# openai/tiktoken

Measured on NVIDIA H100. Metric: input_GB_per_s, higher is better.
Workload: dtype u8

## Files before the change

include/b200bpe.h:

```cpp
#ifndef B200BPE_H
#define B200BPE_H

#include <stdint.h>

#ifdef __cplusplus
extern "C" {
#endif

#define B200BPE_OK        0
#define B200BPE_EINVAL   -1
#define B200BPE_EPATTERN -2
#define B200BPE_EDUPRANK -3
#define B200BPE_ECUDA    -4
#define B200BPE_ENOBYTE  -5
#define B200BPE_EKEY     -6
#define B200BPE_ESPECIAL -7
#define B200BPE_ECAPACITY -8
#define B200BPE_ENOPAIR  -9

typedef struct b200bpe b200bpe_t;
typedef struct b200bpe_result b200bpe_result_t;

int b200bpe_create(const uint8_t *tok_bytes, const uint64_t *tok_off, const uint32_t *tok_rank,
                   uint32_t n_tok,
                   const uint8_t *sp_bytes, const uint64_t *sp_off, const uint32_t *sp_rank,
                   uint32_t n_sp,
                   const char *pat_str, int device, b200bpe_t **out);

int b200bpe_create_multi(const uint8_t *tok_bytes, const uint64_t *tok_off, const uint32_t *tok_rank,
                         uint32_t n_tok,
                         const uint8_t *sp_bytes, const uint64_t *sp_off, const uint32_t *sp_rank,
                         uint32_t n_sp,
                         const char *pat_str, const int *devices, int n_dev, b200bpe_t **out);

int b200bpe_n_devices(b200bpe_t *h);

int b200bpe_trim(b200bpe_t *h);

void b200bpe_destroy(b200bpe_t *h);

int b200bpe_encode_ordinary_batch(b200bpe_t *h, const uint8_t *text, const uint64_t *doc_off,
                                  uint64_t n_docs, b200bpe_result_t **out);

int b200bpe_encode_batch(b200bpe_t *h, const uint8_t *text, const uint64_t *doc_off, uint64_t n_docs,
                         const uint8_t *allowed, b200bpe_result_t **out);

int b200bpe_encode_batch_special(b200bpe_t *h, const uint8_t *text, const uint64_t *doc_off, uint64_t n_docs,
                                 const uint8_t *flags, b200bpe_result_t **out, int32_t *special_index);

int b200bpe_encode_bytes_batch(b200bpe_t *h, const uint8_t *text, const uint64_t *doc_off, uint64_t n_docs,
                               b200bpe_result_t **out);

int b200bpe_encode_with_unstable_batch(b200bpe_t *h, const uint8_t *text, const uint64_t *doc_off, uint64_t n_docs,
                                       const uint8_t *flags, b200bpe_result_t **stable, b200bpe_result_t **completions,
                                       int32_t *special_index);

int b200bpe_bpe_train(const uint8_t *text, const uint64_t *doc_off, uint64_t n_docs, const char *pat_str,
                      uint32_t vocab_size, int device, uint32_t *merges_out, uint64_t merges_cap,
                      uint64_t *n_merges_out, double *stats8);

const char *b200bpe_special_name(b200bpe_t *h, int32_t index);

int b200bpe_encode_device(b200bpe_t *h, const uint8_t *d_text, uint64_t n_bytes,
                          const uint64_t *d_doc_off, uint64_t n_docs,
                          uint32_t *d_tokens, uint64_t *d_tok_off, uint64_t *n_tokens, void *stream);

int b200bpe_encode_device_async(b200bpe_t *h, const uint8_t *d_text, uint64_t n_bytes,
                                const uint64_t *d_doc_off, uint64_t n_docs,
                                uint32_t *d_tokens, uint64_t *d_tok_off, uint64_t *d_counts, void *stream);
int b200bpe_device_wait(b200bpe_t *h, uint64_t *n_tokens);

int b200bpe_encode_single_piece(b200bpe_t *h, const uint8_t *piece, uint64_t len, b200bpe_result_t **out);

const uint32_t *b200bpe_result_tokens(const b200bpe_result_t *r);
const uint64_t *b200bpe_result_offsets(const b200bpe_result_t *r);
uint64_t b200bpe_result_n_tokens(const b200bpe_result_t *r);
const uint64_t *b200bpe_result_groups(const b200bpe_result_t *r, uint64_t *n_groups);
uint64_t b200bpe_result_n_docs(const b200bpe_result_t *r);
void b200bpe_result_free(b200bpe_result_t *r);

int b200bpe_decode_bytes(b200bpe_t *h, const uint32_t *tokens, uint64_t n_tokens, uint8_t *out,
                         uint64_t out_cap, uint64_t *out_len, uint32_t *bad_token);

int b200bpe_decode_batch(b200bpe_t *h, const uint32_t *tokens, const uint64_t *tok_off, uint64_t n_docs,
                         b200bpe_result_t **out, uint32_t *bad_token);

int b200bpe_last_timings(b200bpe_t *h, float *ms9, uint32_t *n_launches);

#define B200BPE_GREW_MISS 1u
#define B200BPE_GREW_SLOW 2u
#define B200BPE_GREW_LONG 4u
int b200bpe_last_reruns(b200bpe_t *h, uint32_t *grown, uint32_t *reruns, uint32_t *token_passes);

int b200bpe_last_piece_classes(b200bpe_t *h, uint64_t *counts8, int *lane_per_piece);

int b200bpe_last_bytes_repairs(b200bpe_t *h, uint64_t *n_docs_repaired);

int b200bpe_last_unstable(b200bpe_t *h, uint64_t *stats5);

int b200bpe_last_miss_memo(b200bpe_t *h, uint64_t *misses, uint64_t *merged, uint64_t *unplaced);

int b200bpe_table_bytes(b200bpe_t *h, uint64_t *bytes4);

int b200bpe_device_count(void);

const char *b200bpe_last_error(void);
const char *b200bpe_version(void);

#ifdef __cplusplus
}
#endif
#endif
```

tiktoken_b200/_lib.py:

```python
from __future__ import annotations

import ctypes as C
import os
import subprocess

_CSRC = os.path.join(os.path.dirname(os.path.abspath(__file__)), "csrc")
_SO = os.path.join(_CSRC, "libb200bpe.so")
_SOURCES = ["b200bpe.cu", "dev_common.cuh", "kernels_pretok.cuh", "kernels_long.cuh", "kernels_mid.cuh", "kernels_pmerge.cuh", "kernels_encode.cuh",
            "kernels_special.cuh", "kernels_decode.cuh", "kernels_bytes.cuh", "kernels_unstable.cuh", "kernels_train.cuh", "utf8_check.cuh", "bpe_device.cuh", "bpe_tables.h", "pretok_rules.cuh",
            "pretok_fast.cuh", "text_access.cuh", "unicode_classes.inc"]

OK, EINVAL, EPATTERN, EDUPRANK, ECUDA, ENOBYTE, EKEY, ESPECIAL, ECAPACITY, ENOPAIR = 0, -1, -2, -3, -4, -5, -6, -7, -8, -9

NVCC_FLAGS = ["-gencode", "arch=compute_90a,code=sm_90a", "-O3", "-lineinfo", "-std=c++17",
              "-shared", "-Xcompiler", "-fPIC"]


def build(force: bool = False) -> str:
    srcs = [os.path.join(_CSRC, s) for s in _SOURCES] + [
        os.path.join(os.path.dirname(_CSRC), "..", "include", "b200bpe.h")]
    stale = force or not os.path.exists(_SO) or any(
        os.path.getmtime(s) > os.path.getmtime(_SO) for s in srcs if os.path.exists(s))
    if stale:
        nvcc = os.environ.get("NVCC", "/usr/local/cuda/bin/nvcc")
        if not os.path.exists(nvcc):
            nvcc = "nvcc"
        subprocess.check_call([nvcc] + NVCC_FLAGS + ["-o", _SO, os.path.join(_CSRC, "b200bpe.cu")])
    return _SO


_lib = None


def lib() -> C.CDLL:
    global _lib
    if _lib is not None:
        return _lib
    so = os.environ.get("B200BPE_LIB") or _SO
    if not os.path.exists(so):
        raise RuntimeError(
            f"{so} is missing: build it with `python -c 'import __graft_entry__ as g; g.build()'` "
            "(tiktoken_b200 has no CPU fallback)")
    L = C.CDLL(so)
    vp, u64, u32, i32 = C.c_void_p, C.c_uint64, C.c_uint32, C.c_int
    L.b200bpe_create.restype = i32
    L.b200bpe_create.argtypes = [vp, vp, vp, u32, vp, vp, vp, u32, C.c_char_p, i32, C.POINTER(vp)]
    L.b200bpe_create_multi.restype = i32
    L.b200bpe_create_multi.argtypes = [vp, vp, vp, u32, vp, vp, vp, u32, C.c_char_p, vp, i32, C.POINTER(vp)]
    L.b200bpe_trim.restype = i32
    L.b200bpe_trim.argtypes = [vp]
    L.b200bpe_n_devices.restype = i32
    L.b200bpe_n_devices.argtypes = [vp]
    L.b200bpe_encode_batch_special.restype = i32
    L.b200bpe_encode_batch_special.argtypes = [vp, vp, vp, u64, vp, C.POINTER(vp), C.POINTER(C.c_int32)]
    L.b200bpe_special_name.restype = C.c_char_p
    L.b200bpe_special_name.argtypes = [vp, C.c_int32]
    L.b200bpe_encode_device_async.restype = i32
    L.b200bpe_encode_device_async.argtypes = [vp, vp, u64, vp, u64, vp, vp, vp, vp]
    L.b200bpe_device_wait.restype = i32
    L.b200bpe_device_wait.argtypes = [vp, C.POINTER(u64)]
    L.b200bpe_destroy.restype = None
    L.b200bpe_destroy.argtypes = [vp]
    L.b200bpe_encode_ordinary_batch.restype = i32
    L.b200bpe_encode_ordinary_batch.argtypes = [vp, vp, vp, u64, C.POINTER(vp)]
    L.b200bpe_encode_batch.restype = i32
    L.b200bpe_encode_batch.argtypes = [vp, vp, vp, u64, vp, C.POINTER(vp)]
    L.b200bpe_encode_device.restype = i32
    L.b200bpe_encode_device.argtypes = [vp, vp, u64, vp, u64, vp, vp, C.POINTER(u64), vp]
    L.b200bpe_encode_bytes_batch.restype = i32
    L.b200bpe_encode_bytes_batch.argtypes = [vp, vp, vp, u64, C.POINTER(vp)]
    L.b200bpe_last_bytes_repairs.restype = i32
    L.b200bpe_last_bytes_repairs.argtypes = [vp, C.POINTER(u64)]
    L.b200bpe_encode_with_unstable_batch.restype = i32
    L.b200bpe_encode_with_unstable_batch.argtypes = [vp, vp, vp, u64, vp, C.POINTER(vp), C.POINTER(vp), C.POINTER(C.c_int32)]
    L.b200bpe_result_groups.restype = vp
    L.b200bpe_result_groups.argtypes = [vp, C.POINTER(u64)]
    L.b200bpe_last_unstable.restype = i32
    L.b200bpe_last_unstable.argtypes = [vp, vp]
    L.b200bpe_last_miss_memo.restype = i32
    L.b200bpe_last_miss_memo.argtypes = [vp, C.POINTER(u64), C.POINTER(u64), C.POINTER(u64)]
    L.b200bpe_encode_single_piece.restype = i32
    L.b200bpe_encode_single_piece.argtypes = [vp, vp, u64, C.POINTER(vp)]
    L.b200bpe_result_tokens.restype = vp
    L.b200bpe_result_tokens.argtypes = [vp]
    L.b200bpe_result_offsets.restype = vp
    L.b200bpe_result_offsets.argtypes = [vp]
    L.b200bpe_result_n_tokens.restype = u64
    L.b200bpe_result_n_tokens.argtypes = [vp]
    L.b200bpe_result_n_docs.restype = u64
    L.b200bpe_result_n_docs.argtypes = [vp]
    L.b200bpe_result_free.restype = None
    L.b200bpe_result_free.argtypes = [vp]
    L.b200bpe_decode_bytes.restype = i32
    L.b200bpe_decode_bytes.argtypes = [vp, vp, u64, vp, u64, C.POINTER(u64), C.POINTER(u32)]
    L.b200bpe_decode_batch.restype = i32
    L.b200bpe_decode_batch.argtypes = [vp, vp, vp, u64, C.POINTER(vp), C.POINTER(u32)]
    L.b200bpe_last_timings.restype = i32
    L.b200bpe_last_timings.argtypes = [vp, vp, C.POINTER(u32)]
    L.b200bpe_last_reruns.restype = i32
    L.b200bpe_last_reruns.argtypes = [vp, C.POINTER(u32), C.POINTER(u32), C.POINTER(u32)]
    L.b200bpe_last_piece_classes.restype = i32
    L.b200bpe_last_piece_classes.argtypes = [vp, vp, C.POINTER(i32)]
    L.b200bpe_table_bytes.restype = i32
    L.b200bpe_table_bytes.argtypes = [vp, vp]
    L.b200bpe_device_count.restype = i32
    L.b200bpe_device_count.argtypes = []
    L.b200bpe_bpe_train.restype = i32
    L.b200bpe_bpe_train.argtypes = [vp, vp, u64, C.c_char_p, u32, i32, vp, u64, C.POINTER(u64), vp]
    L.b200bpe_last_error.restype = C.c_char_p
    L.b200bpe_version.restype = C.c_char_p
    _lib = L
    return L


EXPORTS = [
    "b200bpe_create", "b200bpe_destroy", "b200bpe_encode_ordinary_batch", "b200bpe_encode_batch",
    "b200bpe_encode_device", "b200bpe_encode_single_piece", "b200bpe_result_tokens",
    "b200bpe_result_offsets", "b200bpe_result_n_tokens", "b200bpe_result_n_docs", "b200bpe_result_free",
    "b200bpe_decode_bytes", "b200bpe_decode_batch", "b200bpe_last_timings", "b200bpe_table_bytes", "b200bpe_last_error",
    "b200bpe_version", "b200bpe_device_count", "b200bpe_create_multi", "b200bpe_n_devices", "b200bpe_encode_batch_special",
    "b200bpe_special_name", "b200bpe_encode_device_async", "b200bpe_device_wait", "b200bpe_trim", "b200bpe_last_reruns",
    "b200bpe_last_piece_classes", "b200bpe_encode_bytes_batch", "b200bpe_last_bytes_repairs", "b200bpe_last_miss_memo",
    "b200bpe_encode_with_unstable_batch", "b200bpe_result_groups", "b200bpe_last_unstable", "b200bpe_bpe_train",
]

GREW_MISS, GREW_SLOW, GREW_LONG = 1, 2, 4


def last_error() -> str:
    return (lib().b200bpe_last_error() or b"").decode("utf-8", "replace")


def check(rc: int) -> None:
    if rc == OK:
        return
    msg = last_error()
    if rc in (EINVAL, EPATTERN, EDUPRANK, ESPECIAL, ENOPAIR):
        raise ValueError(msg)
    if rc == EKEY:
        raise KeyError(msg)
    if rc == ENOBYTE:
        raise KeyError(msg)
    raise RuntimeError(msg)
```

tiktoken_b200/_tiktoken.py:

```python
from __future__ import annotations

import ctypes as C
import threading

import numpy as np

from . import _lib

try:
    from . import _b200pack
except ImportError:
    _b200pack = None


def _ptr(a: np.ndarray):
    return C.c_void_p(a.ctypes.data)


def _flatten_bytes(items: list[bytes]):
    blob = b"".join(items)
    off = np.zeros(len(items) + 1, dtype=np.uint64)
    if items:
        np.cumsum(np.fromiter((len(b) for b in items), dtype=np.uint64, count=len(items)), out=off[1:])
    arr = np.frombuffer(blob, dtype=np.uint8) if blob else np.zeros(1, np.uint8)
# ... 253 lines not shown
        if s in self._special:
            return self._special[s]
        raise KeyError(bytes(piece))

    def _encode_bytes(self, data: bytes) -> list[int]:
        try:
            text = data.decode("utf-8")
        except UnicodeDecodeError:
            raise NotImplementedError(
                "_encode_bytes on invalid UTF-8 (unstable-token path, src/py.rs:79-112) is out of scope "
                "of the GPU encoder") from None
        return self.encode_ordinary(text)

    def encode_with_unstable(self, text: str, allowed_special):
        raise NotImplementedError("encode_with_unstable (completion search, src/lib.rs:444-599) is out of scope")

    def decode_bytes(self, tokens) -> bytes:
        arr = np.ascontiguousarray(np.asarray(tokens, dtype=np.uint32))
        n = len(arr)
        if n == 0:
            return b""
        out_len = C.c_uint64(0)
        bad = C.c_uint32(0)
        cap = max(64, 8 * n)
        while True:
            out = np.empty(cap, np.uint8)
            rc = self._L.b200bpe_decode_bytes(self._h, _ptr(arr), n, _ptr(out), cap, C.byref(out_len), C.byref(bad))
            if rc == _lib.EKEY:
                raise KeyError(f"Invalid token for decoding: {bad.value}")
            _lib.check(rc)
            if out_len.value <= cap:
                return out[:out_len.value].tobytes()
            cap = int(out_len.value)

    def decode_batch_buffer(self, tokens: np.ndarray, tok_off: np.ndarray):
        tokens = np.ascontiguousarray(tokens, np.uint32)
        tok_off = np.ascontiguousarray(tok_off, np.uint64)
        res = C.c_void_p()
        bad = C.c_uint32(0)
        rc = self._L.b200bpe_decode_batch(self._h, _ptr(tokens if len(tokens) else np.zeros(1, np.uint32)), _ptr(tok_off),
                                          len(tok_off) - 1, C.byref(res), C.byref(bad))
        if rc == _lib.EKEY:
            raise KeyError(f"Invalid token for decoding: {bad.value}")
        _lib.check(rc)
        n_bytes = int(self._L.b200bpe_result_n_tokens(res))
        n_docs = int(self._L.b200bpe_result_n_docs(res))
        data = np.ctypeslib.as_array(C.cast(self._L.b200bpe_result_tokens(res), C.POINTER(C.c_uint8)),
                                     shape=(max(n_bytes, 1),))[:n_bytes].copy()
        off = np.ctypeslib.as_array(C.cast(self._L.b200bpe_result_offsets(res), C.POINTER(C.c_uint64)),
                                    shape=(n_docs + 1,)).copy()
        self._L.b200bpe_result_free(res)
        return data, off

    def decode_bytes_batch(self, batch) -> list[bytes]:
        lens = np.fromiter((len(t) for t in batch), dtype=np.uint64, count=len(batch))
        off = np.zeros(len(batch) + 1, np.uint64)
        np.cumsum(lens, out=off[1:])
        toks = np.zeros(int(off[-1]), np.uint32)
        for i, t in enumerate(batch):
            toks[int(off[i]):int(off[i + 1])] = np.asarray(t, dtype=np.uint32)
        data, boff = self.decode_batch_buffer(toks, off)
        raw = data.tobytes()
        return [raw[int(boff[i]):int(boff[i + 1])] for i in range(len(batch))]

    def decode_single_token_bytes(self, token: int) -> bytes:
        if self._decoder is None:
            self._decoder = {v: k for k, v in self._encoder.items()}
            self._decoder.update({v: k.encode("utf-8") for k, v in self._special.items()})
        try:
            return self._decoder[token]
        except KeyError:
            raise KeyError(str(token)) from None

    def token_byte_values(self) -> list[bytes]:
        return sorted(self._encoder.keys())

    def last_timings(self) -> dict:
        ms = (C.c_float * 9)()
        n = C.c_uint32(0)
        self._L.b200bpe_last_timings(self._h, ms, C.byref(n))
        keys = ["mark_docs_ms", "pretok_ms", "long_ms", "encode_ms", "device_total_ms", "h2d_ms", "d2h_ms", "gather_ms", "probe_ms"]
        d = {k: float(ms[i]) for i, k in enumerate(keys)}
        d["launches"] = int(n.value)
        return d

    def last_reruns(self) -> dict:
        grown, reruns, passes = C.c_uint32(0), C.c_uint32(0), C.c_uint32(0)
        _lib.check(self._L.b200bpe_last_reruns(self._h, C.byref(grown), C.byref(reruns), C.byref(passes)))
        names = {_lib.GREW_MISS: "miss", _lib.GREW_SLOW: "slow", _lib.GREW_LONG: "long"}
        return {"grown": {s for bit, s in names.items() if grown.value & bit}, "reruns": int(reruns.value),
                "token_passes": int(passes.value)}

    def last_piece_classes(self) -> dict:
        counts, lane = (C.c_uint64 * 8)(), C.c_int32(0)
        _lib.check(self._L.b200bpe_last_piece_classes(self._h, counts, C.byref(lane)))
        return {"counts": [int(x) for x in counts], "lane_per_piece": bool(lane.value)}

    def last_bytes_repairs(self) -> int:
        n = C.c_uint64(0)
        _lib.check(self._L.b200bpe_last_bytes_repairs(self._h, C.byref(n)))
        return int(n.value)

    def last_unstable(self) -> dict:
        v = (C.c_uint64 * 5)()
        _lib.check(self._L.b200bpe_last_unstable(self._h, v))
        return dict(zip(["docs", "encoded", "bpe_candidates", "rounds", "completions"], (int(x) for x in v)))

    def last_miss_memo(self) -> dict:
        v = [C.c_uint64(0) for _ in range(3)]
        _lib.check(self._L.b200bpe_last_miss_memo(self._h, *(C.byref(x) for x in v)))
        return {"misses": int(v[0].value), "merged": int(v[1].value), "unplaced": int(v[2].value)}

    def trim(self) -> None:
        _lib.check(self._L.b200bpe_trim(self._h))

    def table_bytes(self) -> dict:
        b = (C.c_uint64 * 4)()
        self._L.b200bpe_table_bytes(self._h, b)
        return {"piece_table": int(b[0]), "pair_table": int(b[1]), "long_token_table": int(b[2]), "unicode": int(b[3])}

    def encode_device_async(self, d_text_ptr: int, n_bytes: int, d_doc_off_ptr: int, n_docs: int, d_tokens_ptr: int,
                            d_tok_off_ptr: int, d_counts_ptr: int = 0, stream: int = 0) -> None:
        _lib.check(self._L.b200bpe_encode_device_async(self._h, C.c_void_p(d_text_ptr), n_bytes, C.c_void_p(d_doc_off_ptr),
                                                       n_docs, C.c_void_p(d_tokens_ptr), C.c_void_p(d_tok_off_ptr),
                                                       C.c_void_p(d_counts_ptr), C.c_void_p(stream)))

    def device_wait(self) -> int:
        n = C.c_uint64(0)
        _lib.check(self._L.b200bpe_device_wait(self._h, C.byref(n)))
        return int(n.value)

    def encode_device(self, d_text_ptr: int, n_bytes: int, d_doc_off_ptr: int, n_docs: int, d_tokens_ptr: int,
                      d_tok_off_ptr: int, stream: int = 0) -> int:
        n = C.c_uint64(0)
        rc = self._L.b200bpe_encode_device(self._h, C.c_void_p(d_text_ptr), n_bytes, C.c_void_p(d_doc_off_ptr),
                                           n_docs, C.c_void_p(d_tokens_ptr), C.c_void_p(d_tok_off_ptr), C.byref(n),
                                           C.c_void_p(stream))
        _lib.check(rc)
        return int(n.value)
```

tiktoken_b200/csrc/b200bpe.cu:

```cuda
#include <cuda_runtime.h>
#include <stdint.h>
#include <stdio.h>
#include <stdlib.h>
#include <string.h>

#include <algorithm>
#include <atomic>
#include <condition_variable>
#include <deque>
#include <functional>
#include <mutex>
#include <string>
#include <thread>
#include <vector>

#include "../../include/b200bpe.h"
#include "dev_common.cuh"
#include "kernels_pretok.cuh"
#include "kernels_long.cuh"
#include "kernels_mid.cuh"
#include "kernels_pmerge.cuh"
#include "kernels_encode.cuh"
#include "kernels_special.cuh"
#include "kernels_decode.cuh"
// ... 42 lines not shown
        return e;
    }
    void release() { if (p) cudaFree(p); p = nullptr; cap = 0; }
};

struct PinnedBuf {
    void *p = nullptr; size_t cap = 0;
};

long env_long(const char *name, long dflt, long lo, long hi) {
    const char *v = getenv(name);
    if (!v || !*v) return dflt;
    long x = atol(v);
    return x < lo ? lo : x > hi ? hi : x;
}

size_t env_chunk_bytes() {
    const char *v = getenv("B200BPE_CHUNK_MB");
    const long x = v ? atol(v) : 0;
    return x >= 1 && x <= 2048 ? (size_t)x << 20 : 0;
}

struct TaskPool {
    std::vector<std::thread> th; std::mutex mu; std::condition_variable cv; std::deque<std::function<void()>> q; bool stop = false;
    void ensure(int n) {
        std::lock_guard<std::mutex> lk(mu);
        while ((int)th.size() < n) th.emplace_back([this] {
            for (;;) {
                std::function<void()> f;
                {
                    std::unique_lock<std::mutex> lk(mu);
                    cv.wait(lk, [this] { return stop || !q.empty(); });
                    if (q.empty()) return;
                    f = std::move(q.front()); q.pop_front();
                }
                f();
            }
        });
    }
    void push(std::function<void()> f) { { std::lock_guard<std::mutex> lk(mu); q.push_back(std::move(f)); } cv.notify_one(); }
    ~TaskPool() {
        { std::lock_guard<std::mutex> lk(mu); stop = true; }
        cv.notify_all();
        for (auto &t : th) t.join();
    }
};
struct Latch {
    std::mutex mu; std::condition_variable cv; int left;
    explicit Latch(int n) : left(n) {}
    void done() { std::lock_guard<std::mutex> lk(mu); if (--left == 0) cv.notify_all(); }
    void wait() { std::unique_lock<std::mutex> lk(mu); cv.wait(lk, [this] { return left == 0; }); }
};
void pool_for(TaskPool *pool, size_t n, size_t block, const std::function<void(size_t, size_t)> &fn) {
    const size_t nb = (n + block - 1) / block;
    if (!pool || nb <= 1) { if (n) fn(0, n); return; }
    Latch latch((int)nb);
    for (size_t b = 0; b < nb; b++) pool->push([&, b] { fn(b * block, std::min(n, (b + 1) * block)); latch.done(); });
    latch.wait();
}

}

struct Slot {
    DevBuf<uint8_t> w_text; DevBuf<unsigned long long> w_docoff, w_tokoff, w_sub_base;
    DevBuf<uint32_t> w_ptok, w_mres, w_mq_pos, w_mq_roff, w_doc_tiles, w_sub_count; DevBuf<uint8_t> w_mq_len;
    DevBuf<uint4> w_mq_key, w_mq_skey, w_mq_smeta, w_mq_rec;
    DevBuf<uint4> w_memo_key; DevBuf<uint32_t> w_memo_owner, w_mq_slot, w_mq_own, w_memo_bn;
    DevBuf<uint32_t> w_dbits, w_pbits, w_psum, w_sfd, w_lidx, w_out, w_ltok, w_hbits, w_ibits, w_sbits, w_cbits, w_slow;
    DevBuf<unsigned long long> w_lq_start, w_lq_off; DevBuf<unsigned int> w_lq_len, w_lq_ntok, w_lq_cls, w_big_n, w_sort_hist;
    DevBuf<unsigned long long> w_big_dst, w_big_src, w_scan_part;
    DevBuf<uint32_t> w_idA, w_rkA, w_idB, w_rkB, w_aux1, w_aux2; DevBuf<uint8_t> w_flag, w_spflags;
    DevBuf<uint32_t> w_vup, w_kdrop, w_btail, w_b2out, w_bout; DevBuf<uint8_t> w_btext;
    DevBuf<unsigned long long> w_b2doc, w_b2off, w_bbase, w_bpart;
    Counters *d_bctr = nullptr; BytesCounters *d_bytes = nullptr, *h_bytes = nullptr;
    DevBuf<uint32_t> w_ulen, w_unit;
    size_t long_cap = 0;
    size_t miss_cap = 0, mres_cap = 0;
    size_t slow_cap = 0;
    Counters *d_ctr = nullptr; Counters *h_ctr = nullptr;
    unsigned int *d_sticky = nullptr;
    cudaStream_t stream = nullptr;
    cudaStream_t side = nullptr;
    cudaStream_t side2 = nullptr;
    cudaStream_t up = nullptr;
    static const int N_EV = 15;
    cudaEvent_t ev[N_EV];
    PinnedBuf stage;
    float last_ms[9] = {0, 0, 0, 0, 0, 0, 0, 0, 0};
    uint32_t last_launches = 0;
    bool ok = false;

    cudaError_t init() {
        cudaError_t e = cudaMalloc((void **)&d_ctr, sizeof(Counters));
        if (e == cudaSuccess) e = cudaMalloc((void **)&d_sticky, 16);
        if (e == cudaSuccess) e = cudaMemset(d_sticky, 0, 16);
        if (e == cudaSuccess) e = cudaHostAlloc((void **)&h_ctr, sizeof(Counters), cudaHostAllocPortable);
        if (e == cudaSuccess) e = cudaStreamCreateWithFlags(&stream, cudaStreamNonBlocking);
        if (e == cudaSuccess) e = cudaStreamCreateWithFlags(&side, cudaStreamNonBlocking);
        if (e == cudaSuccess) e = cudaStreamCreateWithFlags(&side2, cudaStreamNonBlocking);
        if (e == cudaSuccess) e = cudaStreamCreateWithFlags(&up, cudaStreamNonBlocking);
        for (int i = 0; i < N_EV && e == cudaSuccess; i++) e = cudaEventCreate(&ev[i]);
        ok = (e == cudaSuccess);
        return e;
    }
    void release_workspace() {
        w_text.release(); w_docoff.release(); w_tokoff.release(); w_sub_base.release();
        w_ptok.release(); w_mres.release(); w_mq_pos.release(); w_mq_roff.release(); w_doc_tiles.release(); w_sub_count.release();
        w_mq_len.release(); w_mq_rec.release(); w_mq_key.release(); w_mq_skey.release(); w_mq_smeta.release();
        w_memo_key.release(); w_memo_owner.release(); w_mq_slot.release(); w_mq_own.release(); w_memo_bn.release();
        w_dbits.release(); w_pbits.release(); w_psum.release(); w_sfd.release(); w_lidx.release(); w_out.release(); w_ltok.release();
        w_hbits.release(); w_ibits.release(); w_sbits.release(); w_cbits.release(); w_slow.release(); w_spflags.release();
        w_lq_start.release(); w_lq_off.release(); w_lq_len.release(); w_lq_ntok.release(); w_lq_cls.release(); w_big_n.release();
        w_sort_hist.release(); w_big_dst.release(); w_big_src.release(); w_scan_part.release();
        w_idA.release(); w_rkA.release(); w_idB.release(); w_rkB.release(); w_aux1.release(); w_aux2.release();
        w_flag.release();
        w_vup.release(); w_kdrop.release(); w_btail.release(); w_b2out.release(); w_bout.release(); w_btext.release();
        w_b2doc.release(); w_b2off.release(); w_bbase.release(); w_bpart.release();
        w_ulen.release(); w_unit.release();
        if (stage.p) cudaFreeHost(stage.p);
        stage.p = nullptr; stage.cap = 0;
        long_cap = miss_cap = mres_cap = slow_cap = 0;
    }
    void destroy() {
        release_workspace();
        if (d_ctr) cudaFree(d_ctr);
        if (d_bctr) cudaFree(d_bctr);
        if (d_bytes) cudaFree(d_bytes);
        if (h_bytes) cudaFreeHost(h_bytes);
        if (d_sticky) cudaFree(d_sticky);
        if (h_ctr) cudaFreeHost(h_ctr);
        if (ok) { for (int i = 0; i < N_EV; i++) cudaEventDestroy(ev[i]); }
        if (stream) cudaStreamDestroy(stream);
        if (side) cudaStreamDestroy(side);
        if (side2) cudaStreamDestroy(side2);
        if (up) cudaStreamDestroy(up);
    }
};

struct UnstWs {
    DevBuf<uint32_t> it_lo, it_cnt, it_bytes, it_doc; DevBuf<unsigned long long> item_base, cbase, tbase, part;
    DevBuf<uint4> cinfo; DevBuf<uint32_t> o_len, s_len, out_o, out_s, nkeep, slot, keep, kc;
    DevBuf<unsigned long long> o_off, s_off, tokoff_o, tokoff_s, rcb, rtb, zeros, grp_off;
    DevBuf<uint8_t> text_o, text_s;
    DevBuf<unsigned long long> tkey; DevBuf<uint32_t> tidx, tloc;
    uint32_t tslots_min = 0;
    DevBuf<uint32_t> res_tok, res_doc, grp; DevBuf<unsigned long long> res_off;
    UnstCounters *d_uc = nullptr, *h_uc = nullptr;
    Counters *d_sctr = nullptr;
    void release() {
        it_lo.release(); it_cnt.release(); it_bytes.release(); it_doc.release(); item_base.release(); cbase.release();
        tbase.release(); part.release(); cinfo.release(); o_len.release(); s_len.release(); out_o.release(); out_s.release();
        nkeep.release(); slot.release(); keep.release(); kc.release(); o_off.release(); s_off.release(); tokoff_o.release();
        tokoff_s.release(); rcb.release(); rtb.release(); zeros.release(); grp_off.release(); text_o.release(); text_s.release();
        tkey.release(); tidx.release(); tloc.release(); res_tok.release(); res_doc.release(); grp.release(); res_off.release();
    }
};

struct DevCtx {
    int device = 0;
    uint8_t *arena = nullptr; size_t arena_bytes = 0;
    DevTables T; UcTables uc;
    uint32_t *d_tok_boff = nullptr; uint8_t *d_tok_blob = nullptr;
    uint32_t *d_tok_space = nullptr;
    SpecialTables sp;
    uint8_t *d_sp_arena = nullptr;
    UnstTables ut;
    uint8_t *d_ut_arena = nullptr;
    UnstWs uw;
    static const int N_SLOTS = 3;
    Slot slots[N_SLOTS];
    int n_sm = 0;
};

struct b200bpe_result {
    b200bpe *owner = nullptr;
    PinnedBuf tok, off;
    std::vector<uint32_t> vtok;
    std::vector<uint64_t> voff;
    std::vector<uint64_t> vgrp;
    bool on_host_vec = false;
    uint64_t n_tokens = 0, n_docs = 0;
};

struct PendingDeviceCall {
    bool active = false; int queued = 0;
    const uint8_t *d_text = nullptr; uint64_t n_bytes = 0; const unsigned long long *d_doc_off = nullptr; uint64_t n_docs = 0;
    uint32_t *d_tokens = nullptr; unsigned long long *d_tok_off = nullptr; unsigned long long *d_counts = nullptr;
    cudaStream_t st = nullptr;
};

struct b200bpe {
    int pattern = 0;
    HostTables H;
    std::vector<std::string> specials; std::vector<uint32_t> special_rank;
    std::unordered_map<uint32_t, std::string> special_decoder;
    SpecialHost sp_host;
    uint32_t n_ids = 0; bool decode_on_device = true;
    std::vector<uint32_t> tok_space;
    std::vector<DevCtx *> devs;
    uint64_t table_bytes[4] = {0, 0, 0, 0};
    float last_ms[9] = {0, 0, 0, 0, 0, 0, 0, 0, 0};
    uint32_t last_launches = 0;
    std::atomic<uint32_t> last_grown{0}, last_reruns{0}, last_token_passes{0};
    std::atomic<uint64_t> last_cls[N_CLS] = {};
    std::atomic<int> last_lane_per_piece{0};
    std::atomic<uint64_t> last_bytes_repairs{0};
    std::atomic<uint64_t> last_unstable[5] = {};
    struct {
        bool built = false;
        std::vector<uint32_t> sorted, space, ur_idx, ur_off, ur_tok; std::vector<unsigned long long> lenpre;
        std::vector<uint8_t> u8info; uint32_t max_len = 0;
    } uh;
    std::atomic<uint64_t> last_memo[3] = {};
    void reset_reruns() {
        last_grown = 0; last_reruns = 0; last_token_passes = 0; last_bytes_repairs = 0;
        for (auto &c : last_unstable) c = 0;
        for (auto &c : last_memo) c = 0;
        for (auto &c : last_cls) c = 0;
        last_lane_per_piece = 0;
    }
    void set_piece_classes(const uint64_t *cls) {
        for (int c = 0; c < N_CLS; c++) last_cls[c] = cls[c];
        last_lane_per_piece = mid_group ? 0 : 1;
    }
    void set_miss_memo(const uint64_t *memo) { for (int i = 0; i < 3; i++) last_memo[i] = memo[i]; }
    size_t chunk_bytes = 64u << 20; bool chunk_forced = false;
    int copy_threads = 4;
    TaskPool *pool = nullptr;
    long memo_slots = -1;
    bool mid_group = true;
    std::mutex mu;
    std::vector<PinnedBuf> pinned_pool;
    int live_results = 0;
    bool dead = false;
    PendingDeviceCall pending;

    PinnedBuf take_pinned(size_t bytes) {
        for (size_t i = 0; i < pinned_pool.size(); i++)
            if (pinned_pool[i].cap >= bytes && pinned_pool[i].cap <= 2 * bytes + (64u << 20)) {
                PinnedBuf b = pinned_pool[i]; pinned_pool.erase(pinned_pool.begin() + i); return b;
            }
        PinnedBuf b; size_t want = bytes + bytes / 8 + 4096;
        if (cudaHostAlloc(&b.p, want, cudaHostAllocPortable) != cudaSuccess) { cudaGetLastError(); b.p = nullptr; b.cap = 0; return b; }
        b.cap = want; return b;
    }
    void give_pinned(PinnedBuf b) {
        if (!b.p) return;
        if (pinned_pool.size() >= 4) {
            size_t mn = 0;
            for (size_t i = 1; i < pinned_pool.size(); i++) if (pinned_pool[i].cap < pinned_pool[mn].cap) mn = i;
            if (pinned_pool[mn].cap >= b.cap) { cudaFreeHost(b.p); return; }
            cudaFreeHost(pinned_pool[mn].p); pinned_pool[mn] = b; return;
        }
        pinned_pool.push_back(b);
    }
};

extern "C" const char *b200bpe_last_error(void) { return g_last_error.c_str(); }
extern "C" const char *b200bpe_version(void) { return "b200bpe 0.2 (sm_90a)"; }
extern "C" int b200bpe_device_count(void) {
    int n = 0;
    if (cudaGetDeviceCount(&n) != cudaSuccess) { cudaGetLastError(); return 0; }
    return n;
}

static void devctx_destroy(DevCtx *D) {
    if (!D) return;
    cudaSetDevice(D->device);
    for (int i = 0; i < DevCtx::N_SLOTS; i++) D->slots[i].destroy();
    if (D->arena) cudaFree(D->arena);
    if (D->d_tok_boff) cudaFree(D->d_tok_boff);
    if (D->d_tok_blob) cudaFree(D->d_tok_blob);
    if (D->d_tok_space) cudaFree(D->d_tok_space);
    if (D->d_sp_arena) cudaFree(D->d_sp_arena);
    if (D->d_ut_arena) cudaFree(D->d_ut_arena);
    D->uw.release();
    delete D;
}

static void uc_ascii_table(uint8_t *ascii) {
    for (int i = 0; i < 128; i++) ascii[i] = UC_STAGE2[(uint32_t)UC_STAGE1[0] * 256 + i];
}

static int devctx_create(b200bpe *h, int device, const std::vector<uint32_t> &boff, const std::vector<uint8_t> &blob,
                         DevCtx **out) {
    DevCtx *D = new DevCtx();
    D->device = device;
    const HostTables &H = h->H;
    cudaError_t e = cudaSetDevice(device);
    if (e == cudaSuccess) e = cudaDeviceGetAttribute(&D->n_sm, cudaDevAttrMultiProcessorCount, device);
    uint8_t ascii[128];
    uc_ascii_table(ascii);
    struct Part { const void *src; size_t bytes; size_t off; };
    enum { P_NARROW, P_WIDE, P_PAIR2, P_BYTE_ID, P_PAIR, P_ASCII, P_UC1, P_UC2, P_LONG, P_BLOB, N_PARTS };
    Part parts[N_PARTS] = {{H.narrow_tab.data(), H.narrow_tab.size() * sizeof(U4), 0},
                           {H.wide_tab.data(), H.wide_tab.size() * sizeof(U4), 0}, {H.pair2.data(), 65536 * 4, 0},
                           {H.byte_id.data(), 256 * 4, 0}, {H.pair_tab.data(), H.pair_tab.size() * sizeof(U4), 0},
// ... 83 lines not shown
            bool all = !sp->empty();
            for (char c : *sp) all &= c == ' ' || c == '\n' || c == '\t';
            if (all) space[id >> 5] |= 1u << (id & 31);
        }
    }
    boff[h->n_ids] = (uint32_t)blob.size(); boff[h->n_ids + 1] = (uint32_t)blob.size();
    if (blob.empty()) blob.push_back(0);
    for (int i = 0; i < n_dev; i++) {
        DevCtx *D = nullptr;
        rc = devctx_create(h, devices[i], boff, blob, &D);
        if (rc) { for (auto *d : h->devs) devctx_destroy(d); delete h; return rc; }
        h->devs.push_back(D);
    }
    if (const size_t cb = env_chunk_bytes()) { h->chunk_bytes = cb; h->chunk_forced = true; }
    h->mid_group = H.max_rank < MIDG_MAX_RANK;
    h->memo_slots = env_long("B200BPE_MISS_MEMO_SLOTS", -1, 0, 1l << 24);
    h->copy_threads = (int)env_long("B200BPE_COPY_THREADS", std::max(1u, std::min(16u, std::thread::hardware_concurrency() / 4)), 1, 64);
    h->table_bytes[0] = (H.narrow_tab.size() + H.wide_tab.size()) * sizeof(U4);
    h->table_bytes[1] = H.pair_tab.size() * sizeof(U4) + 65536 * 4 + 1024;
    h->table_bytes[2] = H.long_tab.size() * sizeof(U4) + H.long_blob.size();
    h->table_bytes[3] = sizeof(UC_STAGE1) + sizeof(UC_STAGE2) + 128;
    *out = h;
    return B200BPE_OK;
}

extern "C" int b200bpe_create(const uint8_t *tok_bytes, const uint64_t *tok_off, const uint32_t *tok_rank,
                              uint32_t n_tok, const uint8_t *sp_bytes, const uint64_t *sp_off,
                              const uint32_t *sp_rank, uint32_t n_sp, const char *pat_str, int device,
                              b200bpe_t **out) {
    return b200bpe_create_multi(tok_bytes, tok_off, tok_rank, n_tok, sp_bytes, sp_off, sp_rank, n_sp, pat_str, &device, 1, out);
}

static void engine_teardown(b200bpe *h) {
    DeviceGuard guard;
    for (auto *d : h->devs) devctx_destroy(d);
    for (auto &b : h->pinned_pool) cudaFreeHost(b.p);
    delete h->pool;
    delete h;
}

extern "C" void b200bpe_destroy(b200bpe_t *h) {
    if (!h) return;
    {
        std::lock_guard<std::mutex> lk(h->mu);
        if (h->live_results > 0) { h->dead = true; return; }
    }
    engine_teardown(h);
}

extern "C" int b200bpe_n_devices(b200bpe_t *h) { return h ? (int)h->devs.size() : 0; }

extern "C" int b200bpe_trim(b200bpe_t *h) {
    if (!h) return fail(B200BPE_EINVAL, "null handle");
    std::lock_guard<std::mutex> lk(h->mu);
    if (h->pending.active) return fail(B200BPE_EINVAL, "a device call is in flight: b200bpe_device_wait first");
    DeviceGuard guard;
    for (auto *D : h->devs) {
        CUDA_TRY(cudaSetDevice(D->device));
        for (int i = 0; i < DevCtx::N_SLOTS; i++) {
            CUDA_TRY(cudaStreamSynchronize(D->slots[i].stream));
            CUDA_TRY(cudaStreamSynchronize(D->slots[i].side));
            CUDA_TRY(cudaStreamSynchronize(D->slots[i].side2));
            D->slots[i].release_workspace();
        }
    }
    for (auto &b : h->pinned_pool) cudaFreeHost(b.p);
    h->pinned_pool.clear();
    return B200BPE_OK;
}

struct PipeArgs {
    const uint8_t *d_text = nullptr; uint64_t n_bytes = 0;
    const unsigned long long *d_doc_off = nullptr; uint64_t n_docs = 0;
    uint32_t *d_out = nullptr; unsigned long long *d_tok_off = nullptr;
    unsigned long long *d_counts = nullptr;
    cudaStream_t st = nullptr;
    bool single_piece = false;
    bool bytes = false;
    bool unstable = false;
    const uint8_t *sp_flags = nullptr;
};

static const unsigned long long MISS_CAP_MIN = 1u << 16, LONG_CAP_MIN = 1u << 20;

static int enqueue_pipeline(b200bpe *h, DevCtx *D, Slot &S, const PipeArgs &a) {
    const uint64_t n_bytes = a.n_bytes, n_docs = a.n_docs;
    cudaStream_t st = a.st;
    if (n_bytes >= (1ull << 32) - 4096) return fail(B200BPE_EINVAL, "batch too large for one call (>= 4 GiB)");
    if (n_docs >= 0xFFFFFFFEull) return fail(B200BPE_EINVAL, "too many documents in one call");
    const long long n_words = (long long)((n_bytes + 1 + 31) / 32);
    const long long n_tiles = (n_words + 31) / 32;
    const size_t pb_words = (size_t)n_tiles * 32 + STAGE_PW + 8;
    CUDA_TRY(S.w_dbits.ensure((size_t)n_words + 8));
    CUDA_TRY(S.w_pbits.ensure(pb_words));
    CUDA_TRY(S.w_psum.ensure((size_t)(n_words >> 5) + 4));
    CUDA_TRY(S.w_sfd.ensure((size_t)n_words + 4));
    CUDA_TRY(S.w_sub_base.ensure((size_t)n_tiles + 2));
    CUDA_TRY(S.w_scan_part.ensure((size_t)(n_tiles / SCAN_ITEMS) + 4));
    CUDA_TRY(S.w_sub_count.ensure((size_t)n_tiles + 2));
    CUDA_TRY(S.w_ptok.ensure((size_t)n_tiles * SUB_BYTES + 64));
    {
        const size_t want_q = std::max<size_t>((size_t)(n_bytes / 8) + 4096, MISS_CAP_MIN);
        const size_t want_r = std::max<size_t>((size_t)(n_bytes / 2) + 4096, MISS_CAP_MIN);
        if (S.miss_cap < want_q) S.miss_cap = want_q;
        if (S.mres_cap < want_r) S.mres_cap = want_r;
        const size_t mcap = S.miss_cap;
        CUDA_TRY(S.w_mq_pos.ensure(mcap)); CUDA_TRY(S.w_mq_roff.ensure(mcap)); CUDA_TRY(S.w_mq_rec.ensure(mcap));
        CUDA_TRY(S.w_mq_len.ensure(mcap));
        CUDA_TRY(S.w_mq_key.ensure(mcap)); CUDA_TRY(S.w_mq_skey.ensure(mcap)); CUDA_TRY(S.w_mq_smeta.ensure(mcap));
        CUDA_TRY(S.w_mres.ensure(S.mres_cap + 64));
        CUDA_TRY(S.w_sort_hist.ensure((size_t)D->n_sm * SORT_BLOCKS_PER_SM * 17 + 32));
        CUDA_TRY(S.w_mq_slot.ensure(mcap)); CUDA_TRY(S.w_mq_own.ensure(mcap));
        CUDA_TRY(S.w_memo_bn.ensure((size_t)D->n_sm * SORT_BLOCKS_PER_SM * 2 + 4));
    }
    uint32_t memo_slots = 0;
    if (h->memo_slots) {
        const uint64_t want = h->memo_slots > 0 ? (uint64_t)h->memo_slots
                                                : std::min<uint64_t>(std::max<uint64_t>(n_bytes / 128, 1u << 12), 1u << 21);
        memo_slots = 1;
        while (memo_slots < want) memo_slots <<= 1;
        CUDA_TRY(S.w_memo_key.ensure(memo_slots)); CUDA_TRY(S.w_memo_owner.ensure(memo_slots));
    }
    {
        const size_t want = std::max<size_t>((size_t)(n_bytes / 8) + 4096, MISS_CAP_MIN);
        if (S.slow_cap < want) S.slow_cap = want;
        CUDA_TRY(S.w_slow.ensure(S.slow_cap));
    }
    CUDA_TRY(S.w_lidx.ensure((size_t)(n_bytes >> 4) + 4));
    CUDA_TRY(S.w_ltok.ensure((size_t)n_bytes + 4));
    const size_t qcap = (size_t)(n_bytes / (SHORT_MAX + 1)) + 4;
    CUDA_TRY(S.w_lq_start.ensure(qcap)); CUDA_TRY(S.w_lq_off.ensure(qcap));
    CUDA_TRY(S.w_lq_len.ensure(qcap)); CUDA_TRY(S.w_lq_ntok.ensure(qcap));
    size_t cls_cap[N_CLS], cls_total = 0;
    {
        const size_t min_len[N_CLS] = {SHORT_MAX + 1, 33, 65, 129, 257, GROUP_MAX + 1, BLOCK_MIN + 1, CLUSTER_MIN + 1};
        for (int c = 0; c < N_CLS; c++) { cls_cap[c] = (size_t)(n_bytes / min_len[c]) + 4; cls_total += cls_cap[c]; }
    }
    CUDA_TRY(S.w_lq_cls.ensure(cls_total));
    CUDA_TRY(S.w_big_n.ensure((size_t)(n_bytes / 4097) + 4));
    CUDA_TRY(S.w_big_dst.ensure((size_t)(n_bytes / 4097) + 4)); CUDA_TRY(S.w_big_src.ensure((size_t)(n_bytes / 4097) + 4));
    {
        const size_t want = std::max<size_t>((size_t)(n_bytes / 8) + 4096, LONG_CAP_MIN);
        if (S.long_cap < want) S.long_cap = want;
        const size_t lc = S.long_cap + 4;
        CUDA_TRY(S.w_idA.ensure(lc)); CUDA_TRY(S.w_rkA.ensure(lc)); CUDA_TRY(S.w_idB.ensure(lc)); CUDA_TRY(S.w_rkB.ensure(lc));
        CUDA_TRY(S.w_aux1.ensure(lc)); CUDA_TRY(S.w_aux2.ensure(lc)); CUDA_TRY(S.w_flag.ensure(lc));
    }
    LongQ q;
    q.start = S.w_lq_start.p; q.len = S.w_lq_len.p; q.off = S.w_lq_off.p; q.ntok = S.w_lq_ntok.p; q.scratch_cap = S.long_cap;
    q.sub_count = S.w_sub_count.p;
    { size_t o = 0; for (int c = 0; c < N_CLS; c++) { q.cls[c] = S.w_lq_cls.p + o; o += cls_cap[c]; } }
    const bool sparse_docs = (n_docs + 1) * 4 < (uint64_t)n_tiles;
    if (sparse_docs) CUDA_TRY(S.w_doc_tiles.ensure((size_t)n_docs + 8));
    uint32_t launches = 0;

    CUDA_TRY(cudaEventRecord(S.ev[0], st));
    CUDA_TRY(cudaMemsetAsync(S.d_ctr, 0, sizeof(Counters), st));
    CUDA_TRY(cudaMemsetAsync(S.w_dbits.p, 0, ((size_t)n_words + 8) * 4, st));
    CUDA_TRY(cudaMemsetAsync(S.w_sfd.p, 0xFF, ((size_t)n_words + 4) * 4, st));
    CUDA_TRY(cudaMemsetAsync(S.w_sub_count.p, 0, ((size_t)n_tiles + 2) * 4, st));
    CUDA_TRY(cudaMemsetAsync(S.w_pbits.p + n_words, 0, (pb_words - (size_t)n_words) * 4, st));
    {
        unsigned long long nd1 = n_docs + 1;
        mark_docs_kernel<<<(unsigned)((nd1 + 255) / 256), 256, 0, st>>>(a.d_doc_off, n_docs, n_bytes, S.w_dbits.p, S.w_sfd.p,
                                                                       sparse_docs ? S.w_doc_tiles.p : nullptr, S.d_ctr);
        launches++;
    }
    const uint32_t *hbits = S.w_dbits.p;
    const uint32_t *ibits = nullptr, *sbits = nullptr;
    if (a.sp_flags && !h->specials.empty() && !a.single_piece) {
        const size_t nsp = h->specials.size();
        CUDA_TRY(S.w_spflags.ensure(nsp + 16));
        CUDA_TRY(S.w_hbits.ensure((size_t)n_words + 8)); CUDA_TRY(S.w_ibits.ensure((size_t)n_words + 8));
        CUDA_TRY(S.w_sbits.ensure((size_t)n_words + 8)); CUDA_TRY(S.w_cbits.ensure((size_t)n_words + 8));
        CUDA_TRY(cudaMemcpyAsync(S.w_spflags.p, a.sp_flags, nsp, cudaMemcpyHostToDevice, st));
        CUDA_TRY(cudaMemsetAsync(S.w_ibits.p, 0, ((size_t)n_words + 8) * 4, st));
        CUDA_TRY(cudaMemsetAsync(S.w_cbits.p + n_words, 0, 8 * 4, st));
        const unsigned grid = (unsigned)((n_words + 255) / 256);
        special_mark_kernel<<<grid, 256, 0, st>>>(a.d_text, (long long)n_bytes, S.w_dbits.p, D->sp, S.w_spflags.p, S.w_cbits.p, n_words, S.d_ctr);
        CUDA_TRY(cudaMemcpyAsync(S.w_hbits.p, S.w_dbits.p, ((size_t)n_words + 8) * 4, cudaMemcpyDeviceToDevice, st));
        special_resolve_kernel<<<grid, 256, 0, st>>>(a.d_text, (long long)n_bytes, S.w_dbits.p, D->sp, S.w_spflags.p, S.w_cbits.p,
                                                     S.w_hbits.p, S.w_ibits.p, S.w_sbits.p, S.w_ltok.p, n_words, S.d_ctr);
        launches += 2;
        hbits = S.w_hbits.p; ibits = S.w_ibits.p; sbits = S.w_sbits.p;
    } else if (a.bytes) {
        if (!D->d_tok_space) {
            CUDA_TRY(cudaMalloc((void **)&D->d_tok_space, h->tok_space.size() * 4));
            CUDA_TRY(cudaMemcpy(D->d_tok_space, h->tok_space.data(), h->tok_space.size() * 4, cudaMemcpyHostToDevice));
        }
        if (!S.d_bytes) CUDA_TRY(cudaMalloc((void **)&S.d_bytes, sizeof(BytesCounters)));
        if (!S.h_bytes) CUDA_TRY(cudaHostAlloc((void **)&S.h_bytes, sizeof(BytesCounters), cudaHostAllocPortable));
        CUDA_TRY(cudaMemsetAsync(S.d_bytes, 0, sizeof(BytesCounters), st));
        CUDA_TRY(S.w_hbits.ensure((size_t)n_words + 8)); CUDA_TRY(S.w_ibits.ensure((size_t)n_words + 8));
        CUDA_TRY(S.w_sbits.ensure((size_t)n_words + 8)); CUDA_TRY(S.w_vup.ensure((size_t)n_docs + 2));
        CUDA_TRY(cudaMemsetAsync(S.w_ibits.p, 0, ((size_t)n_words + 8) * 4, st));
        CUDA_TRY(cudaMemsetAsync(S.w_sbits.p, 0, ((size_t)n_words + 8) * 4, st));
        CUDA_TRY(cudaMemsetAsync(S.w_vup.p, 0xFF, ((size_t)n_docs + 2) * 4, st));
        utf8_check_kernel<<<(unsigned)((n_words + 255) / 256), 256, 0, st>>>(a.d_text, (long long)n_bytes, S.w_dbits.p, S.w_sfd.p,
                                                                            a.d_doc_off, n_docs, n_words, S.w_vup.p);
        CUDA_TRY(cudaMemcpyAsync(S.w_hbits.p, S.w_dbits.p, ((size_t)n_words + 8) * 4, cudaMemcpyDeviceToDevice, st));
        if (n_docs) bytes_cut_kernel<<<(unsigned)((n_docs * 32 + 255) / 256), 256, 0, st>>>(a.d_doc_off, n_docs, S.w_vup.p, S.w_hbits.p,
                                                                                          S.w_ibits.p, S.w_sbits.p, S.w_ltok.p);
        launches += 2;
        hbits = S.w_hbits.p; ibits = S.w_ibits.p; sbits = S.w_sbits.p;
    }
    CUDA_TRY(cudaEventRecord(S.ev[1], st));
    {
        unsigned grid = (unsigned)((n_words + 255) / 256);
        if (a.single_piece) single_piece_bits_kernel<<<grid, 256, 0, st>>>(S.w_pbits.p, S.w_psum.p, S.w_dbits.p, n_words);
        else {
            const uint32_t scap = (uint32_t)std::min<size_t>(S.slow_cap, 0xFFFFFFF0u);
#define B2_PRETOK(P)                                                                                                                   \
    if (a.bytes) pretok_kernel<P, true><<<grid, 256, 0, st>>>(a.d_text, (long long)n_bytes, hbits, D->uc, S.w_pbits.p, S.w_psum.p,       \
                                                             n_words, ibits, S.w_slow.p, scap, S.d_ctr);                              \
    else pretok_kernel<P><<<grid, 256, 0, st>>>(a.d_text, (long long)n_bytes, hbits, D->uc, S.w_pbits.p, S.w_psum.p, n_words, ibits,          \
                                          S.w_slow.p, scap, S.d_ctr);                                                                  \
    pretok_slow_kernel<P><<<D->n_sm * 8, 256, 0, st>>>(a.d_text, (long long)n_bytes, hbits, D->uc, S.w_pbits.p, S.w_psum.p, S.w_slow.p, scap, S.d_ctr)
            if (h->pattern == PAT_R50K) { B2_PRETOK(PAT_R50K); }
            else if (h->pattern == PAT_CL100K) { B2_PRETOK(PAT_CL100K); }
            else { B2_PRETOK(PAT_O200K); }
#undef B2_PRETOK
            launches++;
        }
        launches++;
    }
    CUDA_TRY(cudaEventRecord(S.ev[2], st));
    {
        unsigned grid = (unsigned)((n_words + 255) / 256);
        find_long_kernel<<<grid, 256, 0, st>>>(S.w_pbits.p, S.w_psum.p, (long long)n_bytes, n_words, q, S.w_lidx.p, sbits, S.d_ctr);
        launches++;
        cudaStream_t ls = S.side, ls2 = S.side2;
        CUDA_TRY(cudaEventRecord(S.ev[10], st));
        CUDA_TRY(cudaStreamWaitEvent(ls, S.ev[10], 0));
        CUDA_TRY(cudaStreamWaitEvent(ls2, S.ev[10], 0));
        CUDA_TRY(cudaEventRecord(S.ev[11], ls));
        LongScratch LS{S.w_idA.p, S.w_rkA.p, S.w_idB.p, S.w_rkB.p, S.w_aux1.p, S.w_aux2.p, S.w_flag.p};
        if (h->mid_group) {
            pmerge_kernel<256, 3><<<D->n_sm * 10, PM_WARPS * 32, 0, ls>>>(a.d_text, D->T, q, S.w_ltok.p, S.d_ctr);
            pmerge_long_kernel<<<D->n_sm * 4, PM_WARPS_L * 32, 0, ls>>>(a.d_text, D->T, q, S.w_ltok.p, S.d_ctr);
            mid_group32_kernel<<<D->n_sm * 4, MIDG_WARPS * 32, 0, ls>>>(a.d_text, D->T, q, S.w_ltok.p, S.d_ctr, 2);
            mid_group16_kernel<<<D->n_sm * 9, MIDG_WARPS * 32, 0, ls>>>(a.d_text, D->T, q, S.w_ltok.p, S.d_ctr, 1);
        } else {
            mid_thread_kernel<<<D->n_sm * 3, MID_WARPS * 32, MID_SMEM_BYTES, ls>>>(a.d_text, D->T, q, S.w_ltok.p, S.d_ctr);
            long_piece_kernel<<<D->n_sm * 8, LONG_WARPS * 32, 0, ls>>>(a.d_text, D->T, q, LS, S.w_ltok.p, S.d_ctr, CLS_G1024);
        }
        long_piece_kernel<<<D->n_sm * 8, LONG_WARPS * 32, 0, ls2>>>(a.d_text, D->T, q, LS, S.w_ltok.p, S.d_ctr, CLS_WARP);
        giant_piece_kernel<<<D->n_sm, GIANT_THREADS, 0, ls2>>>(a.d_text, D->T, q, LS, S.w_ltok.p, S.d_ctr);
        cluster_piece_kernel<<<(D->n_sm / CLUSTER_CTAS) * CLUSTER_CTAS, GIANT_THREADS, 0, ls2>>>(a.d_text, D->T, q, LS, S.w_ltok.p, S.d_ctr);
        CUDA_TRY(cudaEventRecord(S.ev[13], ls2));
        CUDA_TRY(cudaEventRecord(S.ev[12], ls));
        launches += 5;
    }
    CUDA_TRY(cudaEventRecord(S.ev[3], st));
    {
        TileParams p;
        p.text = a.d_text; p.n_bytes = (long long)n_bytes; p.n_words = n_words; p.n_sub = n_tiles;
        p.pbits = S.w_pbits.p; p.dbits = S.w_dbits.p; p.span_first_doc = S.w_sfd.p;
        p.doc_off = a.d_doc_off; p.n_docs = n_docs; p.q = q; p.lidx = S.w_lidx.p; p.ltok = S.w_ltok.p;
        p.ptok = S.w_ptok.p; p.mres = S.w_mres.p; p.sbits = sbits;
        p.mq.key = S.w_mq_key.p; p.mq.pos = S.w_mq_pos.p; p.mq.roff = S.w_mq_roff.p; p.mq.len = S.w_mq_len.p; p.mq.rec = S.w_mq_rec.p;
        p.doc_tiles = S.w_doc_tiles.p;
        p.mq.skey = S.w_mq_skey.p; p.mq.smeta = S.w_mq_smeta.p; p.mq.cap = (uint32_t)std::min<size_t>(S.miss_cap, 0xFFFFFFF0u);
        p.mq.mres_cap = S.mres_cap;
        p.sub_count = S.w_sub_count.p; p.sub_base = S.w_sub_base.p;
        p.out = a.d_out; p.tok_off = a.d_tok_off; p.ctr = S.d_ctr;
        p.big_dst = S.w_big_dst.p; p.big_src = S.w_big_src.p; p.big_n = S.w_big_n.p;
        MissMemo memo;
        memo.key = S.w_memo_key.p; memo.owner = S.w_memo_owner.p; memo.slot = S.w_mq_slot.p; memo.own = S.w_mq_own.p;
        memo.block_n = S.w_memo_bn.p; memo.mask = memo_slots ? memo_slots - 1 : 0; memo.on = memo_slots ? 1u : 0u;
        memo.limit = std::max<uint32_t>(1u, memo_slots / 2 / (uint32_t)(D->n_sm * SORT_BLOCKS_PER_SM));
        const long long want_blocks = (n_tiles + ENC_WARPS - 1) / ENC_WARPS;
        const unsigned probe_grid = (unsigned)std::min<long long>(want_blocks, (long long)D->n_sm * PROBE_BLOCKS_PER_SM);
        probe_kernel<<<probe_grid, ENC_WARPS * 32, 0, st>>>(p, D->T);
        CUDA_TRY(cudaEventRecord(S.ev[8], st));
        const int sort_blocks = D->n_sm * SORT_BLOCKS_PER_SM;
        if (memo_slots) CUDA_TRY(cudaMemsetAsync(S.w_memo_key.p, 0, (size_t)memo_slots * sizeof(uint4), st));
        miss_dedup_kernel<<<sort_blocks, SORT_THREADS, 0, st>>>(p, memo, S.w_sort_hist.p);
        miss_base_kernel<<<1, 17 * 32, 0, st>>>(S.w_sort_hist.p, sort_blocks);
        miss_scatter_kernel<<<sort_blocks, SORT_THREADS, 0, st>>>(p, memo, S.w_sort_hist.p);
        miss_kernel<<<D->n_sm * 16, MISS_WARPS * 32, 0, st>>>(p, D->T);
        if (memo_slots) miss_fanout_kernel<<<sort_blocks, SORT_THREADS, 0, st>>>(p, memo);
        CUDA_TRY(cudaEventRecord(S.ev[7], st));
        CUDA_TRY(cudaStreamWaitEvent(st, S.ev[12], 0));
        CUDA_TRY(cudaStreamWaitEvent(st, S.ev[13], 0));
        {
            const long long nb = (n_tiles + SCAN_ITEMS - 1) / SCAN_ITEMS;
            scan_partial_kernel<<<(unsigned)nb, 256, 0, st>>>(S.w_sub_count.p, n_tiles, S.w_scan_part.p);
            scan_top_kernel<<<1, 1024, 0, st>>>(S.w_scan_part.p, nb, S.d_ctr);
            scan_final_kernel<<<(unsigned)nb, 256, 0, st>>>(S.w_sub_count.p, n_tiles, S.w_scan_part.p, S.w_sub_base.p, S.d_ctr);
        }
        const unsigned gather_grid = (unsigned)((n_tiles + GATHER_WARPS - 1) / GATHER_WARPS);
        if (sparse_docs) {
            gather_kernel<0><<<gather_grid, GATHER_WARPS * 32, 0, st>>>(p);
            gather_kernel<1><<<(unsigned)((n_docs + 1 + GATHER_WARPS - 1) / GATHER_WARPS), GATHER_WARPS * 32, 0, st>>>(p);
        } else gather_kernel<2><<<gather_grid, GATHER_WARPS * 32, 0, st>>>(p);
        big_copy_kernel<<<D->n_sm * 2, 256, 0, st>>>(p);
        if (a.bytes && n_docs) {
            CUDA_TRY(S.w_kdrop.ensure((size_t)n_docs + 2)); CUDA_TRY(S.w_btail.ensure((size_t)n_docs + 2));
            bytes_repair_kernel<<<(unsigned)((n_docs * 32 + 255) / 256), 256, 0, st>>>(a.d_doc_off, n_docs, S.w_vup.p, S.w_pbits.p, a.d_out,
                                                                                      a.d_tok_off, D->d_tok_boff, D->d_tok_space, h->n_ids,
                                                                                      S.w_kdrop.p, S.w_btail.p, S.d_bytes, S.d_ctr);
            launches++;
        }
        if (a.unstable && n_docs) {
            CUDA_TRY(S.w_kdrop.ensure((size_t)n_docs + 2)); CUDA_TRY(S.w_ulen.ensure((size_t)n_docs + 2));
            CUDA_TRY(S.w_unit.ensure((size_t)n_docs + 2));
            unstable_walk_kernel<<<(unsigned)((n_docs * 32 + 255) / 256), 256, 0, st>>>(a.d_doc_off, n_docs, S.w_pbits.p, sbits, a.d_out,
                                                                                       a.d_tok_off, D->d_tok_boff, D->ut.space, h->n_ids,
                                                                                       D->ut.max_len, S.w_kdrop.p, S.w_ulen.p,
                                                                                       S.w_unit.p, S.d_ctr);
            launches++;
        }
        finalize_kernel<<<1, 32, 0, st>>>(S.d_ctr, S.d_sticky, a.d_counts, n_docs);
        launches += (sparse_docs ? 12 : 11) + (memo_slots ? 1 : 0);
    }
    CUDA_TRY(cudaEventRecord(S.ev[4], st));
    if (a.bytes) CUDA_TRY(cudaMemcpyAsync(S.h_bytes, S.d_bytes, sizeof(BytesCounters), cudaMemcpyDeviceToHost, st));
    CUDA_TRY(cudaMemcpyAsync(S.h_ctr, S.d_ctr, sizeof(Counters), cudaMemcpyDeviceToHost, st));
    CUDA_TRY(cudaEventRecord(S.ev[9], st));
    S.last_launches = launches;
    return B200BPE_OK;
}

static const int B200BPE_RETRY = 1;

static int collect_pipeline(b200bpe *h, Slot &S, int *special_idx, uint64_t *special_pos, uint32_t *grown) {
    (void)h;
    CUDA_TRY(cudaEventSynchronize(S.ev[9]));
    CUDA_TRY(cudaGetLastError());
    cudaEventElapsedTime(&S.last_ms[0], S.ev[0], S.ev[1]);
    cudaEventElapsedTime(&S.last_ms[1], S.ev[1], S.ev[2]);
    cudaEventElapsedTime(&S.last_ms[2], S.ev[11], S.ev[12]);
    cudaEventElapsedTime(&S.last_ms[3], S.ev[3], S.ev[7]);
    cudaEventElapsedTime(&S.last_ms[7], S.ev[7], S.ev[4]);
    cudaEventElapsedTime(&S.last_ms[8], S.ev[3], S.ev[8]);
    cudaEventElapsedTime(&S.last_ms[4], S.ev[0], S.ev[4]);
    const Counters &c = *S.h_ctr;
    if (c.err & ERR_DOCOFF)
        return fail(B200BPE_EINVAL, "document offsets must start at 0, be non-decreasing and end at n_bytes");
    if (c.err & ERR_SPECIAL) {
        const unsigned long long packed = ~c.special_pos;
        if (special_idx) *special_idx = (int)(packed & 0xFFFFu);
        if (special_pos) *special_pos = packed >> 16;
        return fail(B200BPE_ESPECIAL, "text contains a disallowed special token");
    }
    if (c.err & (ERR_LONGCAP | ERR_MISSCAP | ERR_SLOWCAP)) {
        if (c.err & ERR_SLOWCAP) S.slow_cap = (size_t)c.n_slow + (size_t)(c.n_slow / 8) + 4096;
        if (c.err & ERR_LONGCAP) S.long_cap = (size_t)c.long_bytes + (size_t)(c.long_bytes / 8) + 4096;
        if (c.err & ERR_MISSCAP) {
            S.miss_cap = std::max(S.miss_cap, (size_t)c.n_miss + (size_t)(c.n_miss / 8) + 4096);
            S.mres_cap = std::max(S.mres_cap, (size_t)c.miss_bytes + (size_t)(c.miss_bytes / 8) + 4096);
        }
        *grown |= ((c.err & ERR_MISSCAP) ? B200BPE_GREW_MISS : 0u) | ((c.err & ERR_SLOWCAP) ? B200BPE_GREW_SLOW : 0u) |
                  ((c.err & ERR_LONGCAP) ? B200BPE_GREW_LONG : 0u);
        return B200BPE_RETRY;
    }
    if (c.err & ERR_INTERNAL) return fail(B200BPE_ECUDA, "internal error: a merge kernel did not converge");
    if (c.err & ERR_NOBYTE)
        return fail(B200BPE_ENOBYTE, "a piece needs a single-byte token that mergeable_ranks does not contain");
    return B200BPE_OK;
}

static void add_miss_memo(const Slot &S, uint64_t *memo) {
    memo[0] += S.h_ctr->n_miss; memo[1] += S.h_ctr->n_owner; memo[2] += S.h_ctr->n_unplaced;
}

static int device_args_check(b200bpe *h, const uint8_t *d_text, uint64_t n_bytes, const uint64_t *d_doc_off, uint32_t *d_tokens,
                             uint64_t *d_tok_off) {
    if (!h || !d_doc_off || !d_tokens || !d_tok_off || (n_bytes && !d_text)) return fail(B200BPE_EINVAL, "null argument");
    return B200BPE_OK;
}

static int device_enqueue_locked(b200bpe *h, const PendingDeviceCall &c) {
    DevCtx *D = h->devs[0];
    Slot &S = D->slots[0];
    cudaStream_t st = c.st ? c.st : S.stream;
    const uint8_t *txt = c.d_text;
    if (((uintptr_t)c.d_text & 15u) != 0) {
        CUDA_TRY(S.w_text.ensure((size_t)c.n_bytes + 64));
        CUDA_TRY(cudaMemcpyAsync(S.w_text.p, c.d_text, c.n_bytes, cudaMemcpyDeviceToDevice, st));
        txt = S.w_text.p;
    }
    PipeArgs a;
    a.d_text = txt; a.n_bytes = c.n_bytes; a.d_doc_off = c.d_doc_off; a.n_docs = c.n_docs; a.d_out = c.d_tokens;
    a.d_tok_off = c.d_tok_off; a.d_counts = c.d_counts; a.st = st;
    return enqueue_pipeline(h, D, S, a);
}

extern "C" int b200bpe_encode_device_async(b200bpe_t *h, const uint8_t *d_text, uint64_t n_bytes, const uint64_t *d_doc_off,
                                           uint64_t n_docs, uint32_t *d_tokens, uint64_t *d_tok_off, uint64_t *d_counts,
                                           void *stream) {
    if (h) h->reset_reruns();
    int rc = device_args_check(h, d_text, n_bytes, d_doc_off, d_tokens, d_tok_off);
    if (rc) return rc;
    std::lock_guard<std::mutex> lk(h->mu);
    DeviceGuard guard;
    CUDA_TRY(cudaSetDevice(h->devs[0]->device));
    PendingDeviceCall c;
    c.active = true; c.queued = h->pending.active ? h->pending.queued + 1 : 1;
    c.d_text = d_text; c.n_bytes = n_bytes; c.d_doc_off = (const unsigned long long *)d_doc_off; c.n_docs = n_docs;
    c.d_tokens = d_tokens; c.d_tok_off = (unsigned long long *)d_tok_off; c.d_counts = (unsigned long long *)d_counts;
    c.st = (cudaStream_t)stream;
    rc = device_enqueue_locked(h, c);
    if (rc) return rc;
    h->pending = c;
    return B200BPE_OK;
}

extern "C" int b200bpe_device_wait(b200bpe_t *h, uint64_t *n_tokens) {
    if (!h) return fail(B200BPE_EINVAL, "null handle");
    h->reset_reruns();
    std::lock_guard<std::mutex> lk(h->mu);
    if (!h->pending.active) return fail(B200BPE_EINVAL, "no device call in flight");
    DeviceGuard guard;
    DevCtx *D = h->devs[0];
    CUDA_TRY(cudaSetDevice(D->device));
    Slot &S = D->slots[0];
    PendingDeviceCall c = h->pending;
    h->pending.active = false;
    h->last_token_passes = 1;
    cudaStream_t st = c.st ? c.st : S.stream;
    uint32_t grown = 0;
    int rc = collect_pipeline(h, S, nullptr, nullptr, &grown);
    h->last_grown = grown;
    const uint64_t total = S.h_ctr->total_tokens;
    unsigned int sticky = 0;
    CUDA_TRY(cudaMemcpyAsync(&sticky, S.d_sticky, sizeof(unsigned int), cudaMemcpyDeviceToHost, st));
    CUDA_TRY(cudaMemsetAsync(S.d_sticky, 0, sizeof(unsigned int), st));
    CUDA_TRY(cudaStreamSynchronize(st));
    uint64_t total2 = total;
    bool reran = false;
    for (int attempt = 0; rc == B200BPE_RETRY && attempt < 4; attempt++) {
        rc = device_enqueue_locked(h, c);
        if (rc) break;
        h->last_reruns++;
        rc = collect_pipeline(h, S, nullptr, nullptr, &grown);
        h->last_grown = grown;
        total2 = S.h_ctr->total_tokens;
        CUDA_TRY(cudaMemsetAsync(S.d_sticky, 0, sizeof(unsigned int), st));
        reran = true;
    }
    memcpy(h->last_ms, S.last_ms, sizeof(h->last_ms));
    h->last_ms[5] = h->last_ms[6] = 0.f;
    h->last_launches = S.last_launches;
    if (rc == B200BPE_RETRY) return fail(B200BPE_ECUDA, "work-space sizing did not converge");
    if (rc) return rc;
    if (c.queued > 1) {
        if (reran || (sticky & (ERR_LONGCAP | ERR_MISSCAP | ERR_SLOWCAP)))
            return fail(B200BPE_ECAPACITY, "a work-space had to grow while several device calls were queued: only the last "
                                           "one was re-run, re-issue the others");
        if (sticky & ERR_NOBYTE) return fail(B200BPE_ENOBYTE, "a piece needs a single-byte token that mergeable_ranks does not contain");
        if (sticky & ERR_DOCOFF) return fail(B200BPE_EINVAL, "malformed document offsets in a queued device call");
    }
    if (n_tokens) *n_tokens = total2;
    uint64_t cls[N_CLS];
    for (int k = 0; k < N_CLS; k++) cls[k] = S.h_ctr->n_cls[k];
    h->set_piece_classes(cls);
    uint64_t memo[3] = {};
    add_miss_memo(S, memo);
    h->set_miss_memo(memo);
    return B200BPE_OK;
}

extern "C" int b200bpe_encode_device(b200bpe_t *h, const uint8_t *d_text, uint64_t n_bytes, const uint64_t *d_doc_off,
                                     uint64_t n_docs, uint32_t *d_tokens, uint64_t *d_tok_off, uint64_t *n_tokens,
                                     void *stream) {
    int rc = b200bpe_encode_device_async(h, d_text, n_bytes, d_doc_off, n_docs, d_tokens, d_tok_off, nullptr, stream);
    if (rc) return rc;
    return b200bpe_device_wait(h, n_tokens);
}

static void enqueue_scan(const uint32_t *cnt, uint64_t n, unsigned long long *part, unsigned long long *base, Counters *ctr,
                         cudaStream_t st) {
    const long long nb = (long long)((n + SCAN_ITEMS - 1) / SCAN_ITEMS);
    scan_partial_kernel<<<(unsigned)nb, 256, 0, st>>>(cnt, (long long)n, part);
    scan_top_kernel<<<1, 1024, 0, st>>>(part, nb, ctr);
    scan_final_kernel<<<(unsigned)nb, 256, 0, st>>>(cnt, (long long)n, part, base, ctr);
}

static int run_again(b200bpe *h, DevCtx *D, Slot &S, const PipeArgs &a, uint64_t *cls, uint64_t *memo, uint32_t *grown,
                     uint32_t *reruns) {
    int rc = enqueue_pipeline(h, D, S, a);
    if (!rc) rc = collect_pipeline(h, S, nullptr, nullptr, grown);
    for (int attempt = 0; rc == B200BPE_RETRY && attempt < 4; attempt++) {
        rc = enqueue_pipeline(h, D, S, a);
        if (!rc) { (*reruns)++; rc = collect_pipeline(h, S, nullptr, nullptr, grown); }
    }
    if (rc == B200BPE_RETRY) rc = fail(B200BPE_ECUDA, "work-space sizing did not converge");
    if (rc) return rc;
    for (int i = 0; i < N_CLS; i++) cls[i] += S.h_ctr->n_cls[i];
    add_miss_memo(S, memo);
    return B200BPE_OK;
}

static int bytes_tail_runs(b200bpe *h, DevCtx *D, Slot &S, const PipeArgs &a1, uint64_t *nt, uint64_t *cls, uint64_t *memo,
                           uint32_t *grown, uint32_t *reruns) {
    const uint64_t n1 = S.h_ctr->total_tokens, drop = S.h_bytes->drop;
    const float ms1[9] = {S.last_ms[0], S.last_ms[1], S.last_ms[2], S.last_ms[3], S.last_ms[4], S.last_ms[5], S.last_ms[6],
                          S.last_ms[7], S.last_ms[8]};
    const uint32_t launches1 = S.last_launches;
    const uint64_t nd = a1.n_docs, tail = S.h_bytes->tail;
    cudaStream_t st = a1.st;
    CUDA_TRY(S.w_b2doc.ensure((size_t)nd + 2)); CUDA_TRY(S.w_b2off.ensure((size_t)nd + 2)); CUDA_TRY(S.w_bbase.ensure((size_t)nd + 2));
    CUDA_TRY(S.w_bpart.ensure((size_t)(nd / SCAN_ITEMS) + 4));
    CUDA_TRY(S.w_btext.ensure((size_t)tail + 64)); CUDA_TRY(S.w_b2out.ensure((size_t)tail + 64));
    if (!S.d_bctr) CUDA_TRY(cudaMalloc((void **)&S.d_bctr, sizeof(Counters)));
    CUDA_TRY(cudaEventRecord(S.ev[14], st));
    enqueue_scan(S.w_btail.p, nd, S.w_bpart.p, S.w_b2doc.p, S.d_bctr, st);
    bytes_gather_kernel<<<(unsigned)((tail + 16 * 256 - 1) / (16 * 256)), 256, 0, st>>>(a1.d_text, nd, S.w_vup.p, S.w_b2doc.p, S.w_btext.p);
    PipeArgs a2;
    a2.d_text = S.w_btext.p; a2.n_bytes = tail; a2.d_doc_off = S.w_b2doc.p; a2.n_docs = nd;
    a2.d_out = S.w_b2out.p; a2.d_tok_off = S.w_b2off.p; a2.st = st; a2.single_piece = true;
    int rc = run_again(h, D, S, a2, cls, memo, grown, reruns);
    if (rc) return rc;
    float ms2 = 0; cudaEventElapsedTime(&ms2, S.ev[14], S.ev[4]);
    const uint32_t launches2 = S.last_launches;
    *nt = n1 - drop + S.h_ctr->total_tokens;
    CUDA_TRY(S.w_bout.ensure((size_t)std::max<uint64_t>(*nt, a1.n_bytes) + 64));
    bytes_count_kernel<<<(unsigned)((nd + 255) / 256), 256, 0, st>>>(S.w_tokoff.p, S.w_b2off.p, S.w_kdrop.p, nd, S.w_btail.p);
    enqueue_scan(S.w_btail.p, nd, S.w_bpart.p, S.w_bbase.p, S.d_bctr, st);
    bytes_splice_kernel<<<(unsigned)std::min<uint64_t>(nd, (uint64_t)D->n_sm * 16), 256, 0, st>>>(
        S.w_out.p, S.w_tokoff.p, S.w_b2out.p, S.w_b2off.p, S.w_kdrop.p, S.w_bbase.p, nd, S.w_bout.p);
    CUDA_TRY(cudaGetLastError());
    std::swap(S.w_out, S.w_bout);
    std::swap(S.w_tokoff, S.w_bbase);
    memcpy(S.last_ms, ms1, sizeof(ms1));
    S.last_ms[4] += ms2;
    S.last_launches = launches1 + launches2 + 9;
    return B200BPE_OK;
}


static void host_byte_pair_encode(const DevTables &T, const std::string &b, std::vector<uint32_t> &ids) {
    const size_t n = b.size();
    ids.resize(n);
    for (size_t j = 0; j < n; j++) ids[j] = T.byte_id[(uint8_t)b[j]];
    std::vector<uint32_t> rk(n);
    auto rank_at = [&](size_t j) { return j + 1 < ids.size() ? pair_lookup(T, ids[j], ids[j + 1]) : RANK_MAX; };
    for (size_t j = 0; j < n; j++) rk[j] = rank_at(j);
    for (;;) {
        uint32_t best = RANK_MAX; size_t bj = 0;
        for (size_t j = 0; j < ids.size(); j++) if (rk[j] < best) { best = rk[j]; bj = j; }
        if (best == RANK_MAX) break;
        ids[bj] = best;
        ids.erase(ids.begin() + (long)bj + 1); rk.erase(rk.begin() + (long)bj + 1);
        rk[bj] = rank_at(bj);
        if (bj) rk[bj - 1] = rank_at(bj - 1);
    }
}

static void unstable_host_build(b200bpe *h) {
    auto &u = h->uh;
    if (u.built) return;
    const HostTables &H = h->H;
    const DevTables T = H.view();
    u.sorted.clear();
    for (auto &kv : H.decoder) u.sorted.push_back(kv.first);
    std::sort(u.sorted.begin(), u.sorted.end(), [&](uint32_t a, uint32_t b) { return H.decoder.at(a) < H.decoder.at(b); });
    u.lenpre.assign(u.sorted.size() + 1, 0);
    for (size_t i = 0; i < u.sorted.size(); i++) u.lenpre[i + 1] = u.lenpre[i] + H.decoder.at(u.sorted[i]).size();
    u.space.assign((size_t)h->n_ids / 32 + 2, 0);
    u.u8info.assign((size_t)h->n_ids + 1, 0);
    u.ur_idx.assign((size_t)h->n_ids + 1, UR_NONE);
    u.ur_off.assign(1, 0); u.ur_tok.clear();
    u.max_len = 0;
    std::vector<uint32_t> ids, zero;
    for (uint32_t id : u.sorted) {
        const std::string &b = H.decoder.at(id);
        u.max_len = std::max<uint32_t>(u.max_len, (uint32_t)b.size());
        bool all = !b.empty();
        for (char c : b) all &= c == ' ' || c == '\n' || c == '\t';
        if (all) u.space[id >> 5] |= 1u << (id & 31);
        uint32_t c = 0;
        while (c < b.size() && c < 4 && ((uint8_t)b[c] & 0xC0u) == 0x80u) c++;
        bool rest_ok = true;
        if (c < 4) {
            const uint8_t *r = (const uint8_t *)b.data() + c;
            const int64_t rn = (int64_t)b.size() - c;
            zero.assign((size_t)(rn / 32) + 3, 0);
            zero[0] = 1u;
            for (int64_t w = 0; w * 32 < rn && rest_ok; w++) rest_ok = utf8_bad_word(r, rn, zero.data(), w) == 0;
        }
        u.u8info[id] = (uint8_t)(c | (rest_ok ? 8u : 0u));
        if (b.size() >= 2) {
            host_byte_pair_encode(T, b, ids);
            if (!(ids.size() == 1 && ids[0] == id)) {
                u.ur_idx[id] = (uint32_t)(u.ur_off.size() - 1);
                u.ur_tok.insert(u.ur_tok.end(), ids.begin(), ids.end());
                u.ur_off.push_back((uint32_t)u.ur_tok.size());
            }
        }
    }
    u.built = true;
}

static int unstable_upload(b200bpe *h, DevCtx *D) {
    if (D->d_ut_arena) return B200BPE_OK;
    const auto &u = h->uh;
    struct Part { const void *src; size_t bytes; size_t off; };
    std::vector<uint32_t> one(1, 0);
    Part parts[] = {{u.sorted.data(), u.sorted.size() * 4, 0}, {u.lenpre.data(), u.lenpre.size() * 8, 0},
                    {u.space.data(), u.space.size() * 4, 0}, {u.u8info.data(), u.u8info.size(), 0},
                    {u.ur_idx.data(), u.ur_idx.size() * 4, 0}, {u.ur_off.data(), u.ur_off.size() * 4, 0},
                    {u.ur_tok.empty() ? one.data() : u.ur_tok.data(), std::max<size_t>(u.ur_tok.size(), 1) * 4, 0}};
    size_t total = 0;
    for (auto &p : parts) { p.off = total; total += (p.bytes + 255) & ~(size_t)255; }
    CUDA_TRY(cudaSetDevice(D->device));
    UnstWs &W = D->uw;
    if (!W.d_uc) CUDA_TRY(cudaMalloc((void **)&W.d_uc, sizeof(UnstCounters)));
    if (!W.h_uc) CUDA_TRY(cudaHostAlloc((void **)&W.h_uc, sizeof(UnstCounters), cudaHostAllocPortable));
    if (!W.d_sctr) CUDA_TRY(cudaMalloc((void **)&W.d_sctr, sizeof(Counters)));
    uint8_t *arena = nullptr;
    CUDA_TRY(cudaMalloc((void **)&arena, total));
    for (auto &p : parts)
        if (p.bytes) {
            cudaError_t e = cudaMemcpy(arena + p.off, p.src, p.bytes, cudaMemcpyHostToDevice);
            if (e != cudaSuccess) { cudaFree(arena); return fail(B200BPE_ECUDA, std::string("completion tables: ") + cudaGetErrorString(e)); }
        }
    D->d_ut_arena = arena;
    UnstTables &U = D->ut;
    U.sorted = (const uint32_t *)(arena + parts[0].off); U.n_sorted = (uint32_t)u.sorted.size();
    U.lenpre = (const unsigned long long *)(arena + parts[1].off);
    U.space = (const uint32_t *)(arena + parts[2].off);
    U.u8info = arena + parts[3].off;
    U.ur_idx = (const uint32_t *)(arena + parts[4].off);
    U.ur_off = (const uint32_t *)(arena + parts[5].off);
    U.ur_tok = (const uint32_t *)(arena + parts[6].off);
    U.tok_boff = D->d_tok_boff; U.tok_blob = D->d_tok_blob; U.n_ids = h->n_ids; U.max_len = u.max_len;
    return B200BPE_OK;
}

template <class Tp>
static cudaError_t grow_keep(DevBuf<Tp> &b, size_t used, size_t n, cudaStream_t st) {
    if (n <= b.cap) return cudaSuccess;
    DevBuf<Tp> nb;
    cudaError_t e = nb.ensure(std::max(n, 2 * b.cap));
    if (e == cudaSuccess && used) e = cudaMemcpyAsync(nb.p, b.p, used * sizeof(Tp), cudaMemcpyDeviceToDevice, st);
    if (e == cudaSuccess) e = cudaStreamSynchronize(st);
    if (e != cudaSuccess) { nb.release(); return e; }
    b.release();
    b = nb;
    return cudaSuccess;
}

static void uscan(UnstWs &W, const uint32_t *cnt, uint64_t n, unsigned long long *base, cudaStream_t st) {
    if (n == 0) { cudaMemsetAsync(base, 0, 8, st); return; }
    enqueue_scan(cnt, n, W.part.p, base, W.d_sctr, st);
}

struct UChunk {
    std::vector<uint32_t> tok; std::vector<uint64_t> off, grp;
};

static int unstable_search(b200bpe *h, DevCtx *D, Slot &S, const PipeArgs &a1, UChunk &out, uint64_t *stats, uint64_t *nt,
                           uint64_t *cls, uint64_t *memo, uint32_t *grown, uint32_t *reruns) {
    UnstWs &W = D->uw;
    const UnstTables &U = D->ut;
    const uint64_t nd = a1.n_docs;
    cudaStream_t st = a1.st;
    const float ms1[9] = {S.last_ms[0], S.last_ms[1], S.last_ms[2], S.last_ms[3], S.last_ms[4], S.last_ms[5], S.last_ms[6],
                          S.last_ms[7], S.last_ms[8]};
    const uint32_t launches1 = S.last_launches;
    out.tok.clear(); out.off.assign(1, 0); out.grp.assign((size_t)nd + 1, 0);
    if (nd == 0) return B200BPE_OK;
    const uint64_t n1 = *nt;
    CUDA_TRY(S.w_btail.ensure((size_t)nd + 2)); CUDA_TRY(S.w_bbase.ensure((size_t)nd + 2));
    CUDA_TRY(S.w_bpart.ensure((size_t)(nd / SCAN_ITEMS) + 4));
    CUDA_TRY(S.w_bout.ensure((size_t)std::max<uint64_t>(n1, a1.n_bytes) + 64));
    CUDA_TRY(W.zeros.ensure((size_t)nd + 2));
    if (!S.d_bctr) CUDA_TRY(cudaMalloc((void **)&S.d_bctr, sizeof(Counters)));
    CUDA_TRY(cudaMemsetAsync(W.zeros.p, 0, ((size_t)nd + 2) * 8, st));
    bytes_count_kernel<<<(unsigned)((nd + 255) / 256), 256, 0, st>>>(S.w_tokoff.p, W.zeros.p, S.w_kdrop.p, nd, S.w_btail.p);
    enqueue_scan(S.w_btail.p, nd, S.w_bpart.p, S.w_bbase.p, S.d_bctr, st);
    bytes_splice_kernel<<<(unsigned)std::min<uint64_t>(nd, (uint64_t)D->n_sm * 16), 256, 0, st>>>(
        S.w_out.p, S.w_tokoff.p, S.w_out.p, W.zeros.p, S.w_kdrop.p, S.w_bbase.p, nd, S.w_bout.p);
    std::swap(S.w_out, S.w_bout);
    std::swap(S.w_tokoff, S.w_bbase);
    CUDA_TRY(W.item_base.ensure((size_t)nd + 2));
    CUDA_TRY(W.part.ensure((size_t)(nd / SCAN_ITEMS) + 4));
    CUDA_TRY(cudaMemsetAsync(W.d_uc, 0, sizeof(UnstCounters), st));
    uscan(W, S.w_unit.p, nd, W.item_base.p, st);
    CUDA_TRY(cudaMemcpyAsync(&W.h_uc->tot[0], W.item_base.p + nd, 8, cudaMemcpyDeviceToHost, st));
    CUDA_TRY(cudaMemcpyAsync(&W.h_uc->tot[1], S.w_tokoff.p + nd, 8, cudaMemcpyDeviceToHost, st));
    CUDA_TRY(cudaStreamSynchronize(st));
    *nt = W.h_uc->tot[1];
    const uint64_t n_items = W.h_uc->tot[0];
    uint64_t n_cand = 0;
    if (n_items) {
        CUDA_TRY(W.it_lo.ensure((size_t)n_items + 2)); CUDA_TRY(W.it_cnt.ensure((size_t)n_items + 2));
        CUDA_TRY(W.it_bytes.ensure((size_t)n_items + 2)); CUDA_TRY(W.it_doc.ensure((size_t)n_items + 2));
        CUDA_TRY(W.cbase.ensure((size_t)n_items + 2)); CUDA_TRY(W.tbase.ensure((size_t)n_items + 2));
        CUDA_TRY(W.part.ensure((size_t)(n_items / SCAN_ITEMS) + 4));
        unstable_search_kernel<<<(unsigned)((nd * 32 + 255) / 256), 256, 0, st>>>(U, a1.d_text, a1.d_doc_off, nd, S.w_ulen.p,
                                                                                 W.item_base.p, W.it_lo.p, W.it_cnt.p, W.it_bytes.p,
                                                                                 W.it_doc.p, W.d_uc);
        uscan(W, W.it_cnt.p, n_items, W.cbase.p, st);
        uscan(W, W.it_bytes.p, n_items, W.tbase.p, st);
        CUDA_TRY(cudaMemcpyAsync(W.h_uc, W.d_uc, sizeof(UnstCounters), cudaMemcpyDeviceToHost, st));
        CUDA_TRY(cudaMemcpyAsync(&W.h_uc->tot[0], W.cbase.p + n_items, 8, cudaMemcpyDeviceToHost, st));
        CUDA_TRY(cudaStreamSynchronize(st));
        if (W.h_uc->err & UERR_BIG) return fail(B200BPE_EINVAL, "the completion candidates of one document need 4 GiB of text or more");
        n_cand = W.h_uc->tot[0];
        stats[0] += W.h_uc->n_docs;
    }
    if (n_cand >= 0xFFFFFFF0ull) return fail(B200BPE_EINVAL, "too many completion candidates in one chunk (2^32)");
    UnstItems I;
    I.doc_off = a1.d_doc_off; I.ulen = S.w_ulen.p; I.item_base = W.item_base.p; I.lo = W.it_lo.p; I.cnt = W.it_cnt.p;
    I.doc = W.it_doc.p; I.cbase = W.cbase.p; I.tbase = W.tbase.p; I.n_items = n_items;
    const uint64_t cap = h->chunk_bytes, max_n = std::max<uint64_t>(cap / 32, 4096);
    CUDA_TRY(W.grp.ensure((size_t)nd + 2)); CUDA_TRY(W.grp_off.ensure((size_t)nd + 2));
    uint64_t n_comp = 0, n_tok = 0, rounds = 0, enc = 0, bpe = 0;
    for (int attempt = 0;; attempt++) {
        uint32_t slots = 4096;
        while (slots < std::min<uint64_t>(2 * n_cand, 1u << 24)) slots <<= 1;
        slots = std::max(slots, W.tslots_min);
        CUDA_TRY(W.tkey.ensure(slots)); CUDA_TRY(W.tidx.ensure(slots)); CUDA_TRY(W.tloc.ensure(slots));
        CUDA_TRY(cudaMemsetAsync(W.tkey.p, 0, (size_t)slots * 8, st));
        CUDA_TRY(cudaMemsetAsync(W.tidx.p, 0xFF, (size_t)slots * 4, st));
        CUDA_TRY(cudaMemsetAsync(W.grp.p, 0, ((size_t)nd + 2) * 4, st));
        UnstTable T{W.tkey.p, W.tidx.p, W.tloc.p, slots - 1};
        const unsigned long long seed = 0x9E3779B97F4A7C15ull * (unsigned long long)(attempt + 1);
        n_comp = n_tok = rounds = enc = bpe = 0;
        uint32_t err = 0;
        for (uint64_t c0 = 0; c0 < n_cand && !err;) {
            CUDA_TRY(cudaMemsetAsync(W.d_uc, 0, sizeof(UnstCounters), st));
            unstable_round_kernel<<<1, 32, 0, st>>>(U, I, n_cand, c0, max_n, cap, W.d_uc);
            CUDA_TRY(cudaMemcpyAsync(&W.h_uc->round, &W.d_uc->round, sizeof(W.h_uc->round), cudaMemcpyDeviceToHost, st));
            CUDA_TRY(cudaStreamSynchronize(st));
            const uint64_t c1 = W.h_uc->round[0], nr = c1 - c0;
            CUDA_TRY(W.cinfo.ensure((size_t)nr + 2)); CUDA_TRY(W.o_len.ensure((size_t)nr + 2)); CUDA_TRY(W.s_len.ensure(2 * (size_t)nr + 2));
            CUDA_TRY(W.o_off.ensure((size_t)nr + 2)); CUDA_TRY(W.s_off.ensure(2 * (size_t)nr + 2));
            CUDA_TRY(W.tokoff_o.ensure((size_t)nr + 2)); CUDA_TRY(W.tokoff_s.ensure(2 * (size_t)nr + 2));
            CUDA_TRY(W.nkeep.ensure((size_t)nr + 2)); CUDA_TRY(W.slot.ensure((size_t)nr + 2)); CUDA_TRY(W.keep.ensure((size_t)nr + 2));
            CUDA_TRY(W.kc.ensure((size_t)nr + 2)); CUDA_TRY(W.rcb.ensure((size_t)nr + 2)); CUDA_TRY(W.rtb.ensure((size_t)nr + 2));
            CUDA_TRY(W.part.ensure((size_t)(2 * nr / SCAN_ITEMS) + 4));
            const unsigned grid = (unsigned)((nr + 255) / 256);
            unstable_meta_kernel<<<grid, 256, 0, st>>>(U, I, a1.d_text, c0, nr, W.cinfo.p, W.o_len.p, W.s_len.p, W.d_uc);
            uscan(W, W.o_len.p, nr, W.o_off.p, st);
            uscan(W, W.s_len.p, 2 * nr, W.s_off.p, st);
            CUDA_TRY(cudaMemcpyAsync(&W.h_uc->tot[0], W.o_off.p + nr, 8, cudaMemcpyDeviceToHost, st));
            CUDA_TRY(cudaMemcpyAsync(&W.h_uc->tot[1], W.s_off.p + 2 * nr, 8, cudaMemcpyDeviceToHost, st));
            CUDA_TRY(cudaStreamSynchronize(st));
            const uint64_t ob = W.h_uc->tot[0], sb = W.h_uc->tot[1];
            if (ob) {
                CUDA_TRY(W.text_o.ensure((size_t)ob + 64)); CUDA_TRY(W.out_o.ensure((size_t)ob + 64));
                unstable_gather_kernel<<<(unsigned)((ob + 16 * 256 - 1) / (16 * 256)), 256, 0, st>>>(
                    U, a1.d_text, a1.d_doc_off, S.w_ulen.p, W.cinfo.p, nr, 1, W.o_off.p, W.text_o.p);
                PipeArgs a2;
                a2.d_text = W.text_o.p; a2.n_bytes = ob; a2.d_doc_off = W.o_off.p; a2.n_docs = nr;
                a2.d_out = W.out_o.p; a2.d_tok_off = W.tokoff_o.p; a2.st = st;
                int rc = run_again(h, D, S, a2, cls, memo, grown, reruns);
                if (rc) return rc;
            } else CUDA_TRY(cudaMemsetAsync(W.tokoff_o.p, 0, ((size_t)nr + 1) * 8, st));
            if (sb) {
                CUDA_TRY(W.text_s.ensure((size_t)sb + 64)); CUDA_TRY(W.out_s.ensure((size_t)sb + 64));
                unstable_gather_kernel<<<(unsigned)((sb + 16 * 256 - 1) / (16 * 256)), 256, 0, st>>>(
                    U, a1.d_text, a1.d_doc_off, S.w_ulen.p, W.cinfo.p, nr, 2, W.s_off.p, W.text_s.p);
                PipeArgs a3;
                a3.d_text = W.text_s.p; a3.n_bytes = sb; a3.d_doc_off = W.s_off.p; a3.n_docs = 2 * nr;
                a3.d_out = W.out_s.p; a3.d_tok_off = W.tokoff_s.p; a3.st = st; a3.single_piece = true;
                int rc = run_again(h, D, S, a3, cls, memo, grown, reruns);
                if (rc) return rc;
            } else CUDA_TRY(cudaMemsetAsync(W.tokoff_s.p, 0, (2 * (size_t)nr + 1) * 8, st));
            RunOut R{W.out_o.p, W.tokoff_o.p, W.out_s.p, W.tokoff_s.p};
            UnstResult res{W.res_tok.p, W.res_off.p, W.res_doc.p, W.grp.p};
            CUDA_TRY(cudaMemsetAsync(S.d_bctr, 0, sizeof(Counters), st));
            unstable_insert_kernel<<<grid, 256, 0, st>>>(U, R, W.cinfo.p, S.w_ulen.p, c0, nr, seed, T, W.nkeep.p, W.slot.p, W.d_uc, S.d_bctr);
            unstable_verify_kernel<<<grid, 256, 0, st>>>(U, R, W.cinfo.p, c0, nr, T, res, W.nkeep.p, W.slot.p, W.keep.p, W.kc.p, W.d_uc);
            uscan(W, W.keep.p, nr, W.rcb.p, st);
            uscan(W, W.kc.p, nr, W.rtb.p, st);
            CUDA_TRY(cudaMemcpyAsync(W.h_uc, W.d_uc, sizeof(UnstCounters), cudaMemcpyDeviceToHost, st));
            CUDA_TRY(cudaMemcpyAsync(&W.h_uc->tot[0], W.rcb.p + nr, 8, cudaMemcpyDeviceToHost, st));
            CUDA_TRY(cudaMemcpyAsync(&W.h_uc->tot[1], W.rtb.p + nr, 8, cudaMemcpyDeviceToHost, st));
            CUDA_TRY(cudaMemcpyAsync(S.h_ctr, S.d_bctr, sizeof(Counters), cudaMemcpyDeviceToHost, st));
            CUDA_TRY(cudaStreamSynchronize(st));
            CUDA_TRY(cudaGetLastError());
            if (S.h_ctr->err & ERR_NOBYTE)
                return fail(B200BPE_ENOBYTE, "a piece needs a single-byte token that mergeable_ranks does not contain");
            err = W.h_uc->err;
            if (err) break;
            enc += W.h_uc->n_encoded; bpe += W.h_uc->n_bpe;
            const uint64_t kept = W.h_uc->tot[0], toks = W.h_uc->tot[1];
            CUDA_TRY(grow_keep(W.res_tok, (size_t)n_tok, (size_t)(n_tok + toks) + 1, st));
            CUDA_TRY(grow_keep(W.res_off, (size_t)(n_comp ? n_comp + 1 : 0), (size_t)(n_comp + kept) + 2, st));
            CUDA_TRY(grow_keep(W.res_doc, (size_t)n_comp, (size_t)(n_comp + kept) + 1, st));
            res = UnstResult{W.res_tok.p, W.res_off.p, W.res_doc.p, W.grp.p};
            unstable_write_kernel<<<grid, 256, 0, st>>>(U, R, W.cinfo.p, nr, T, res, W.keep.p, W.kc.p, W.slot.p, W.rcb.p, W.rtb.p,
                                                        n_comp, n_tok);
            n_comp += kept; n_tok += toks; rounds++;
            c0 = c1;
        }
        if (!err) break;
        if (attempt >= 3) return fail(B200BPE_ECUDA, "completion deduplication did not converge");
        if (err & UERR_TABLE) W.tslots_min = slots * 4;
        (*reruns)++;
    }
    CUDA_TRY(grow_keep(W.res_off, (size_t)(n_comp ? n_comp + 1 : 0), (size_t)n_comp + 2, st));
    W.h_uc->tot[2] = n_tok;
    CUDA_TRY(cudaMemcpyAsync(W.res_off.p + n_comp, &W.h_uc->tot[2], 8, cudaMemcpyHostToDevice, st));
    uscan(W, W.grp.p, nd, W.grp_off.p, st);
    out.tok.resize((size_t)n_tok); out.off.resize((size_t)n_comp + 1);
    if (n_tok) CUDA_TRY(cudaMemcpyAsync(out.tok.data(), W.res_tok.p, (size_t)n_tok * 4, cudaMemcpyDeviceToHost, st));
    CUDA_TRY(cudaMemcpyAsync(out.off.data(), W.res_off.p, ((size_t)n_comp + 1) * 8, cudaMemcpyDeviceToHost, st));
    CUDA_TRY(cudaMemcpyAsync(out.grp.data(), W.grp_off.p, ((size_t)nd + 1) * 8, cudaMemcpyDeviceToHost, st));
    CUDA_TRY(cudaStreamSynchronize(st));
    CUDA_TRY(cudaGetLastError());
    stats[1] += enc; stats[2] += bpe; stats[3] += rounds; stats[4] += n_comp;
    memcpy(S.last_ms, ms1, sizeof(ms1));
    S.last_launches = launches1;
    return B200BPE_OK;
}

struct HostJob {
    b200bpe *h = nullptr;
    const uint8_t *text = nullptr; const uint64_t *doc_off = nullptr; uint64_t n_docs = 0;
    bool single_piece = false, pageable = false, bytes = false, unstable = false;
    const uint8_t *sp_flags = nullptr;
    std::vector<uint64_t> cut;
    std::vector<std::atomic<long long>> count;
    b200bpe_result *r = nullptr; size_t tok_cap = 0;
    std::atomic<int> error{0}; std::atomic<bool> overflow{false};
    std::string error_msg; std::mutex err_mu;
    int special_idx = -1; uint64_t special_pos = 0;
    float sum_ms[9] = {0, 0, 0, 0, 0, 0, 0, 0, 0}; uint32_t launches = 0; std::mutex stat_mu;
    uint32_t grown = 0, reruns = 0;
    uint64_t cls[N_CLS] = {};
    uint64_t bytes_repairs = 0;
    std::vector<UChunk> uch;
    uint64_t ustats[5] = {};
    uint64_t memo[3] = {};

    void set_error(int rc) {
        std::lock_guard<std::mutex> lk(err_mu);
        if (!error.load()) { error_msg = g_last_error; error.store(rc); }
    }
};

static void host_worker(HostJob *J, int dev_index, size_t first, size_t step) {
    b200bpe *h = J->h;
    DevCtx *D = h->devs[dev_index];
    const size_t n_chunks = J->cut.size() - 1;
    std::vector<size_t> mine;
    for (size_t c = first; c < n_chunks; c += step) mine.push_back(c);
    auto bail = [&](int rc) {
        if (rc) J->set_error(rc);
        for (size_t k = 0; k < mine.size(); k++) { long long m1 = -1; J->count[mine[k]].compare_exchange_strong(m1, 0); }
        for (int i = 0; i < DevCtx::N_SLOTS; i++) { cudaStreamSynchronize(D->slots[i].up); cudaStreamSynchronize(D->slots[i].stream); }
    };
    if (mine.empty()) return;
    if (cudaSetDevice(D->device) != cudaSuccess) { fail(B200BPE_ECUDA, "cudaSetDevice failed"); return bail(B200BPE_ECUDA); }
    const uint64_t *doc_off = J->doc_off;
    auto slot_of = [&](size_t k) -> Slot & { return D->slots[k % DevCtx::N_SLOTS]; };

    auto enqueue_h2d = [&](size_t k) -> int {
        Slot &S = slot_of(k);
        const size_t c = mine[k];
        const uint64_t lo = J->cut[c], hi = J->cut[c + 1], b0 = doc_off[lo], nb = doc_off[hi] - b0, nd = hi - lo;
        const bool staged = J->pageable && nb;
        cudaStream_t us = staged ? S.up : S.stream;
        if (!staged || S.w_text.cap < (size_t)nb + 64 || S.w_docoff.cap < (size_t)nd + 2 || S.w_tokoff.cap < (size_t)nd + 2 ||
            S.w_out.cap < (size_t)nb + 64)
            CUDA_TRY(cudaStreamSynchronize(S.stream));
        else if (k >= (size_t)DevCtx::N_SLOTS) CUDA_TRY(cudaStreamWaitEvent(S.up, S.ev[4], 0));
        CUDA_TRY(S.w_text.ensure((size_t)nb + 64)); CUDA_TRY(S.w_docoff.ensure((size_t)nd + 2));
        CUDA_TRY(S.w_tokoff.ensure((size_t)nd + 2)); CUDA_TRY(S.w_out.ensure((size_t)nb + 64));
        const uint8_t *src = J->text + b0;
        CUDA_TRY(cudaEventRecord(S.ev[5], us));
        if (staged) {
            CUDA_TRY(cudaStreamSynchronize(S.up));
            if (S.stage.cap < nb) {
                if (S.stage.p) cudaFreeHost(S.stage.p);
                S.stage.p = nullptr; S.stage.cap = 0;
                const size_t want = (size_t)nb + (size_t)(nb / 8) + 4096;
                CUDA_TRY(cudaHostAlloc(&S.stage.p, want, cudaHostAllocPortable));
                S.stage.cap = want;
            }
            uint8_t *stg = (uint8_t *)S.stage.p;
            const size_t group = std::max<size_t>((((size_t)nb / 4) + 4095) & ~(size_t)4095, (size_t)4 << 20);
            for (size_t g0 = 0; g0 < (size_t)nb; g0 += group) {
                const size_t len = std::min(group, (size_t)nb - g0);
                pool_for(h->pool, len, (size_t)1 << 20, [&](size_t lo, size_t hi) { memcpy(stg + g0 + lo, src + g0 + lo, hi - lo); });
                CUDA_TRY(cudaMemcpyAsync(S.w_text.p + g0, stg + g0, len, cudaMemcpyHostToDevice, us));
            }
        } else if (nb) CUDA_TRY(cudaMemcpyAsync(S.w_text.p, src, nb, cudaMemcpyHostToDevice, us));
        CUDA_TRY(cudaMemcpyAsync(S.w_docoff.p, doc_off + lo, (nd + 1) * 8, cudaMemcpyHostToDevice, us));
        if (b0) add_offset_kernel<<<(unsigned)((nd + 1 + 255) / 256), 256, 0, us>>>(S.w_docoff.p, nd + 1, -(long long)b0);
        CUDA_TRY(cudaEventRecord(S.ev[6], us));
        if (staged) CUDA_TRY(cudaStreamWaitEvent(S.stream, S.ev[6], 0));
        return B200BPE_OK;
    };
    auto args_of = [&](size_t k) {
        Slot &S = slot_of(k);
        const size_t c = mine[k];
        const uint64_t lo = J->cut[c], hi = J->cut[c + 1];
        PipeArgs a;
        a.d_text = S.w_text.p; a.n_bytes = doc_off[hi] - doc_off[lo]; a.d_doc_off = S.w_docoff.p; a.n_docs = hi - lo;
        a.d_out = S.w_out.p; a.d_tok_off = S.w_tokoff.p; a.st = S.stream; a.single_piece = J->single_piece; a.sp_flags = J->sp_flags;
        a.bytes = J->bytes; a.unstable = J->unstable;
        return a;
    };
    size_t known = 0; uint64_t known_sum = 0;
    float sum_ms[9] = {0, 0, 0, 0, 0, 0, 0, 0, 0}; uint32_t launches = 0; float last_d2h = 0;
    uint32_t grown = 0, reruns = 0;
    uint64_t cls[N_CLS] = {}, repaired = 0, memo[3] = {}, ustats[5] = {};
    auto drain = [&](size_t k) -> int {
        Slot &S = slot_of(k);
        const size_t c = mine[k];
        const uint64_t lo = J->cut[c], hi = J->cut[c + 1], nd = hi - lo;
        int sidx = -1; uint64_t spos = 0;
        int rc = collect_pipeline(h, S, &sidx, &spos, &grown);
        for (int attempt = 0; rc == B200BPE_RETRY && attempt < 4; attempt++) {
            rc = enqueue_pipeline(h, D, S, args_of(k));
            if (!rc) { reruns++; rc = collect_pipeline(h, S, &sidx, &spos, &grown); }
        }
        if (rc == B200BPE_RETRY) rc = fail(B200BPE_ECUDA, "work-space sizing did not converge");
        if (rc == B200BPE_ESPECIAL) {
            std::lock_guard<std::mutex> lk(J->err_mu);
            const uint64_t gpos = spos + doc_off[lo];
            if (J->special_idx < 0 || gpos < J->special_pos) { J->special_idx = sidx; J->special_pos = gpos; }
        }
        if (rc) return rc;
        float h2d = 0; cudaEventElapsedTime(&h2d, S.ev[5], S.ev[6]);
        uint64_t nt = S.h_ctr->total_tokens;
        for (int i = 0; i < N_CLS; i++) cls[i] += S.h_ctr->n_cls[i];
        add_miss_memo(S, memo);
        if (J->bytes && S.h_bytes->n_docs) {
            repaired += S.h_bytes->n_docs;
            rc = bytes_tail_runs(h, D, S, args_of(k), &nt, cls, memo, &grown, &reruns);
            if (rc) return rc;
        }
        if (J->unstable) {
            rc = unstable_search(h, D, S, args_of(k), J->uch[c], ustats, &nt, cls, memo, &grown, &reruns);
            if (rc) return rc;
        }
        J->count[c].store((long long)nt);
        while (known < c) {
            long long v = J->count[known].load();
            if (v < 0) {
                if (J->error.load() || J->overflow.load()) return B200BPE_OK;
                std::this_thread::yield();
                continue;
            }
            known_sum += (uint64_t)v; known++;
        }
        const uint64_t token_base = known_sum;
        if (token_base + nt > J->tok_cap) { J->overflow.store(true); return B200BPE_OK; }
        if (token_base) add_offset_kernel<<<(unsigned)((nd + 1 + 255) / 256), 256, 0, S.stream>>>(S.w_tokoff.p, nd + 1, (long long)token_base);
        CUDA_TRY(cudaEventRecord(S.ev[5], S.stream));
        CUDA_TRY(cudaMemcpyAsync((uint64_t *)J->r->off.p + lo, S.w_tokoff.p, (nd + 1) * 8, cudaMemcpyDeviceToHost, S.stream));
        if (nt) CUDA_TRY(cudaMemcpyAsync((uint32_t *)J->r->tok.p + token_base, S.w_out.p, nt * 4, cudaMemcpyDeviceToHost, S.stream));
        CUDA_TRY(cudaEventRecord(S.ev[6], S.stream));
        for (int i = 0; i < 5; i++) sum_ms[i] += S.last_ms[i];
        sum_ms[7] += S.last_ms[7]; sum_ms[8] += S.last_ms[8]; sum_ms[5] += h2d; launches += S.last_launches;
        return B200BPE_OK;
    };
    auto stop = [&]() { return J->error.load() != 0 || J->overflow.load(); };
    const size_t AHEAD = (size_t)DevCtx::N_SLOTS - 2;
    int rc = B200BPE_OK;
    for (size_t k = 0; k < AHEAD && k < mine.size(); k++) { rc = enqueue_h2d(k); if (rc) return bail(rc); }
    const size_t lag = J->unstable ? 0 : 1;
    for (size_t k = 0; k < mine.size() && !stop(); k++) {
        if (k + AHEAD < mine.size()) { rc = enqueue_h2d(k + AHEAD); if (rc) return bail(rc); }
        rc = enqueue_pipeline(h, D, slot_of(k), args_of(k));
        if (rc) return bail(rc);
        if (k >= lag) { rc = drain(k - lag); if (rc) return bail(rc); }
    }
    if (lag && !stop()) { rc = drain(mine.size() - 1); if (rc) return bail(rc); }
    bail(0);
    if (!stop()) { Slot &S = slot_of(mine.size() - 1); cudaEventElapsedTime(&last_d2h, S.ev[5], S.ev[6]); }
    std::lock_guard<std::mutex> lk(J->stat_mu);
    for (int i = 0; i < 9; i++) J->sum_ms[i] = std::max(J->sum_ms[i], sum_ms[i]);
    J->sum_ms[6] = std::max(J->sum_ms[6], last_d2h);
    J->launches += launches;
    J->grown |= grown; J->reruns += reruns;
    for (int i = 0; i < N_CLS; i++) J->cls[i] += cls[i];
    J->bytes_repairs += repaired;
    for (int i = 0; i < 5; i++) J->ustats[i] += ustats[i];
    for (int i = 0; i < 3; i++) J->memo[i] += memo[i];
}

static int chunk_plan(const uint64_t *doc_off, uint64_t n_docs, size_t chunk, bool single_piece, std::vector<uint64_t> &cut) {
    const uint64_t n_bytes = doc_off[n_docs];
    cut.assign(1, 0);
    if (!single_piece && n_bytes > chunk + chunk / 2) {
        uint64_t lo = 0;
        while (lo < n_docs) {
            const uint64_t want = doc_off[lo] + chunk;
            uint64_t hi = (uint64_t)(std::upper_bound(doc_off + lo, doc_off + n_docs + 1, want) - doc_off);
            if (hi > 0) hi--;
            if (hi <= lo) hi = lo + 1;
            if (hi > n_docs) hi = n_docs;
            cut.push_back(hi); lo = hi;
        }
    } else cut.push_back(n_docs);
    for (size_t c = 0; c + 1 < cut.size(); c++) {
        const uint64_t cb = doc_off[cut[c + 1]] - doc_off[cut[c]];
        if (doc_off[cut[c + 1]] < doc_off[cut[c]] || cb >= (1ull << 32) - 4096)
            return fail(B200BPE_EINVAL, cb >= (1ull << 32) - 4096 ? "a single document of >= 4 GiB is not supported"
                                                                  : "document offsets must be non-decreasing");
    }
    return B200BPE_OK;
}

static int encode_host(b200bpe *h, const uint8_t *text, const uint64_t *doc_off, uint64_t n_docs, bool single_piece,
                       const uint8_t *sp_flags, b200bpe_result **out, int *special_idx, bool bytes = false,
                       b200bpe_result **completions = nullptr) {
    const uint64_t n_bytes = doc_off[n_docs];
    if (doc_off[0] != 0) return fail(B200BPE_EINVAL, "document offsets must start at 0");
    const int n_dev = (int)h->devs.size();
    if (!h->pool) h->pool = new TaskPool();
    h->pool->ensure(h->copy_threads);
    size_t chunk = h->chunk_bytes;
    if (!h->chunk_forced && n_dev > 1) chunk = std::min<size_t>(64u << 20, std::max<size_t>(8u << 20, (size_t)(n_bytes / (4 * (uint64_t)n_dev))));
    std::vector<uint64_t> cut;
    if (int rc = chunk_plan(doc_off, n_docs, chunk, single_piece, cut)) return rc;
    const size_t n_chunks = cut.size() - 1;
    bool pageable = false;
    if (n_bytes) {
        cudaPointerAttributes at;
        if (cudaPointerGetAttributes(&at, text) != cudaSuccess) { cudaGetLastError(); pageable = true; }
        else pageable = (at.type == cudaMemoryTypeUnregistered);
    }
    for (int pass = 0; pass < 2; pass++) {
        HostJob J;
        J.h = h; J.text = text; J.doc_off = doc_off; J.n_docs = n_docs; J.single_piece = single_piece; J.pageable = pageable;
        J.sp_flags = sp_flags; J.cut = cut; J.bytes = bytes; J.unstable = completions != nullptr;
        if (J.unstable) J.uch.resize(n_chunks);
        J.count = std::vector<std::atomic<long long>>(n_chunks);
        for (auto &c : J.count) c.store(-1);
        b200bpe_result *r = new b200bpe_result();
        r->owner = h; r->n_docs = n_docs;
        r->off = h->take_pinned((size_t)(n_docs + 1) * 8);
        const size_t want_tok = pass == 0 ? (size_t)(n_bytes / 2) + 4096 : (size_t)n_bytes + 4096;
        r->tok = h->take_pinned(want_tok * 4);
        auto cleanup = [&](int rc) { h->give_pinned(r->tok); h->give_pinned(r->off); delete r; return rc; };
        if (!r->off.p || !r->tok.p) return cleanup(fail(B200BPE_ECUDA, "pinned allocation failed"));
        J.r = r; J.tok_cap = r->tok.cap / 4;
        const int workers = (int)std::min<size_t>((size_t)n_dev, n_chunks);
        if (workers <= 1) host_worker(&J, 0, 0, 1);
        else {
            std::vector<std::thread> th;
            for (int d = 0; d < workers; d++) th.emplace_back(host_worker, &J, d, (size_t)d, (size_t)workers);
            for (auto &t : th) t.join();
        }
        h->last_grown |= J.grown; h->last_reruns += J.reruns; h->last_token_passes = (uint32_t)pass + 1;
        if (J.error.load()) {
            g_last_error = J.error_msg;
            if (J.error.load() == B200BPE_ESPECIAL && special_idx) *special_idx = J.special_idx;
            return cleanup(J.error.load());
        }
        if (J.overflow.load()) { cleanup(0); continue; }
        uint64_t total = 0;
        for (auto &c : J.count) total += (uint64_t)std::max<long long>(0, c.load());
        memcpy(h->last_ms, J.sum_ms, sizeof(J.sum_ms)); h->last_launches = J.launches;
        r->n_tokens = total;
        h->set_piece_classes(J.cls);
        h->last_bytes_repairs = J.bytes_repairs;
        h->set_miss_memo(J.memo);
        if (completions) {
            b200bpe_result *r2 = new b200bpe_result();
            r2->owner = h; r2->on_host_vec = true;
            size_t nt = 0, nc = 0;
            for (auto &u : J.uch) { nt += u.tok.size(); nc += u.off.size() - 1; }
            r2->vtok.reserve(nt); r2->voff.reserve(nc + 1); r2->vgrp.reserve((size_t)n_docs + 1);
            r2->vgrp.push_back(0);
            for (auto &u : J.uch) {
                const uint64_t tb = r2->vtok.size(), cb = r2->voff.size();
                r2->vtok.insert(r2->vtok.end(), u.tok.begin(), u.tok.end());
                for (size_t q = 0; q + 1 < u.off.size(); q++) r2->voff.push_back(tb + u.off[q]);
                for (size_t d = 1; d < u.grp.size(); d++) r2->vgrp.push_back(cb + u.grp[d]);
            }
            r2->voff.push_back(r2->vtok.size());
            r2->n_tokens = r2->vtok.size(); r2->n_docs = r2->voff.size() - 1;
            for (int i = 0; i < 5; i++) h->last_unstable[i] = J.ustats[i];
            h->live_results++;
            *completions = r2;
        }
        h->live_results++;
        *out = r;
        return B200BPE_OK;
    }
    return fail(B200BPE_ECUDA, "token buffer sizing did not converge");
}

extern "C" int b200bpe_encode_ordinary_batch(b200bpe_t *h, const uint8_t *text, const uint64_t *doc_off,
                                             uint64_t n_docs, b200bpe_result_t **out) {
    if (h) h->reset_reruns();
    if (!h || !doc_off || !out) return fail(B200BPE_EINVAL, "null argument");
    if (doc_off[n_docs] && !text) return fail(B200BPE_EINVAL, "null text");
    std::lock_guard<std::mutex> lk(h->mu);
    DeviceGuard guard;
    return encode_host(h, text, doc_off, n_docs, false, nullptr, out, nullptr);
}

extern "C" int b200bpe_encode_bytes_batch(b200bpe_t *h, const uint8_t *text, const uint64_t *doc_off, uint64_t n_docs,
                                          b200bpe_result_t **out) {
    if (h) h->reset_reruns();
    if (!h || !doc_off || !out) return fail(B200BPE_EINVAL, "null argument");
    if (doc_off[n_docs] && !text) return fail(B200BPE_EINVAL, "null text");
    if (!h->decode_on_device)
        return fail(B200BPE_EINVAL, "bytes mode reads token lengths from the device decode tables: every token id must be < 2^24");
    std::lock_guard<std::mutex> lk(h->mu);
    DeviceGuard guard;
    return encode_host(h, text, doc_off, n_docs, false, nullptr, out, nullptr, true);
}

extern "C" int b200bpe_encode_single_piece(b200bpe_t *h, const uint8_t *piece, uint64_t len, b200bpe_result_t **out) {
    if (h) h->reset_reruns();
    if (!h || !out || (len && !piece)) return fail(B200BPE_EINVAL, "null argument");
    std::lock_guard<std::mutex> lk(h->mu);
    DeviceGuard guard;
    uint64_t off[2] = {0, len};
    return encode_host(h, piece, off, 1, true, nullptr, out, nullptr);
}

extern "C" int b200bpe_encode_batch_special(b200bpe_t *h, const uint8_t *text, const uint64_t *doc_off, uint64_t n_docs,
                                            const uint8_t *flags, b200bpe_result_t **out, int32_t *special_index) {
    if (h) h->reset_reruns();
    if (!h || !doc_off || !out) return fail(B200BPE_EINVAL, "null argument");
    if (doc_off[n_docs] && !text) return fail(B200BPE_EINVAL, "null text");
    bool any = false;
    if (flags) for (size_t i = 0; i < h->specials.size(); i++) any |= flags[i] != 0;
    std::lock_guard<std::mutex> lk(h->mu);
    DeviceGuard guard;
    int sidx = -1;
    int rc = encode_host(h, text, doc_off, n_docs, false, any ? flags : nullptr, out, &sidx);
    if (rc == B200BPE_ESPECIAL && special_index) *special_index = sidx;
    return rc;
}

extern "C" int b200bpe_encode_batch(b200bpe_t *h, const uint8_t *text, const uint64_t *doc_off, uint64_t n_docs,
                                    const uint8_t *allowed, b200bpe_result_t **out) {
    if (!h) return fail(B200BPE_EINVAL, "null argument");
    h->reset_reruns();
    std::vector<uint8_t> flags(h->specials.size() + 1, 0);
    if (allowed) for (size_t i = 0; i < h->specials.size(); i++) flags[i] = allowed[i] ? 1 : 0;
    return b200bpe_encode_batch_special(h, text, doc_off, n_docs, allowed ? flags.data() : nullptr, out, nullptr);
// ... 97 lines not shown
        r->owner = h; r->n_docs = n_docs;
        uint64_t total = 0;
        for (uint64_t i = 0; i < n; i++) {
            const std::string *s = decode_one(h, tokens[i]);
            if (!s) { if (bad_token) *bad_token = tokens[i]; return fail(B200BPE_EKEY, "Invalid token for decoding: " + std::to_string(tokens[i])); }
            total += s->size();
        }
        r->off = h->take_pinned((size_t)(n_docs + 1) * 8);
        r->tok = h->take_pinned((size_t)total + 16);
        if (!r->off.p || !r->tok.p) return fail(B200BPE_ECUDA, "pinned allocation failed");
        uint8_t *dst = (uint8_t *)r->tok.p; uint64_t k = 0;
        for (uint64_t d = 0; d < n_docs; d++) {
            ((uint64_t *)r->off.p)[d] = k;
            for (uint64_t i = tok_off[d]; i < tok_off[d + 1]; i++) { const std::string *s = decode_one(h, tokens[i]); memcpy(dst + k, s->data(), s->size()); k += s->size(); }
        }
        ((uint64_t *)r->off.p)[n_docs] = k;
        r->n_tokens = k; rg.keep = true; h->live_results++;
        memset(h->last_ms, 0, sizeof(h->last_ms)); h->last_launches = 0;
        *out = r;
        return B200BPE_OK;
    }
    DevCtx *D = h->devs[0];
    CUDA_TRY(cudaSetDevice(D->device));
    Slot &S = D->slots[0];
    cudaStream_t st = S.stream;
    CUDA_TRY(S.w_out.ensure((size_t)n + 4)); CUDA_TRY(S.w_sub_count.ensure((size_t)n + 4));
    CUDA_TRY(S.w_sub_base.ensure((size_t)n + 4)); CUDA_TRY(S.w_scan_part.ensure((size_t)(n / SCAN_ITEMS) + 4));
    CUDA_TRY(S.w_docoff.ensure((size_t)n_docs + 2)); CUDA_TRY(S.w_tokoff.ensure((size_t)n_docs + 2));
    CUDA_TRY(cudaMemsetAsync(S.d_ctr, 0, sizeof(Counters), st));
    CUDA_TRY(cudaMemsetAsync(&S.d_ctr->ticket, 0xFF, sizeof(unsigned int), st));
    CUDA_TRY(cudaEventRecord(S.ev[0], st));
    if (n) CUDA_TRY(cudaMemcpyAsync(S.w_out.p, tokens, n * 4, cudaMemcpyHostToDevice, st));
    CUDA_TRY(cudaMemcpyAsync(S.w_docoff.p, tok_off, (n_docs + 1) * 8, cudaMemcpyHostToDevice, st));
    CUDA_TRY(cudaEventRecord(S.ev[1], st));
    const long long nn = (long long)n;
    const long long nb = (nn + SCAN_ITEMS - 1) / SCAN_ITEMS;
    if (n) decode_len_kernel<<<(unsigned)((n + 255) / 256), 256, 0, st>>>(S.w_out.p, n, D->d_tok_boff, h->n_ids, S.w_sub_count.p, S.d_ctr);
    if (nb) scan_partial_kernel<<<(unsigned)nb, 256, 0, st>>>(S.w_sub_count.p, nn, S.w_scan_part.p);
    scan_top_kernel<<<1, 1024, 0, st>>>(S.w_scan_part.p, nb, S.d_ctr);
    if (nb) scan_final_kernel<<<(unsigned)nb, 256, 0, st>>>(S.w_sub_count.p, nn, S.w_scan_part.p, S.w_sub_base.p, S.d_ctr);
    else CUDA_TRY(cudaMemsetAsync(S.w_sub_base.p, 0, 8, st));
    CUDA_TRY(cudaMemcpyAsync(S.h_ctr, S.d_ctr, sizeof(Counters), cudaMemcpyDeviceToHost, st));
    CUDA_TRY(cudaStreamSynchronize(st));
    if (S.h_ctr->err & ERR_BADTOKEN) {
        const uint32_t t = tokens[S.h_ctr->ticket];
        if (bad_token) *bad_token = t;
        return fail(B200BPE_EKEY, "Invalid token for decoding: " + std::to_string(t));
    }
    const uint64_t n_out = S.h_ctr->total_tokens;
    CUDA_TRY(S.w_text.ensure((size_t)n_out + 64));
    if (n) decode_copy_kernel<<<(unsigned)((n + 255) / 256), 256, 0, st>>>(S.w_out.p, n, D->d_tok_boff, h->n_ids, D->d_tok_blob,
                                                                        S.w_sub_base.p, S.w_text.p);
    decode_doc_off_kernel<<<(unsigned)((n_docs + 1 + 255) / 256), 256, 0, st>>>(S.w_docoff.p, n_docs, S.w_sub_base.p, S.w_tokoff.p);
    CUDA_TRY(cudaEventRecord(S.ev[2], st));
    b200bpe_result *r = new b200bpe_result();
    rg.r = r;
    r->owner = h; r->n_docs = n_docs; r->n_tokens = n_out;
    r->off = h->take_pinned((size_t)(n_docs + 1) * 8);
    r->tok = h->take_pinned((size_t)n_out + 16);
    if (!r->off.p || !r->tok.p) return fail(B200BPE_ECUDA, "pinned allocation failed");
    CUDA_TRY(cudaMemcpyAsync(r->off.p, S.w_tokoff.p, (n_docs + 1) * 8, cudaMemcpyDeviceToHost, st));
    if (n_out) CUDA_TRY(cudaMemcpyAsync(r->tok.p, S.w_text.p, n_out, cudaMemcpyDeviceToHost, st));
    CUDA_TRY(cudaEventRecord(S.ev[3], st));
    CUDA_TRY(cudaStreamSynchronize(st));
    CUDA_TRY(cudaGetLastError());
    memset(h->last_ms, 0, sizeof(h->last_ms));
    cudaEventElapsedTime(&h->last_ms[5], S.ev[0], S.ev[1]);
    cudaEventElapsedTime(&h->last_ms[4], S.ev[1], S.ev[2]);
    cudaEventElapsedTime(&h->last_ms[6], S.ev[2], S.ev[3]);
    h->last_launches = 6;
    rg.keep = true;
    h->live_results++;
    *out = r;
    return B200BPE_OK;
}

extern "C" int b200bpe_last_timings(b200bpe_t *h, float *ms9, uint32_t *n_launches) {
    if (!h) return fail(B200BPE_EINVAL, "null handle");
    if (ms9) memcpy(ms9, h->last_ms, sizeof(h->last_ms));
    if (n_launches) *n_launches = h->last_launches;
    return B200BPE_OK;
}

extern "C" int b200bpe_last_reruns(b200bpe_t *h, uint32_t *grown, uint32_t *reruns, uint32_t *token_passes) {
    if (!h) return fail(B200BPE_EINVAL, "null handle");
    if (grown) *grown = h->last_grown.load();
    if (reruns) *reruns = h->last_reruns.load();
    if (token_passes) *token_passes = h->last_token_passes.load();
    return B200BPE_OK;
}

extern "C" int b200bpe_last_piece_classes(b200bpe_t *h, uint64_t *counts8, int *lane_per_piece) {
    if (!h) return fail(B200BPE_EINVAL, "null handle");
    if (counts8) for (int c = 0; c < N_CLS; c++) counts8[c] = h->last_cls[c].load();
    if (lane_per_piece) *lane_per_piece = h->last_lane_per_piece.load();
    return B200BPE_OK;
}

extern "C" int b200bpe_last_miss_memo(b200bpe_t *h, uint64_t *misses, uint64_t *merged, uint64_t *unplaced) {
    if (!h) return fail(B200BPE_EINVAL, "null handle");
    if (misses) *misses = h->last_memo[0].load();
    if (merged) *merged = h->last_memo[1].load();
    if (unplaced) *unplaced = h->last_memo[2].load();
    return B200BPE_OK;
}

extern "C" int b200bpe_last_bytes_repairs(b200bpe_t *h, uint64_t *n_docs_repaired) {
    if (!h) return fail(B200BPE_EINVAL, "null handle");
    if (n_docs_repaired) *n_docs_repaired = h->last_bytes_repairs.load();
    return B200BPE_OK;
}

extern "C" int b200bpe_last_unstable(b200bpe_t *h, uint64_t *stats5) {
    if (!h || !stats5) return fail(B200BPE_EINVAL, "null argument");
    for (int i = 0; i < 5; i++) stats5[i] = h->last_unstable[i].load();
    return B200BPE_OK;
}

extern "C" int b200bpe_table_bytes(b200bpe_t *h, uint64_t *bytes4) {
    if (!h || !bytes4) return fail(B200BPE_EINVAL, "null argument");
    memcpy(bytes4, h->table_bytes, sizeof(h->table_bytes));
    return B200BPE_OK;
}

namespace {

struct TrainRun {
    DevBuf<uint8_t> all, ct, uc;
    DevBuf<unsigned long long> doff, npieces, wkey, wcnt, wfirst, wused, part, tbase, dfirst, dcnt, woff;
    DevBuf<unsigned long long> pkey, pcnt, th, tpw, tlen;
    DevBuf<uint32_t> dbits, sfd, pbits, psum, slow, wlen, fbits, tcnt, dlen, wl1, sym, pocc, tslot, stamp, aff, merges;
    Counters *ctr = nullptr, *h_ctr = nullptr; TrainState *st = nullptr, *h_st = nullptr;
    unsigned long long *h_u64 = nullptr;
    cudaStream_t s = nullptr;
    cudaEvent_t ev[4] = {nullptr, nullptr, nullptr, nullptr};
    cudaGraphExec_t exec = nullptr; cudaGraph_t graph = nullptr;
    ~TrainRun() {
        DevBuf<uint8_t> *b8[] = {&all, &ct, &uc};
        for (auto *b : b8) b->release();
        DevBuf<unsigned long long> *b64[] = {&doff, &npieces, &wkey, &wcnt, &wfirst, &wused, &part, &tbase, &dfirst, &dcnt, &woff,
                                             &pkey, &pcnt, &th, &tpw, &tlen};
        for (auto *b : b64) b->release();
        DevBuf<uint32_t> *b32[] = {&dbits, &sfd, &pbits, &psum, &slow, &wlen, &fbits, &tcnt, &dlen, &wl1, &sym, &pocc, &tslot,
                                   &stamp, &aff, &merges};
        for (auto *b : b32) b->release();
        if (ctr) cudaFree(ctr);
        if (st) cudaFree(st);
        if (h_ctr) cudaFreeHost(h_ctr);
        if (h_st) cudaFreeHost(h_st);
        if (h_u64) cudaFreeHost(h_u64);
        if (exec) cudaGraphExecDestroy(exec);
        if (graph) cudaGraphDestroy(graph);
        for (auto &e : ev) if (e) cudaEventDestroy(e);
        if (s) cudaStreamDestroy(s);
    }
};

uint64_t train_pow2(uint64_t x) { uint64_t p = 1; while (p < x) p <<= 1; return p; }

float event_ms(cudaEvent_t a, cudaEvent_t b) { float ms = 0.f; if (cudaEventElapsedTime(&ms, a, b) != cudaSuccess) { cudaGetLastError(); ms = 0.f; } return ms; }

}

static int train_words_reserve(TrainRun &T, TrainWords &W, uint64_t need) {
    const uint64_t want = train_pow2(std::max<uint64_t>(2 * need, 1u << 16));
    if (W.key && W.mask + 1 >= want) return B200BPE_OK;
    TrainRun O;
    std::swap(O.wkey, T.wkey); std::swap(O.wcnt, T.wcnt); std::swap(O.wfirst, T.wfirst); std::swap(O.wlen, T.wlen);
    const uint64_t n_old = W.key ? W.mask + 1 : 0;
    CUDA_TRY(T.wkey.ensure(want)); CUDA_TRY(T.wcnt.ensure(want)); CUDA_TRY(T.wfirst.ensure(want)); CUDA_TRY(T.wlen.ensure(want));
    CUDA_TRY(cudaMemsetAsync(T.wkey.p, 0, want * 8, T.s)); CUDA_TRY(cudaMemsetAsync(T.wcnt.p, 0, want * 8, T.s));
    CUDA_TRY(cudaMemsetAsync(T.wfirst.p, 0xFF, want * 8, T.s));
    TrainWords N{T.wkey.p, T.wcnt.p, T.wfirst.p, T.wlen.p, want - 1, T.wused.p};
    if (n_old) {
        CUDA_TRY(cudaMemsetAsync(T.wused.p, 0, 8, T.s));
        TrainWords Wo{O.wkey.p, O.wcnt.p, O.wfirst.p, O.wlen.p, W.mask, W.n_used};
        train_rehash_kernel<<<1024, 256, 0, T.s>>>(Wo, n_old, N);
        CUDA_TRY(cudaStreamSynchronize(T.s));
    }
    W = N;
    return B200BPE_OK;
}

extern "C" int b200bpe_bpe_train(const uint8_t *text, const uint64_t *doc_off, uint64_t n_docs, const char *pat_str,
                                 uint32_t vocab_size, int device, uint32_t *merges_out, uint64_t merges_cap,
                                 uint64_t *n_merges_out, double *stats8) {
    if (stats8) for (int i = 0; i < 8; i++) stats8[i] = 0.0;
    if (n_merges_out) *n_merges_out = 0;
    if (!doc_off || !pat_str || !n_merges_out || (merges_cap && !merges_out)) return fail(B200BPE_EINVAL, "null argument");
    int pattern;
    if (strcmp(pat_str, R50K_PAT) == 0) pattern = PAT_R50K;
    else if (strcmp(pat_str, CL100K_PAT) == 0) pattern = PAT_CL100K;
    else if (strcmp(pat_str, O200K_PAT) == 0) pattern = PAT_O200K;
    else return fail(B200BPE_EPATTERN, "unsupported pat_str: the GPU pre-tokeniser implements exactly the r50k/p50k, cl100k and "
                                       "o200k patterns of tiktoken_ext/openai_public.py");
    if (vocab_size < 256) return fail(B200BPE_EINVAL, "vocab_size must be at least 256, so we can encode all bytes");
    if (doc_off[0] != 0) return fail(B200BPE_EINVAL, "document offsets must start at 0");
    const uint64_t N = doc_off[n_docs];
    if (N && !text) return fail(B200BPE_EINVAL, "null text");
    size_t chunk = env_chunk_bytes();
    if (!chunk) chunk = 64u << 20;
    std::vector<uint64_t> cut;
    if (int rc = chunk_plan(doc_off, n_docs, chunk, false, cut)) return rc;
    const uint32_t target = vocab_size;
    if (target == 256) return B200BPE_OK;
    if (merges_cap > 0xFFFFFFF0ull) merges_cap = 0xFFFFFFF0ull;
    int ndev = 0;
    if (cudaGetDeviceCount(&ndev) != cudaSuccess || ndev == 0) { cudaGetLastError(); return fail(B200BPE_ECUDA, "no CUDA device: libb200bpe has no CPU fallback"); }
    if (device < 0 || device >= ndev) return fail(B200BPE_EINVAL, "bad device index");
    DeviceGuard guard;
    CUDA_TRY(cudaSetDevice(device));
    int n_sm = 0;
    CUDA_TRY(cudaDeviceGetAttribute(&n_sm, cudaDevAttrMultiProcessorCount, device));
    TrainRun T;
    CUDA_TRY(cudaStreamCreateWithFlags(&T.s, cudaStreamNonBlocking));
    for (auto &e : T.ev) CUDA_TRY(cudaEventCreate(&e));
    CUDA_TRY(cudaMalloc((void **)&T.ctr, sizeof(Counters))); CUDA_TRY(cudaMalloc((void **)&T.st, sizeof(TrainState)));
    CUDA_TRY(cudaHostAlloc((void **)&T.h_ctr, sizeof(Counters), cudaHostAllocPortable));
    CUDA_TRY(cudaHostAlloc((void **)&T.h_st, sizeof(TrainState), cudaHostAllocPortable));
    CUDA_TRY(cudaHostAlloc((void **)&T.h_u64, 4 * 8, cudaHostAllocPortable));
    cudaStream_t s = T.s;
    UcTables uc;
    {
        uint8_t ascii[128];
        uc_ascii_table(ascii);
        const size_t o2 = (sizeof(UC_STAGE1) + 255) & ~(size_t)255, o3 = o2 + ((sizeof(UC_STAGE2) + 255) & ~(size_t)255);
        CUDA_TRY(T.uc.ensure(o3 + 128));
        CUDA_TRY(cudaMemcpy(T.uc.p, UC_STAGE1, sizeof(UC_STAGE1), cudaMemcpyHostToDevice));
        CUDA_TRY(cudaMemcpy(T.uc.p + o2, UC_STAGE2, sizeof(UC_STAGE2), cudaMemcpyHostToDevice));
        CUDA_TRY(cudaMemcpy(T.uc.p + o3, ascii, 128, cudaMemcpyHostToDevice));
        uc.stage1 = (const uint16_t *)T.uc.p; uc.stage2 = T.uc.p + o2; uc.ascii = T.uc.p + o3; uc.one = 1u;
    }
    CUDA_TRY(T.all.ensure(N + 64));
    if (N) CUDA_TRY(cudaMemcpy(T.all.p, text, N, cudaMemcpyHostToDevice));
    CUDA_TRY(T.fbits.ensure((N + 1 + 1023) / 1024 * 32 + 64));
    CUDA_TRY(cudaMemsetAsync(T.fbits.p, 0, T.fbits.cap * 4, s));
    CUDA_TRY(cudaMemsetAsync(T.st, 0, sizeof(TrainState), s));
    CUDA_TRY(T.npieces.ensure(1)); CUDA_TRY(T.wused.ensure(1));
    CUDA_TRY(cudaMemsetAsync(T.wused.p, 0, 8, s));
    TrainWords W{}; W.n_used = T.wused.p;
    if (int rc = train_words_reserve(T, W, 1u << 15)) return rc;
    double ms_split = 0, ms_words = 0, ms_loop = 0;
    uint64_t n_pieces = 0;
    for (size_t c = 0; c + 1 < cut.size(); c++) {
        const uint64_t lo = cut[c], hi = cut[c + 1], base = doc_off[lo], n = doc_off[hi] - base, nd = hi - lo;
        if (n == 0) continue;
        const long long n_words = (long long)((n + 1 + 31) / 32);
        std::vector<unsigned long long> rel(nd + 1);
        for (uint64_t d = 0; d <= nd; d++) rel[d] = doc_off[lo + d] - base;
        CUDA_TRY(T.doff.ensure(nd + 1)); CUDA_TRY(T.ct.ensure(n + 64));
        CUDA_TRY(T.dbits.ensure((size_t)n_words + 8)); CUDA_TRY(T.sfd.ensure((size_t)n_words + 4));
        CUDA_TRY(T.pbits.ensure((size_t)n_words + 8)); CUDA_TRY(T.psum.ensure((size_t)(n_words >> 5) + 4));
        CUDA_TRY(T.slow.ensure(n + 64));
        CUDA_TRY(cudaMemcpyAsync(T.doff.p, rel.data(), (nd + 1) * 8, cudaMemcpyHostToDevice, s));
        CUDA_TRY(cudaMemcpyAsync(T.ct.p, T.all.p + base, n, cudaMemcpyDeviceToDevice, s));
        CUDA_TRY(cudaMemsetAsync(T.ct.p + n, 0, 64, s));
        CUDA_TRY(cudaMemsetAsync(T.ctr, 0, sizeof(Counters), s));
        CUDA_TRY(cudaMemsetAsync(T.dbits.p, 0, ((size_t)n_words + 8) * 4, s));
        CUDA_TRY(cudaMemsetAsync(T.sfd.p, 0xFF, ((size_t)n_words + 4) * 4, s));
        CUDA_TRY(cudaMemsetAsync(T.pbits.p + n_words, 0, 8 * 4, s));
        CUDA_TRY(cudaMemsetAsync(T.npieces.p, 0, 8, s));
        CUDA_TRY(cudaEventRecord(T.ev[0], s));
        mark_docs_kernel<<<(unsigned)((nd + 1 + 255) / 256), 256, 0, s>>>(T.doff.p, nd, n, T.dbits.p, T.sfd.p, nullptr, T.ctr);
        const unsigned grid = (unsigned)((n_words + 255) / 256);
        const uint32_t scap = (uint32_t)std::min<uint64_t>(n + 64, 0xFFFFFFF0u);
#define B2_TRAIN_PRETOK(P)                                                                                                  \
    pretok_kernel<P><<<grid, 256, 0, s>>>(T.ct.p, (long long)n, T.dbits.p, uc, T.pbits.p, T.psum.p, n_words, nullptr,     \
                                          T.slow.p, scap, T.ctr);                                                         \
    pretok_slow_kernel<P><<<n_sm * 8, 256, 0, s>>>(T.ct.p, (long long)n, T.dbits.p, uc, T.pbits.p, T.psum.p, T.slow.p, scap, T.ctr)
        if (pattern == PAT_R50K) { B2_TRAIN_PRETOK(PAT_R50K); }
        else if (pattern == PAT_CL100K) { B2_TRAIN_PRETOK(PAT_CL100K); }
        else { B2_TRAIN_PRETOK(PAT_O200K); }
#undef B2_TRAIN_PRETOK
        CUDA_TRY(cudaEventRecord(T.ev[1], s));
        train_count_kernel<<<grid, 256, 0, s>>>(T.pbits.p, (long long)n, n_words, T.npieces.p);
        CUDA_TRY(cudaMemcpyAsync(T.h_ctr, T.ctr, sizeof(Counters), cudaMemcpyDeviceToHost, s));
        CUDA_TRY(cudaMemcpyAsync(T.h_u64, T.npieces.p, 8, cudaMemcpyDeviceToHost, s));
        CUDA_TRY(cudaMemcpyAsync(T.h_u64 + 1, T.wused.p, 8, cudaMemcpyDeviceToHost, s));
        CUDA_TRY(cudaStreamSynchronize(s));
        if (T.h_ctr->err & ERR_DOCOFF) return fail(B200BPE_EINVAL, "malformed document offsets");
        if (T.h_ctr->err) return fail(B200BPE_ECUDA, "pre-tokeniser error flags " + std::to_string(T.h_ctr->err));
        n_pieces += T.h_u64[0];
        ms_split += event_ms(T.ev[0], T.ev[1]);
        if (int rc = train_words_reserve(T, W, T.h_u64[0] + T.h_u64[1])) return rc;
        CUDA_TRY(cudaEventRecord(T.ev[2], s));
        train_insert_kernel<<<grid, 256, 0, s>>>(T.ct.p, (long long)n, T.pbits.p, n_words, base, W);
        train_verify_kernel<<<grid, 256, 0, s>>>(T.ct.p, (long long)n, T.pbits.p, n_words, base, W, T.all.p, T.fbits.p, T.st);
        CUDA_TRY(cudaEventRecord(T.ev[3], s));
        CUDA_TRY(cudaStreamSynchronize(s));
        ms_words += event_ms(T.ev[2], T.ev[3]);
    }
    CUDA_TRY(cudaGetLastError());
    CUDA_TRY(cudaEventRecord(T.ev[2], s));
    const long long n_tiles = (long long)((N + 1 + 1023) / 1024);
    CUDA_TRY(T.tcnt.ensure((size_t)n_tiles + 4)); CUDA_TRY(T.tbase.ensure((size_t)n_tiles + 4));
    CUDA_TRY(T.part.ensure((size_t)(n_tiles / SCAN_ITEMS) + 4));
    CUDA_TRY(cudaMemsetAsync(T.ctr, 0, sizeof(Counters), s));
    train_tile_count_kernel<<<(unsigned)((n_tiles + 255) / 256), 256, 0, s>>>(T.fbits.p, n_tiles, T.tcnt.p);
    {
        const long long nb = (n_tiles + SCAN_ITEMS - 1) / SCAN_ITEMS;
        scan_partial_kernel<<<(unsigned)nb, 256, 0, s>>>(T.tcnt.p, n_tiles, T.part.p);
        scan_top_kernel<<<1, 1024, 0, s>>>(T.part.p, nb, T.ctr);
        scan_final_kernel<<<(unsigned)nb, 256, 0, s>>>(T.tcnt.p, n_tiles, T.part.p, T.tbase.p, T.ctr);
    }
    CUDA_TRY(cudaMemcpyAsync(T.h_ctr, T.ctr, sizeof(Counters), cudaMemcpyDeviceToHost, s));
    CUDA_TRY(cudaMemcpyAsync(T.h_u64 + 1, T.wused.p, 8, cudaMemcpyDeviceToHost, s));
    CUDA_TRY(cudaStreamSynchronize(s));
    const uint64_t D = T.h_ctr->total_tokens;
    if (D != T.h_u64[1]) return fail(B200BPE_ECUDA, "internal: distinct words and first occurrences disagree");
    if (D >= 0xFFFFFFF0ull) return fail(B200BPE_EINVAL, "too many distinct words (>= 2^32)");
    CUDA_TRY(T.dfirst.ensure(D + 2)); CUDA_TRY(T.dlen.ensure(D + 2)); CUDA_TRY(T.dcnt.ensure(D + 2)); CUDA_TRY(T.wl1.ensure(D + 2));
    CUDA_TRY(T.woff.ensure(D + 2));
    train_compact_kernel<<<n_sm * 8, 256, 0, s>>>(W, T.fbits.p, T.tbase.p, T.dfirst.p, T.dlen.p, T.dcnt.p, T.wl1.p, D, T.st);
    {
        const long long nb = ((long long)D + SCAN_ITEMS - 1) / SCAN_ITEMS;
        CUDA_TRY(T.part.ensure((size_t)nb + 4));
        CUDA_TRY(cudaMemsetAsync(T.ctr, 0, sizeof(Counters), s));
        if (nb) {
            scan_partial_kernel<<<(unsigned)nb, 256, 0, s>>>(T.wl1.p, (long long)D, T.part.p);
            scan_top_kernel<<<1, 1024, 0, s>>>(T.part.p, nb, T.ctr);
            scan_final_kernel<<<(unsigned)nb, 256, 0, s>>>(T.wl1.p, (long long)D, T.part.p, T.woff.p, T.ctr);
        } else CUDA_TRY(cudaMemsetAsync(T.woff.p, 0, 8, s));
    }
    CUDA_TRY(cudaMemcpyAsync(T.h_ctr, T.ctr, sizeof(Counters), cudaMemcpyDeviceToHost, s));
    CUDA_TRY(cudaMemcpyAsync(T.h_st, T.st, sizeof(TrainState), cudaMemcpyDeviceToHost, s));
    CUDA_TRY(cudaStreamSynchronize(s));
    if (T.h_st->err) return fail(B200BPE_ECUDA, T.h_st->err & 1u ? "internal: two different pieces share a 64-bit hash"
                                                                 : "internal: word index out of range");
    const uint64_t S = T.h_ctr->total_tokens;
    CUDA_TRY(T.sym.ensure(S + 4));
    if (D) train_fill_kernel<<<n_sm * 8, 256, 0, s>>>(T.all.p, T.dfirst.p, T.dlen.p, T.woff.p, D, T.sym.p);
    CUDA_TRY(cudaStreamSynchronize(s));
    T.all.release(); T.ct.release(); T.slow.release(); T.pbits.release(); T.dbits.release(); T.sfd.release();
    T.wkey.release(); T.wcnt.release(); T.wfirst.release(); T.wlen.release();
    const uint64_t P0 = S - 2 * D;
    const uint64_t pcap = train_pow2(std::max<uint64_t>(6 * P0 + 1024, 1u << 12));
    if (pcap > (1ull << 32)) return fail(B200BPE_EINVAL, "corpus too large for one training call (pair table >= 2^32 slots)");
    CUDA_TRY(T.pkey.ensure(pcap)); CUDA_TRY(T.pcnt.ensure(pcap)); CUDA_TRY(T.pocc.ensure(pcap));
    CUDA_TRY(cudaMemsetAsync(T.pkey.p, 0xFF, pcap * 8, s)); CUDA_TRY(cudaMemsetAsync(T.pcnt.p, 0, pcap * 8, s));
    TrainPairs P{T.pkey.p, T.pcnt.p, T.pocc.p, pcap - 1};
    const uint64_t tcap = train_pow2(2ull * target + 1024);
    CUDA_TRY(T.th.ensure(target + 2)); CUDA_TRY(T.tpw.ensure(target + 2)); CUDA_TRY(T.tlen.ensure(target + 2));
    CUDA_TRY(T.tslot.ensure(tcap));
    CUDA_TRY(cudaMemsetAsync(T.tslot.p, 0xFF, tcap * 4, s));
    TrainTok TT{T.th.p, T.tpw.p, T.tlen.p, T.tslot.p, tcap - 1};
    train_tok_init_kernel<<<1, 32, 0, s>>>(TT);
    CUDA_TRY(T.stamp.ensure(D + 2)); CUDA_TRY(T.aff.ensure(D + 2)); CUDA_TRY(T.merges.ensure(3 * merges_cap + 3));
    CUDA_TRY(cudaMemsetAsync(T.stamp.p, 0, (D + 2) * 4, s));
    {
        TrainState init; memset(&init, 0, sizeof(init));
        init.best = ~0ull; init.n_ids = 256;
        *T.h_st = init;
// ... 52 lines not shown
```

tiktoken_b200/csrc/dev_common.cuh:

```cuda
#pragma once
#include <cuda_runtime.h>
#include <stdint.h>

#include "bpe_tables.h"
#include "text_access.cuh"

namespace b2bpe {

static const uint32_t ERR_NOBYTE = 1u;
static const uint32_t ERR_DOCOFF = 2u;
static const uint32_t ERR_BADTOKEN = 4u;
static const uint32_t ERR_LONGCAP = 8u;
static const uint32_t ERR_MISSCAP = 16u;
static const uint32_t ERR_SLOWCAP = 64u;
static const uint32_t ERR_INTERNAL = 128u;
static const uint32_t ERR_SPECIAL = 32u;

struct UcTables {
    const uint16_t *stage1; const uint8_t *stage2; const uint8_t *ascii;
    uint32_t one;
};

static const int N_CLS = 8;
static const int CLS_G1024 = 4, CLS_WARP = 5, CLS_BLOCK = 6, CLS_CLUSTER = 7;

struct Counters {
    unsigned long long long_bytes;
    unsigned long long miss_bytes;
    unsigned long long total_tokens;
    unsigned long long special_pos;
    unsigned int n_long;
    unsigned int n_cls[10];
    unsigned int cls_head[10];
    unsigned int n_big;
    unsigned int n_miss;
    unsigned int n_cut;
    unsigned int n_doc_tiles;
    unsigned int n_slow;
    unsigned int special_idx;
    unsigned int ticket;
    unsigned int err;
    unsigned int n_owner;
    unsigned int n_unplaced;
};

static const uint32_t GROUP_MAX = 1024;
static const uint32_t BLOCK_MIN = 4096;
static const uint32_t CLUSTER_MIN = 32768;
static const uint32_t LONG_SCRATCH_MIN = 256;

struct LongQ {
    unsigned long long *start;
    unsigned int *len;
    unsigned long long *off;
    unsigned int *ntok;
    unsigned int *cls[N_CLS];
    unsigned long long scratch_cap;
    uint32_t *sub_count;
};

__device__ __forceinline__ void long_piece_done(const LongQ &q, unsigned int qi, uint32_t nt) {
    q.ntok[qi] = nt;
    atomicAdd(q.sub_count + (q.start[qi] >> 10), nt);
}

struct LongScratch {
    uint32_t *idA, *rkA, *idB, *rkB, *aux1, *aux2;
    uint8_t *flag;
};

struct SmemCol32 {
    uint32_t *base;
    __device__ __forceinline__ uint32_t &operator[](int j) const { return base[j * 32]; }
};

__device__ __forceinline__ uint32_t warp_min_u32(uint32_t v) {
    return __reduce_min_sync(0xFFFFFFFFu, v);
}
__device__ __forceinline__ uint32_t warp_sum_u32(uint32_t v) {
    return __reduce_add_sync(0xFFFFFFFFu, v);
}
__device__ __forceinline__ uint32_t warp_incl_scan_u32(uint32_t v, int lane) {
#pragma unroll
    for (int o = 1; o < 32; o <<= 1) { const uint32_t y = __shfl_up_sync(0xFFFFFFFFu, v, o); if (lane >= o) v += y; }
    return v;
}

__device__ __forceinline__ uint4 ld_stream_u4(const void *p) {
    uint4 v;
    asm("ld.global.nc.L1::no_allocate.v4.u32 {%0,%1,%2,%3}, [%4];" : "=r"(v.x), "=r"(v.y), "=r"(v.z), "=r"(v.w) : "l"(p));
    return v;
}
__device__ __forceinline__ uint32_t ld_stream_u32(const void *p) {
    uint32_t v;
    asm("ld.global.nc.L1::no_allocate.u32 %0, [%1];" : "=r"(v) : "l"(p));
    return v;
}
__device__ __forceinline__ U4 ld_stream_U4(const U4 *p) {
    const uint4 v = ld_stream_u4(p);
    U4 r; r.x = v.x; r.y = v.y; r.z = v.z; r.w = v.w; return r;
}
__device__ __forceinline__ void st_stream_u32(uint32_t *p, uint32_t v) { __stcs(p, v); }
__device__ __forceinline__ void st_stream_u4(uint4 *p, uint4 v) { __stcs(p, v); }

__device__ __forceinline__ uint4 u4_of(unsigned long long lo, unsigned long long hi) {
    return make_uint4((uint32_t)lo, (uint32_t)(lo >> 32), (uint32_t)hi, (uint32_t)(hi >> 32));
}
__device__ __forceinline__ uint4 ld_relaxed_b128(const uint4 *p) {
    unsigned long long lo, hi;
    asm volatile("{\n\t.reg .b128 t;\n\tld.relaxed.gpu.global.b128 t, [%2];\n\tmov.b128 {%0, %1}, t;\n\t}"
                 : "=l"(lo), "=l"(hi) : "l"(p) : "memory");
    return u4_of(lo, hi);
}
__device__ __forceinline__ uint4 cas_zero_b128(uint4 *p, uint4 v) {
    unsigned long long lo, hi;
    const unsigned long long vlo = (unsigned long long)v.y << 32 | v.x, vhi = (unsigned long long)v.w << 32 | v.z, z = 0;
    asm volatile("{\n\t.reg .b128 c, v, r;\n\tmov.b128 c, {%2, %2};\n\tmov.b128 v, {%3, %4};\n\t"
                 "atom.relaxed.gpu.global.cas.b128 r, [%5], c, v;\n\tmov.b128 {%0, %1}, r;\n\t}"
                 : "=l"(lo), "=l"(hi) : "l"(z), "l"(vlo), "l"(vhi), "l"(p) : "memory");
    return u4_of(lo, hi);
}

__device__ __forceinline__ uint32_t smem_u32(const void *p) { return (uint32_t)__cvta_generic_to_shared(p); }
__device__ __forceinline__ void mbar_init(uint32_t mbar, uint32_t count) {
    asm volatile("mbarrier.init.shared::cta.b64 [%0], %1;" ::"r"(mbar), "r"(count) : "memory");
}
// ... 29 lines not shown
```

tiktoken_b200/csrc/kernels_encode.cuh:

```cuda
#pragma once
#include "dev_common.cuh"

using namespace b2bpe;

static const uint32_t PT_MISS = 0x40000000u, PT_LONG = 0x80000000u, PT_KIND = 0xC0000000u, PT_PAYLOAD = 0x3FFFFFFFu;
static const uint32_t PT_EMPTY = 0xFFFFFFFFu;

struct MissQ {
    uint4 *key;
    uint32_t *pos;
    uint32_t *roff;
    uint8_t *len;
    uint4 *rec;
    uint4 *skey;
    uint4 *smeta;
    uint32_t cap;
    unsigned long long mres_cap;
};

struct MissMemo {
    uint4 *key;
    uint32_t *owner;
    uint32_t *slot;
    uint32_t *own;
    uint32_t *block_n;
    uint32_t mask;
    uint32_t limit;
    uint32_t on;
};
static const int MEMO_PROBES = 8;
static const uint32_t MEMO_TRIAL = 256;

struct TileParams {
    const uint8_t *text; long long n_bytes; long long n_words; long long n_sub;
    const uint32_t *pbits; const uint32_t *dbits; const uint32_t *span_first_doc;
    const unsigned long long *doc_off; unsigned long long n_docs;
    LongQ q; const uint32_t *lidx; const uint32_t *ltok;
    const uint32_t *doc_tiles;
    const uint32_t *sbits;
    uint32_t *ptok;
    MissQ mq; uint32_t *mres;
    uint32_t *sub_count;
    unsigned long long *sub_base;
    uint32_t *out; unsigned long long *tok_off;
    unsigned long long *big_dst, *big_src; uint32_t *big_n;
    Counters *ctr;
};

static const int ENC_WARPS = 4;
static const int PROBE_BLOCKS_PER_SM = 12;
static const int SUB_BYTES = 1024;
static const int STAGE_TEXT = SUB_BYTES + 32;
static const int STAGE_PW = 36;

struct ProbeSmem {
    __align__(16) uint8_t text[2][STAGE_TEXT];
    __align__(16) uint32_t p[2][STAGE_PW];
    __align__(8) unsigned long long mbar[2];
    uint32_t nmiss;
    uint16_t plist[SUB_BYTES + 2];
    uint16_t miss[SUB_BYTES / 2];
};

__device__ __forceinline__ void load_key(const uint8_t *txt, int off, int len, uint32_t &a0, uint32_t &a1, uint32_t &a2, uint32_t &a3) {
    const uint32_t *wp = reinterpret_cast<const uint32_t *>(txt) + (off >> 2);
    const int sh = (off & 3) * 8;
    const uint32_t w0 = wp[0], w1 = wp[1], w2 = wp[2], w3 = wp[3], w4 = wp[4];
    const int nb = len * 8;
    a0 = __funnelshift_r(w0, w1, sh) & low_mask_clamped(nb);
    a1 = __funnelshift_r(w1, w2, sh) & low_mask_clamped(nb - 32);
    a2 = __funnelshift_r(w2, w3, sh) & low_mask_clamped(nb - 64);
    a3 = __funnelshift_r(w3, w4, sh) & low_mask_clamped(nb - 96);
}

__global__ void __launch_bounds__(ENC_WARPS * 32) probe_kernel(TileParams p, DevTables T) {
    __shared__ ProbeSmem smem[ENC_WARPS];
    ProbeSmem &S = smem[threadIdx.x >> 5];
    const int lane = threadIdx.x & 31;
    const long long stride = (long long)gridDim.x * ENC_WARPS;
    long long sub = (long long)blockIdx.x * ENC_WARPS + (threadIdx.x >> 5);
    if (sub >= p.n_sub) return;
    const uint32_t mb0 = smem_u32(&S.mbar[0]), s_text0 = smem_u32(S.text[0]), s_pw0 = smem_u32(S.p[0]);
    auto mb = [&](int b) -> uint32_t { return mb0 + (uint32_t)b * (uint32_t)sizeof(S.mbar[0]); };
    const uint64_t pol = l2_policy_evict_first();
    if (lane == 0) { mbar_init(mb(0), 1); mbar_init(mb(1), 1); mbar_fence_init(); }
    __syncwarp();
    auto stage = [&](long long t, int b) {
        const long long left = p.n_bytes - t * SUB_BYTES;
        const uint32_t tbytes = left >= STAGE_TEXT ? (uint32_t)STAGE_TEXT : (uint32_t)((left + 15) & ~15ll);
        mbar_arrive_expect_tx(mb(b), tbytes + STAGE_PW * 4);
        if (tbytes) tma_load_1d(s_text0 + (uint32_t)b * (uint32_t)sizeof(S.text[0]), p.text + t * SUB_BYTES, tbytes, mb(b), pol);
        tma_load_1d(s_pw0 + (uint32_t)b * (uint32_t)sizeof(S.p[0]), p.pbits + t * 32, STAGE_PW * 4, mb(b), pol);
    };
    if (lane == 0) stage(sub, 0);
    int cur = 0; uint32_t phase = 0;
    for (; sub < p.n_sub; sub += stride, cur ^= 1) {
        if (lane == 0 && sub + stride < p.n_sub) stage(sub + stride, cur ^ 1);
        mbar_wait(mb(cur), (phase >> cur) & 1u);
        phase ^= 1u << cur;
        const uint8_t *txt = S.text[cur];
        const uint32_t *pw = S.p[cur];
        const long long sub_byte = sub * SUB_BYTES;
        uint32_t *const slot = p.ptok + sub * SUB_BYTES;
        if (lane == 0) S.nmiss = 0;

        uint32_t pv = pw[lane];
        {
            const long long span0 = sub_byte + lane * 32;
            if (span0 + 32 > p.n_bytes) {
                const long long keep = p.n_bytes - span0;
                pv = keep <= 0 ? 0u : (pv & ((1u << keep) - 1u));
            }
        }
        uint32_t np;
        {
            const uint32_t c = __popc(pv);
            const uint32_t inc = warp_incl_scan_u32(c, lane);
            np = __shfl_sync(0xFFFFFFFFu, inc, 31);
            uint16_t *dst = S.plist + (inc - c);
            for (uint32_t m = pv; m;) { const int j = __ffs(m) - 1; m &= m - 1; *dst++ = (uint16_t)(lane * 32 + j); }
            if (lane == 0) {
                const uint32_t nx = pw[32];
                const long long tail = p.n_bytes - sub_byte;
                S.plist[np] = (uint16_t)(tail <= SUB_BYTES ? tail : (nx ? SUB_BYTES + __ffs(nx) - 1 : SUB_BYTES + 32));
            }
        }
        __syncwarp();

        uint32_t cnt = 0;
        auto prep = [&](uint32_t i, int &len, uint32_t &a0, uint32_t &a1, uint32_t &a2, uint32_t &a3) -> int {
            if (i >= np) return 0;
            const int off = S.plist[i];
            len = (int)S.plist[i + 1] - off;
            if (p.sbits) {
                const long long pos = sub_byte + off;
                if ((p.sbits[pos >> 5] >> (pos & 31)) & 1u) { st_stream_u32(slot + i, p.ltok[pos]); cnt++; return 0; }
            }
            if (len > SHORT_MAX) {
                const uint32_t qi = p.lidx[(sub_byte + off) >> 4];
                st_stream_u32(slot + i, PT_LONG | qi);
                return 0;
            }
            load_key(txt, off, len, a0, a1, a2, a3);
            return 1;
        };
        auto finish = [&](uint32_t i, int len, uint32_t a0, uint32_t a1, uint32_t a2, uint32_t a3, uint32_t s, U4 e0, U4 e1) {
            const uint32_t r = piece_finish(T, a0, a1, a2, a3, (uint32_t)len, s, e0, e1);
            if (r != RANK_MAX) { st_stream_u32(slot + i, r); cnt++; }
            else S.miss[atomicAdd(&S.nmiss, 1u)] = (uint16_t)i;
        };
        for (uint32_t i = lane; i < np; i += 64) {
            int lenA = 0, lenB = 0;
            uint32_t a0 = 0, a1 = 0, a2 = 0, a3 = 0, b0 = 0, b1 = 0, b2 = 0, b3 = 0;
            const int needA = prep(i, lenA, a0, a1, a2, a3);
            const int needB = prep(i + 32, lenB, b0, b1, b2, b3);
            uint32_t sA = 0, sB = 0;
            U4 eA0 = {0, 0, 0, 0}, eA1 = {0, 0, 0, 0}, eB0 = {0, 0, 0, 0}, eB1 = {0, 0, 0, 0};
            if (needA) sA = piece_issue(T, a0, a1, a2, a3, (uint32_t)lenA, eA0, eA1);
            if (needB) sB = piece_issue(T, b0, b1, b2, b3, (uint32_t)lenB, eB0, eB1);
            if (needA) finish(i, lenA, a0, a1, a2, a3, sA, eA0, eA1);
            if (needB) finish(i + 32, lenB, b0, b1, b2, b3, sB, eB0, eB1);
        }
        __syncwarp();

        const uint32_t nmiss = S.nmiss;
        if (nmiss) {
            uint32_t run = 0;
            for (uint32_t k0 = 0; k0 < nmiss; k0 += 32) {
                const uint32_t k = k0 + lane;
                uint32_t len = 0;
                if (k < nmiss) { const uint32_t i = S.miss[k]; len = (uint32_t)S.plist[i + 1] - S.plist[i]; }
                run += warp_sum_u32(len);
            }
            uint32_t qbase = 0; unsigned long long rbase = 0;
            if (lane == 0) {
                qbase = atomicAdd(&p.ctr->n_miss, nmiss);
                rbase = atomicAdd(&p.ctr->miss_bytes, (unsigned long long)run);
            }
            qbase = __shfl_sync(0xFFFFFFFFu, qbase, 0); rbase = __shfl_sync(0xFFFFFFFFu, rbase, 0);
            const bool fits = (unsigned long long)qbase + nmiss <= p.mq.cap && rbase + run <= p.mq.mres_cap;
// ... 363 lines not shown
```

tiktoken_b200/csrc/kernels_long.cuh:

```cuda
#pragma once
#include <cooperative_groups.h>

#include "dev_common.cuh"

using namespace b2bpe;
namespace cg = cooperative_groups;

__global__ void __launch_bounds__(256) find_long_kernel(const uint32_t *__restrict__ pbits,
                                                        const uint32_t *__restrict__ psum, long long n_bytes,
                                                        long long n_words, LongQ q, uint32_t *lidx,
                                                        const uint32_t *__restrict__ sbits, Counters *ctr) {
    long long w = blockIdx.x * (long long)blockDim.x + threadIdx.x;
    if (w >= n_words) return;
    const uint32_t pw = pbits[w];
    if (pw == 0) return;
    uint32_t cand;
    {
        const uint64_t x = ((uint64_t)pbits[w + 1] << 32) | pw;
        uint64_t z = ~x;
        z &= z >> 1; z &= z >> 2; z &= z >> 4; z &= z >> 8;
        cand = pw & (uint32_t)(z >> 1);
        if (sbits) cand &= ~sbits[w];
    }
    for (uint32_t mm = cand; mm;) {
        const int j = __ffs(mm) - 1; mm &= mm - 1;
        const long long s = w * 32 + j;
        if (s >= n_bytes) break;
        const uint32_t m = (j == 31) ? 0u : (pw & ~((2u << j) - 1u));
        long long nxt;
        if (m) nxt = w * 32 + (__ffs(m) - 1);
        else {
            long long w2 = w + 1;
            uint32_t x = pbits[w2];
            if (x == 0) {
                uint32_t sm = ((w2 & 31) == 31) ? 0u : (psum[w2 >> 5] & ~((2u << (w2 & 31)) - 1u));
                long long grp = w2 >> 5;
                while (sm == 0) { grp++; sm = psum[grp]; }
                w2 = grp * 32 + (__ffs(sm) - 1);
                x = pbits[w2];
            }
            nxt = w2 * 32 + (__ffs(x) - 1);
        }
        const long long len = nxt - s;
        if (len > SHORT_MAX) {
            const uint32_t peers = __activemask();
            unsigned int i = 0;
            if ((threadIdx.x & 31) == __ffs(peers) - 1) i = atomicAdd(&ctr->n_long, (unsigned int)__popc(peers));
            i = __shfl_sync(peers, i, __ffs(peers) - 1) + __popc(peers & ((1u << (threadIdx.x & 31)) - 1u));
            unsigned long long off = 0; bool fits = true;
            if (len > LONG_SCRATCH_MIN) {
                off = atomicAdd(&ctr->long_bytes, (unsigned long long)len);
                if (off + (unsigned long long)len > q.scratch_cap) { fits = false; atomicOr(&ctr->err, ERR_LONGCAP); }
            }
            q.start[i] = (unsigned long long)s; q.len[i] = (unsigned int)len; q.off[i] = off; q.ntok[i] = 0;
            lidx[s >> 4] = i;
            const int c = !fits ? N_CLS : len > CLUSTER_MIN ? CLS_CLUSTER : len > BLOCK_MIN ? CLS_BLOCK : len > GROUP_MAX ? CLS_WARP
                          : len > 256 ? CLS_G1024 : len > 128 ? 3 : len > 64 ? 2 : len > 32 ? 1 : 0;
            const uint32_t same = __match_any_sync(peers, c);
            unsigned int k = 0;
            if ((threadIdx.x & 31) == __ffs(same) - 1) k = atomicAdd(&ctr->n_cls[c], (unsigned int)__popc(same));
            k = __shfl_sync(peers, k, __ffs(same) - 1) + __popc(same & ((1u << (threadIdx.x & 31)) - 1u));
            if (c == N_CLS) continue;
            unsigned int *lst = c == 0 ? q.cls[0] : c == 1 ? q.cls[1] : c == 2 ? q.cls[2] : c == 3 ? q.cls[3] : c == 4 ? q.cls[4]
                                : c == 5 ? q.cls[5] : c == 6 ? q.cls[6] : q.cls[7];
            lst[k] = i;
        }
    }
}

__device__ uint32_t long_piece_warp(const DevTables &T, const uint8_t *__restrict__ piece, uint32_t n,
                                    LongScratch S, uint32_t *__restrict__ out, uint32_t *err) {
    const int lane = threadIdx.x & 31;
    if (n <= T.max_token_len) {
        uint32_t r = RANK_MAX;
        if (lane == 0) {
            if (n <= (uint32_t)SHORT_MAX) {
                uint64_t k0 = 0, k1 = 0;
                for (uint32_t i = 0; i < n; i++) {
                    if (i < 8) k0 |= (uint64_t)piece[i] << (8 * i); else k1 |= (uint64_t)piece[i] << (8 * (i - 8));
                }
                r = piece_lookup16(T, k0, k1, n);
            } else {
                uint64_t h = long_hash_init(n);
                for (uint32_t i = 0; i < n; i += 8) {
                    uint64_t w = 0;
                    for (uint32_t k = 0; k < 8 && i + k < n; k++) w |= (uint64_t)piece[i + k] << (8 * k);
                    h = long_hash_step(h, w, i / 8);
                }
                r = piece_lookup_long(T, h, n, [&](uint32_t i) { return piece[i]; });
            }
        }
        r = __shfl_sync(0xFFFFFFFFu, r, 0);
        if (r != RANK_MAX) { if (lane == 0) out[0] = r; return 1; }
    }
    if (n == 1) {
        uint32_t id = T.byte_id[piece[0]];
        if (lane == 0) { out[0] = id; if (id >= PSEUDO_BASE) atomicOr(err, ERR_NOBYTE); }
        return 1;
    }
    uint32_t *id = S.idA, *rk = S.rkA, *id2 = S.idB, *rk2 = S.rkB;
    for (uint32_t i = lane; i < n; i += 32) {
        uint32_t b = piece[i];
        id[i] = __ldg(T.byte_id + b);
        rk[i] = (i + 1 < n) ? __ldg(T.pair2 + ((b << 8) | piece[i + 1])) : RANK_MAX;
    }
    __syncwarp();
    uint32_t m = n;
    for (;;) {
        uint32_t g = RANK_MAX;
        for (uint32_t i = lane; i < m; i += 32) g = min(g, rk[i]);
        g = warp_min_u32(g);
        if (g == RANK_MAX) break;
        uint32_t carry_par = 0;
        for (uint32_t base = 0; base < m; base += 32) {
            uint32_t i = base + lane;
            bool cand = i < m && rk[i] == g;
            uint32_t c = __ballot_sync(0xFFFFFFFFu, cand);
            uint32_t zeros_below = ~c & ((1u << lane) - 1u);
            uint32_t before;
            if (zeros_below == 0) before = (uint32_t)lane + carry_par;
            else before = (uint32_t)lane - (32u - (uint32_t)__clz((int)zeros_below));
            bool sel = cand && ((before & 1u) == 0);
            if (i < m) S.flag[i] = sel ? 1 : 0;
            if (c == 0xFFFFFFFFu) carry_par = carry_par;
            else carry_par = (uint32_t)__clz((int)~c) & 1u;
        }
        __syncwarp();
        uint32_t vmin = RANK_MAX;
        for (uint32_t i = lane; i < m; i += 32) {
            if (!S.flag[i]) continue;
            uint32_t nl = RANK_MAX, nr = RANK_MAX;
            if (i >= 1 && i + 2 < m) {
                const uint32_t lid = (i >= 2 && S.flag[i - 2]) ? g : id[i - 1];
                pair_lookup2(T, lid, g, g, id[i + 2], nl, nr);
            } else if (i >= 1) {
                nl = pair_lookup(T, (i >= 2 && S.flag[i - 2]) ? g : id[i - 1], g);
            } else if (i + 2 < m) {
                nr = pair_lookup(T, g, id[i + 2]);
            }
            S.aux1[i] = nl; S.aux2[i] = nr;
            if (nl < g || nr < g) vmin = min(vmin, i);
        }
        uint32_t v = warp_min_u32(vmin);
        __syncwarp();
        uint32_t outn = 0;
        for (uint32_t base = 0; base < m; base += 32) {
            uint32_t i = base + lane;
            bool in = i < m;
            bool com = in && S.flag[i] && i <= v;
// ... 472 lines not shown
```

tiktoken_b200/csrc/kernels_pretok.cuh:

```cuda
#pragma once
#include "dev_common.cuh"
#include "pretok_fast.cuh"

using namespace b2bpe;

__global__ void mark_docs_kernel(const unsigned long long *__restrict__ doc_off, unsigned long long n_docs,
                                 unsigned long long n_bytes, uint32_t *dbits, uint32_t *span_first_doc,
                                 uint32_t *doc_tiles , Counters *ctr) {
    unsigned long long d = blockIdx.x * (unsigned long long)blockDim.x + threadIdx.x;
    if (d > n_docs) return;
    unsigned long long pos = doc_off[d];
    bool bad = pos > n_bytes || (d < n_docs && doc_off[d + 1] < pos) || (d == 0 && pos != 0) ||
               (d == n_docs && pos != n_bytes);
    if (bad) { atomicOr(&ctr->err, ERR_DOCOFF); return; }
    atomicOr(&dbits[pos >> 5], 1u << (pos & 31));
    atomicMin(&span_first_doc[pos >> 5], (uint32_t)d);
    if (doc_tiles && (d == 0 || (doc_off[d - 1] >> 10) != (pos >> 10))) {
        const uint32_t peers = __activemask();
        const int lane = threadIdx.x & 31, leader = __ffs(peers) - 1;
        unsigned int base = 0;
        if (lane == leader) base = atomicAdd(&ctr->n_doc_tiles, (unsigned int)__popc(peers));
        base = __shfl_sync(peers, base, leader);
        doc_tiles[base + __popc(peers & ((1u << lane) - 1u))] = (uint32_t)(pos >> 10);
    }
}

static const int PRETOK_WARPS = 8;

__device__ __noinline__ bool slow_boundary_o200k(const TextAccess &t, long long pos) { return boundary_before<PAT_O200K>(t, pos); }

template <int PAT>
__device__ __forceinline__ bool slow_boundary(const TextAccess &t, long long pos) {
    if (PAT == PAT_O200K) return slow_boundary_o200k(t, pos);
    return boundary_before<PAT>(t, pos);
}

template <int PAT, bool CUT = false>
__global__ void __launch_bounds__(PRETOK_WARPS * 32, PAT == PAT_O200K ? 4 : 5) pretok_kernel(const uint8_t *__restrict__ text, long long n_bytes,
                                                                  const uint32_t *__restrict__ dbits, UcTables uc,
                                                                  uint32_t *__restrict__ pbits, uint32_t *__restrict__ psum,
                                                                  long long n_words, const uint32_t *__restrict__ ibits,
                                                                  uint32_t *__restrict__ slow_list, uint32_t slow_cap, Counters *ctr) {
    __shared__ uint32_t s_cnt, s_base;
    const long long w = blockIdx.x * (long long)blockDim.x + threadIdx.x;
    const int lane = threadIdx.x & 31;
    const TextAccess t{text, n_bytes, dbits, uc.stage1, uc.stage2, uc.ascii, uc.one};
    if (threadIdx.x == 0) s_cnt = 0;
    uint64_t b = 0, slow = 0;
    if (w < n_words) b = span_fast<PAT, CUT>(t, w, slow);
    uint32_t sm = (uint32_t)(slow >> 8);
    if (ibits && w < n_words) sm &= ~ibits[w];
    uint32_t word = 0;
    if (w < n_words) {
        word = span_word(t, w, b);
        if (ibits) word &= ~ibits[w];
        pbits[w] = word;
    }
    const uint32_t nz = __ballot_sync(0xFFFFFFFFu, word != 0);
    if (lane == 0 && (w >> 5) <= ((n_words - 1) >> 5)) psum[w >> 5] = nz;
    const uint32_t cnt = (uint32_t)__popc(sm);
    const uint32_t inc = warp_incl_scan_u32(cnt, lane);
    const uint32_t wtot = __shfl_sync(0xFFFFFFFFu, inc, 31);
    __syncthreads();
    uint32_t woff = 0;
    if (lane == 0 && wtot) woff = atomicAdd(&s_cnt, wtot);
    woff = __shfl_sync(0xFFFFFFFFu, woff, 0);
    __syncthreads();
    const uint32_t btot = s_cnt;
    if (btot == 0) return;
    if (threadIdx.x == 0) s_base = atomicAdd(&ctr->n_slow, btot);
    __syncthreads();
    if (cnt) {
        uint32_t o = s_base + woff + inc - cnt;
        if ((unsigned long long)s_base + btot > slow_cap) { atomicOr(&ctr->err, ERR_SLOWCAP); return; }
        for (uint32_t mm = sm; mm; mm &= mm - 1) slow_list[o++] = (uint32_t)(w * 32 + (__ffs(mm) - 1));
    }
}

template <int PAT>
__global__ void __launch_bounds__(256) pretok_slow_kernel(const uint8_t *__restrict__ text, long long n_bytes,
                                                         const uint32_t *__restrict__ dbits, UcTables uc,
                                                         uint32_t *pbits, uint32_t *psum, const uint32_t *__restrict__ slow_list,
                                                         uint32_t slow_cap, const Counters *ctr) {
    if (ctr->err & ERR_SLOWCAP) return;
    const uint32_t n = min(ctr->n_slow, slow_cap);
    const TextAccess t{text, n_bytes, dbits, uc.stage1, uc.stage2, uc.ascii};
    for (uint32_t i = blockIdx.x * 256u + threadIdx.x; i < n; i += gridDim.x * 256u) {
        const uint32_t pos = slow_list[i];
        if (slow_boundary<PAT>(t, (long long)pos)) {
            atomicOr(&pbits[pos >> 5], 1u << (pos & 31));
            atomicOr(&psum[pos >> 10], 1u << ((pos >> 5) & 31));
        }
    }
}

__global__ void single_piece_bits_kernel(uint32_t *pbits, uint32_t *psum, const uint32_t *__restrict__ dbits, long long n_words) {
    long long w = blockIdx.x * (long long)blockDim.x + threadIdx.x;
    uint32_t word = 0;
    if (w < n_words) {
        word = dbits[w];
        pbits[w] = word;
    }
    const uint32_t nz = __ballot_sync(0xFFFFFFFFu, word != 0);
    if ((threadIdx.x & 31) == 0 && (w >> 5) <= ((n_words - 1) >> 5)) psum[w >> 5] = nz;
}
```

Baseline: 159.8.

## Segment pretokenize and probe stages to overlap on a high-priority stream

Splits pretokenization, slow-boundary fixup and long-piece start discovery into tile segments, so the probe kernel for each segment can run on a new high-priority stream while later segments are still being pretokenized. The psum summary moves into a separate pass after all segments finish. find_long is split into a per-segment start-recording pass and a final pass that computes lengths and classes. This aims to hide probe latency behind pretokenization, at the cost of more kernel launches, cross-stream events, a ticket-based slow_done counter, and the risk that segment boundaries (the +4 word overlap) or psum-dependent logic in probe behave differently.

```diff
diff --git a/include/b200bpe.h b/include/b200bpe.h
--- a/include/b200bpe.h
+++ b/include/b200bpe.h
@@ -87,6 +87,8 @@
 
 int b200bpe_last_timings(b200bpe_t *h, float *ms9, uint32_t *n_launches);
 
+int b200bpe_last_segments(b200bpe_t *h, uint32_t *n_segments);
+
 #define B200BPE_GREW_MISS 1u
 #define B200BPE_GREW_SLOW 2u
 #define B200BPE_GREW_LONG 4u
diff --git a/tiktoken_b200/_lib.py b/tiktoken_b200/_lib.py
--- a/tiktoken_b200/_lib.py
+++ b/tiktoken_b200/_lib.py
@@ -97,6 +97,8 @@
     L.b200bpe_decode_batch.argtypes = [vp, vp, vp, u64, C.POINTER(vp), C.POINTER(u32)]
     L.b200bpe_last_timings.restype = i32
     L.b200bpe_last_timings.argtypes = [vp, vp, C.POINTER(u32)]
+    L.b200bpe_last_segments.restype = i32
+    L.b200bpe_last_segments.argtypes = [vp, C.POINTER(u32)]
     L.b200bpe_last_reruns.restype = i32
     L.b200bpe_last_reruns.argtypes = [vp, C.POINTER(u32), C.POINTER(u32), C.POINTER(u32)]
     L.b200bpe_last_piece_classes.restype = i32
@@ -120,6 +122,7 @@
     "b200bpe_decode_bytes", "b200bpe_decode_batch", "b200bpe_last_timings", "b200bpe_table_bytes", "b200bpe_last_error",
     "b200bpe_version", "b200bpe_device_count", "b200bpe_create_multi", "b200bpe_n_devices", "b200bpe_encode_batch_special",
     "b200bpe_special_name", "b200bpe_encode_device_async", "b200bpe_device_wait", "b200bpe_trim", "b200bpe_last_reruns",
+    "b200bpe_last_segments",
     "b200bpe_last_piece_classes", "b200bpe_encode_bytes_batch", "b200bpe_last_bytes_repairs", "b200bpe_last_miss_memo",
     "b200bpe_encode_with_unstable_batch", "b200bpe_result_groups", "b200bpe_last_unstable", "b200bpe_bpe_train",
 ]
diff --git a/tiktoken_b200/_tiktoken.py b/tiktoken_b200/_tiktoken.py
--- a/tiktoken_b200/_tiktoken.py
+++ b/tiktoken_b200/_tiktoken.py
@@ -359,6 +359,9 @@
         keys = ["mark_docs_ms", "pretok_ms", "long_ms", "encode_ms", "device_total_ms", "h2d_ms", "d2h_ms", "gather_ms", "probe_ms"]
         d = {k: float(ms[i]) for i, k in enumerate(keys)}
         d["launches"] = int(n.value)
+        seg = C.c_uint32(0)
+        self._L.b200bpe_last_segments(self._h, C.byref(seg))
+        d["segments"] = int(seg.value)
         return d
 
     def last_reruns(self) -> dict:
diff --git a/tiktoken_b200/csrc/b200bpe.cu b/tiktoken_b200/csrc/b200bpe.cu
--- a/tiktoken_b200/csrc/b200bpe.cu
+++ b/tiktoken_b200/csrc/b200bpe.cu
@@ -148,12 +148,13 @@
     cudaStream_t stream = nullptr;
     cudaStream_t side = nullptr;
     cudaStream_t side2 = nullptr;
+    cudaStream_t hi = nullptr;
     cudaStream_t up = nullptr;
-    static const int N_EV = 15;
+    static const int N_EV = 16;
     cudaEvent_t ev[N_EV];
     PinnedBuf stage;
     float last_ms[9] = {0, 0, 0, 0, 0, 0, 0, 0, 0};
-    uint32_t last_launches = 0;
+    uint32_t last_launches = 0, last_segments = 0;
     bool ok = false;
 
     cudaError_t init() {
@@ -165,6 +166,9 @@
         if (e == cudaSuccess) e = cudaStreamCreateWithFlags(&side, cudaStreamNonBlocking);
         if (e == cudaSuccess) e = cudaStreamCreateWithFlags(&side2, cudaStreamNonBlocking);
         if (e == cudaSuccess) e = cudaStreamCreateWithFlags(&up, cudaStreamNonBlocking);
+        int prio_low = 0, prio_high = 0;
+        if (e == cudaSuccess) e = cudaDeviceGetStreamPriorityRange(&prio_low, &prio_high);
+        if (e == cudaSuccess) e = cudaStreamCreateWithPriority(&hi, cudaStreamNonBlocking, prio_high);
         for (int i = 0; i < N_EV && e == cudaSuccess; i++) e = cudaEventCreate(&ev[i]);
         ok = (e == cudaSuccess);
         return e;
@@ -199,6 +203,7 @@
         if (stream) cudaStreamDestroy(stream);
         if (side) cudaStreamDestroy(side);
         if (side2) cudaStreamDestroy(side2);
+        if (hi) cudaStreamDestroy(hi);
         if (up) cudaStreamDestroy(up);
     }
 };
@@ -278,7 +283,9 @@
         std::vector<uint8_t> u8info; uint32_t max_len = 0;
     } uh;
     std::atomic<uint64_t> last_memo[3] = {};
+    std::atomic<uint32_t> last_segments{0};
     void reset_reruns() {
+        last_segments = 0;
         last_grown = 0; last_reruns = 0; last_token_passes = 0; last_bytes_repairs = 0;
         for (auto &c : last_unstable) c = 0;
         for (auto &c : last_memo) c = 0;
@@ -528,6 +535,8 @@
 };
 
 static const unsigned long long MISS_CAP_MIN = 1u << 16, LONG_CAP_MIN = 1u << 20;
+static const long long SEG_TILES = 64 * 1024;
+static const int PROBE_SEG_BLOCKS = 6;
 
 static int enqueue_pipeline(b200bpe *h, DevCtx *D, Slot &S, const PipeArgs &a) {
     const uint64_t n_bytes = a.n_bytes, n_docs = a.n_docs;
@@ -650,30 +659,67 @@
         launches += 2;
         hbits = S.w_hbits.p; ibits = S.w_ibits.p; sbits = S.w_sbits.p;
     }
+    TileParams p;
+    p.text = a.d_text; p.n_bytes = (long long)n_bytes; p.n_words = n_words; p.n_sub = n_tiles;
+    p.pbits = S.w_pbits.p; p.dbits = S.w_dbits.p; p.span_first_doc = S.w_sfd.p;
+    p.doc_off = a.d_doc_off; p.n_docs = n_docs; p.q = q; p.lidx = S.w_lidx.p; p.ltok = S.w_ltok.p;
+    p.ptok = S.w_ptok.p; p.mres = S.w_mres.p; p.sbits = sbits;
+    p.mq.key = S.w_mq_key.p; p.mq.pos = S.w_mq_pos.p; p.mq.roff = S.w_mq_roff.p; p.mq.len = S.w_mq_len.p; p.mq.rec = S.w_mq_rec.p;
+    p.doc_tiles = S.w_doc_tiles.p;
+    p.mq.skey = S.w_mq_skey.p; p.mq.smeta = S.w_mq_smeta.p; p.mq.cap = (uint32_t)std::min<size_t>(S.miss_cap, 0xFFFFFFF0u);
+    p.mq.mres_cap = S.mres_cap;
+    p.sub_count = S.w_sub_count.p; p.sub_base = S.w_sub_base.p;
+    p.out = a.d_out; p.tok_off = a.d_tok_off; p.ctr = S.d_ctr;
+    p.big_dst = S.w_big_dst.p; p.big_src = S.w_big_src.p; p.big_n = S.w_big_n.p;
     CUDA_TRY(cudaEventRecord(S.ev[1], st));
-    {
-        unsigned grid = (unsigned)((n_words + 255) / 256);
-        if (a.single_piece) single_piece_bits_kernel<<<grid, 256, 0, st>>>(S.w_pbits.p, S.w_psum.p, S.w_dbits.p, n_words);
-        else {
-            const uint32_t scap = (uint32_t)std::min<size_t>(S.slow_cap, 0xFFFFFFF0u);
+    const int n_seg = (int)std::max<long long>(1, n_tiles / SEG_TILES);
+    S.last_segments = (uint32_t)n_seg;
+    if (a.single_piece) {
+        single_piece_bits_kernel<<<(unsigned)((n_words + 255) / 256), 256, 0, st>>>(S.w_pbits.p, S.w_psum.p, S.w_dbits.p, n_words);
+        launches++;
+    }
+    const uint32_t scap = (uint32_t)std::min<size_t>(S.slow_cap, 0xFFFFFFF0u);
+    for (int k = 0; k < n_seg; k++) {
+        const bool last = k == n_seg - 1;
+        const long long t0 = (long long)k * SEG_TILES, t1 = last ? n_tiles : t0 + SEG_TILES;
+        if (!a.single_piece) {
+            const long long w0 = k == 0 ? 0 : 32 * t0 + 4, w1 = last ? n_words : 32 * t1 + 4;
+            const unsigned grid = (unsigned)((w1 - w0 + 255) / 256);
 #define B2_PRETOK(P)                                                                                                                   \
-    if (a.bytes) pretok_kernel<P, true><<<grid, 256, 0, st>>>(a.d_text, (long long)n_bytes, hbits, D->uc, S.w_pbits.p, S.w_psum.p,       \
-                                                             n_words, ibits, S.w_slow.p, scap, S.d_ctr);                              \
-    else pretok_kernel<P><<<grid, 256, 0, st>>>(a.d_text, (long long)n_bytes, hbits, D->uc, S.w_pbits.p, S.w_psum.p, n_words, ibits,          \
-                                          S.w_slow.p, scap, S.d_ctr);                                                                  \
-    pretok_slow_kernel<P><<<D->n_sm * 8, 256, 0, st>>>(a.d_text, (long long)n_bytes, hbits, D->uc, S.w_pbits.p, S.w_psum.p, S.w_slow.p, scap, S.d_ctr)
+    if (a.bytes) pretok_kernel<P, true><<<grid, 256, 0, st>>>(a.d_text, (long long)n_bytes, hbits, D->uc, S.w_pbits.p, w0, w1, ibits,   \
+                                                             S.w_slow.p, scap, S.d_ctr);                                              \
+    else pretok_kernel<P><<<grid, 256, 0, st>>>(a.d_text, (long long)n_bytes, hbits, D->uc, S.w_pbits.p, w0, w1, ibits, S.w_slow.p,     \
+                                              scap, S.d_ctr);                                                                          \
+    pretok_slow_kernel<P><<<D->n_sm * 8, 256, 0, st>>>(a.d_text, (long long)n_bytes, hbits, D->uc, S.w_pbits.p, S.w_slow.p, scap, S.d_ctr)
             if (h->pattern == PAT_R50K) { B2_PRETOK(PAT_R50K); }
             else if (h->pattern == PAT_CL100K) { B2_PRETOK(PAT_CL100K); }
             else { B2_PRETOK(PAT_O200K); }
 #undef B2_PRETOK
+            launches += 2;
+        }
+        {
+            const long long w0 = 32 * t0, w1 = last ? n_words : 32 * t1;
+            find_long_kernel<false><<<(unsigned)((w1 - w0 + 255) / 256), 256, 0, st>>>(S.w_pbits.p, S.w_psum.p, (long long)n_bytes, w0, w1,
+                                                                                    q, S.w_lidx.p, sbits, S.d_ctr);
             launches++;
         }
+        CUDA_TRY(cudaEventRecord(S.ev[15], st));
+        CUDA_TRY(cudaStreamWaitEvent(S.hi, S.ev[15], 0));
+        if (k == 0) CUDA_TRY(cudaEventRecord(S.ev[3], S.hi));
+        const long long want_blocks = (t1 - t0 + ENC_WARPS - 1) / ENC_WARPS;
+        const unsigned probe_grid = (unsigned)std::min<long long>(want_blocks, (long long)D->n_sm * PROBE_SEG_BLOCKS);
+        probe_kernel<<<probe_grid, ENC_WARPS * 32, 0, S.hi>>>(p, D->T, t0, t1);
         launches++;
     }
+    CUDA_TRY(cudaEventRecord(S.ev[8], S.hi));
     CUDA_TRY(cudaEventRecord(S.ev[2], st));
     {
-        unsigned grid = (unsigned)((n_words + 255) / 256);
-        find_long_kernel<<<grid, 256, 0, st>>>(S.w_pbits.p, S.w_psum.p, (long long)n_bytes, n_words, q, S.w_lidx.p, sbits, S.d_ctr);
+        if (!a.single_piece) {
+            psum_kernel<<<(unsigned)((n_words + 255) / 256), 256, 0, st>>>(S.w_pbits.p, S.w_psum.p, n_words);
+            launches++;
+        }
+        find_long_kernel<true><<<(unsigned)((n_words + 255) / 256), 256, 0, st>>>(S.w_pbits.p, S.w_psum.p, (long long)n_bytes, 0, n_words,
+                                                                                q, S.w_lidx.p, sbits, S.d_ctr);
         launches++;
         cudaStream_t ls = S.side, ls2 = S.side2;
         CUDA_TRY(cudaEventRecord(S.ev[10], st));
@@ -697,28 +743,12 @@
         CUDA_TRY(cudaEventRecord(S.ev[12], ls));
         launches += 5;
     }
-    CUDA_TRY(cudaEventRecord(S.ev[3], st));
     {
-        TileParams p;
-        p.text = a.d_text; p.n_bytes = (long long)n_bytes; p.n_words = n_words; p.n_sub = n_tiles;
-        p.pbits = S.w_pbits.p; p.dbits = S.w_dbits.p; p.span_first_doc = S.w_sfd.p;
-        p.doc_off = a.d_doc_off; p.n_docs = n_docs; p.q = q; p.lidx = S.w_lidx.p; p.ltok = S.w_ltok.p;
-        p.ptok = S.w_ptok.p; p.mres = S.w_mres.p; p.sbits = sbits;
-        p.mq.key = S.w_mq_key.p; p.mq.pos = S.w_mq_pos.p; p.mq.roff = S.w_mq_roff.p; p.mq.len = S.w_mq_len.p; p.mq.rec = S.w_mq_rec.p;
-        p.doc_tiles = S.w_doc_tiles.p;
-        p.mq.skey = S.w_mq_skey.p; p.mq.smeta = S.w_mq_smeta.p; p.mq.cap = (uint32_t)std::min<size_t>(S.miss_cap, 0xFFFFFFF0u);
-        p.mq.mres_cap = S.mres_cap;
-        p.sub_count = S.w_sub_count.p; p.sub_base = S.w_sub_base.p;
-        p.out = a.d_out; p.tok_off = a.d_tok_off; p.ctr = S.d_ctr;
-        p.big_dst = S.w_big_dst.p; p.big_src = S.w_big_src.p; p.big_n = S.w_big_n.p;
         MissMemo memo;
         memo.key = S.w_memo_key.p; memo.owner = S.w_memo_owner.p; memo.slot = S.w_mq_slot.p; memo.own = S.w_mq_own.p;
         memo.block_n = S.w_memo_bn.p; memo.mask = memo_slots ? memo_slots - 1 : 0; memo.on = memo_slots ? 1u : 0u;
         memo.limit = std::max<uint32_t>(1u, memo_slots / 2 / (uint32_t)(D->n_sm * SORT_BLOCKS_PER_SM));
-        const long long want_blocks = (n_tiles + ENC_WARPS - 1) / ENC_WARPS;
-        const unsigned probe_grid = (unsigned)std::min<long long>(want_blocks, (long long)D->n_sm * PROBE_BLOCKS_PER_SM);
-        probe_kernel<<<probe_grid, ENC_WARPS * 32, 0, st>>>(p, D->T);
-        CUDA_TRY(cudaEventRecord(S.ev[8], st));
+        CUDA_TRY(cudaStreamWaitEvent(st, S.ev[8], 0));
         const int sort_blocks = D->n_sm * SORT_BLOCKS_PER_SM;
         if (memo_slots) CUDA_TRY(cudaMemsetAsync(S.w_memo_key.p, 0, (size_t)memo_slots * sizeof(uint4), st));
         miss_dedup_kernel<<<sort_blocks, SORT_THREADS, 0, st>>>(p, memo, S.w_sort_hist.p);
@@ -758,7 +788,7 @@
             launches++;
         }
         finalize_kernel<<<1, 32, 0, st>>>(S.d_ctr, S.d_sticky, a.d_counts, n_docs);
-        launches += (sparse_docs ? 12 : 11) + (memo_slots ? 1 : 0);
+        launches += (sparse_docs ? 11 : 10) + (memo_slots ? 1 : 0);
     }
     CUDA_TRY(cudaEventRecord(S.ev[4], st));
     if (a.bytes) CUDA_TRY(cudaMemcpyAsync(S.h_bytes, S.d_bytes, sizeof(BytesCounters), cudaMemcpyDeviceToHost, st));
@@ -889,6 +919,7 @@
     memcpy(h->last_ms, S.last_ms, sizeof(h->last_ms));
     h->last_ms[5] = h->last_ms[6] = 0.f;
     h->last_launches = S.last_launches;
+    h->last_segments = S.last_segments;
     if (rc == B200BPE_RETRY) return fail(B200BPE_ECUDA, "work-space sizing did not converge");
     if (rc) return rc;
     if (c.queued > 1) {
@@ -944,7 +975,7 @@
     const uint64_t n1 = S.h_ctr->total_tokens, drop = S.h_bytes->drop;
     const float ms1[9] = {S.last_ms[0], S.last_ms[1], S.last_ms[2], S.last_ms[3], S.last_ms[4], S.last_ms[5], S.last_ms[6],
                           S.last_ms[7], S.last_ms[8]};
-    const uint32_t launches1 = S.last_launches;
+    const uint32_t launches1 = S.last_launches, segments1 = S.last_segments;
     const uint64_t nd = a1.n_docs, tail = S.h_bytes->tail;
     cudaStream_t st = a1.st;
     CUDA_TRY(S.w_b2doc.ensure((size_t)nd + 2)); CUDA_TRY(S.w_b2off.ensure((size_t)nd + 2)); CUDA_TRY(S.w_bbase.ensure((size_t)nd + 2));
@@ -973,6 +1004,7 @@
     memcpy(S.last_ms, ms1, sizeof(ms1));
     S.last_ms[4] += ms2;
     S.last_launches = launches1 + launches2 + 9;
+    S.last_segments = std::max(segments1, S.last_segments);
     return B200BPE_OK;
 }
 
@@ -1106,7 +1138,7 @@
     cudaStream_t st = a1.st;
     const float ms1[9] = {S.last_ms[0], S.last_ms[1], S.last_ms[2], S.last_ms[3], S.last_ms[4], S.last_ms[5], S.last_ms[6],
                           S.last_ms[7], S.last_ms[8]};
-    const uint32_t launches1 = S.last_launches;
+    const uint32_t launches1 = S.last_launches, segments1 = S.last_segments;
     out.tok.clear(); out.off.assign(1, 0); out.grp.assign((size_t)nd + 1, 0);
     if (nd == 0) return B200BPE_OK;
     const uint64_t n1 = *nt;
@@ -1254,6 +1286,7 @@
     stats[1] += enc; stats[2] += bpe; stats[3] += rounds; stats[4] += n_comp;
     memcpy(S.last_ms, ms1, sizeof(ms1));
     S.last_launches = launches1;
+    S.last_segments = segments1;
     return B200BPE_OK;
 }
 
@@ -1268,7 +1301,7 @@
     std::atomic<int> error{0}; std::atomic<bool> overflow{false};
     std::string error_msg; std::mutex err_mu;
     int special_idx = -1; uint64_t special_pos = 0;
-    float sum_ms[9] = {0, 0, 0, 0, 0, 0, 0, 0, 0}; uint32_t launches = 0; std::mutex stat_mu;
+    float sum_ms[9] = {0, 0, 0, 0, 0, 0, 0, 0, 0}; uint32_t launches = 0, segments = 0; std::mutex stat_mu;
     uint32_t grown = 0, reruns = 0;
     uint64_t cls[N_CLS] = {};
     uint64_t bytes_repairs = 0;
@@ -1346,7 +1379,7 @@
         return a;
     };
     size_t known = 0; uint64_t known_sum = 0;
-    float sum_ms[9] = {0, 0, 0, 0, 0, 0, 0, 0, 0}; uint32_t launches = 0; float last_d2h = 0;
+    float sum_ms[9] = {0, 0, 0, 0, 0, 0, 0, 0, 0}; uint32_t launches = 0, segments = 0; float last_d2h = 0;
     uint32_t grown = 0, reruns = 0;
     uint64_t cls[N_CLS] = {}, repaired = 0, memo[3] = {}, ustats[5] = {};
     auto drain = [&](size_t k) -> int {
@@ -1398,6 +1431,7 @@
         CUDA_TRY(cudaEventRecord(S.ev[6], S.stream));
         for (int i = 0; i < 5; i++) sum_ms[i] += S.last_ms[i];
         sum_ms[7] += S.last_ms[7]; sum_ms[8] += S.last_ms[8]; sum_ms[5] += h2d; launches += S.last_launches;
+        segments = std::max(segments, S.last_segments);
         return B200BPE_OK;
     };
     auto stop = [&]() { return J->error.load() != 0 || J->overflow.load(); };
@@ -1418,6 +1452,7 @@
     for (int i = 0; i < 9; i++) J->sum_ms[i] = std::max(J->sum_ms[i], sum_ms[i]);
     J->sum_ms[6] = std::max(J->sum_ms[6], last_d2h);
     J->launches += launches;
+    J->segments = std::max(J->segments, segments);
     J->grown |= grown; J->reruns += reruns;
     for (int i = 0; i < N_CLS; i++) J->cls[i] += cls[i];
     J->bytes_repairs += repaired;
@@ -1499,6 +1534,7 @@
         uint64_t total = 0;
         for (auto &c : J.count) total += (uint64_t)std::max<long long>(0, c.load());
         memcpy(h->last_ms, J.sum_ms, sizeof(J.sum_ms)); h->last_launches = J.launches;
+        h->last_segments = J.segments;
         r->n_tokens = total;
         h->set_piece_classes(J.cls);
         h->last_bytes_repairs = J.bytes_repairs;
@@ -1762,6 +1798,12 @@
     return B200BPE_OK;
 }
 
+extern "C" int b200bpe_last_segments(b200bpe_t *h, uint32_t *n_segments) {
+    if (!h) return fail(B200BPE_EINVAL, "null handle");
+    if (n_segments) *n_segments = h->last_segments.load();
+    return B200BPE_OK;
+}
+
 extern "C" int b200bpe_last_reruns(b200bpe_t *h, uint32_t *grown, uint32_t *reruns, uint32_t *token_passes) {
     if (!h) return fail(B200BPE_EINVAL, "null handle");
     if (grown) *grown = h->last_grown.load();
@@ -1809,7 +1851,7 @@
     DevBuf<uint8_t> all, ct, uc;
     DevBuf<unsigned long long> doff, npieces, wkey, wcnt, wfirst, wused, part, tbase, dfirst, dcnt, woff;
     DevBuf<unsigned long long> pkey, pcnt, th, tpw, tlen;
-    DevBuf<uint32_t> dbits, sfd, pbits, psum, slow, wlen, fbits, tcnt, dlen, wl1, sym, pocc, tslot, stamp, aff, merges;
+    DevBuf<uint32_t> dbits, sfd, pbits, slow, wlen, fbits, tcnt, dlen, wl1, sym, pocc, tslot, stamp, aff, merges;
     Counters *ctr = nullptr, *h_ctr = nullptr; TrainState *st = nullptr, *h_st = nullptr;
     unsigned long long *h_u64 = nullptr;
     cudaStream_t s = nullptr;
@@ -1821,7 +1863,7 @@
         DevBuf<unsigned long long> *b64[] = {&doff, &npieces, &wkey, &wcnt, &wfirst, &wused, &part, &tbase, &dfirst, &dcnt, &woff,
                                              &pkey, &pcnt, &th, &tpw, &tlen};
         for (auto *b : b64) b->release();
-        DevBuf<uint32_t> *b32[] = {&dbits, &sfd, &pbits, &psum, &slow, &wlen, &fbits, &tcnt, &dlen, &wl1, &sym, &pocc, &tslot,
+        DevBuf<uint32_t> *b32[] = {&dbits, &sfd, &pbits, &slow, &wlen, &fbits, &tcnt, &dlen, &wl1, &sym, &pocc, &tslot,
                                    &stamp, &aff, &merges};
         for (auto *b : b32) b->release();
         if (ctr) cudaFree(ctr);
@@ -1930,7 +1972,7 @@
         for (uint64_t d = 0; d <= nd; d++) rel[d] = doc_off[lo + d] - base;
         CUDA_TRY(T.doff.ensure(nd + 1)); CUDA_TRY(T.ct.ensure(n + 64));
         CUDA_TRY(T.dbits.ensure((size_t)n_words + 8)); CUDA_TRY(T.sfd.ensure((size_t)n_words + 4));
-        CUDA_TRY(T.pbits.ensure((size_t)n_words + 8)); CUDA_TRY(T.psum.ensure((size_t)(n_words >> 5) + 4));
+        CUDA_TRY(T.pbits.ensure((size_t)n_words + 8));
         CUDA_TRY(T.slow.ensure(n + 64));
         CUDA_TRY(cudaMemcpyAsync(T.doff.p, rel.data(), (nd + 1) * 8, cudaMemcpyHostToDevice, s));
         CUDA_TRY(cudaMemcpyAsync(T.ct.p, T.all.p + base, n, cudaMemcpyDeviceToDevice, s));
@@ -1945,9 +1987,9 @@
         const unsigned grid = (unsigned)((n_words + 255) / 256);
         const uint32_t scap = (uint32_t)std::min<uint64_t>(n + 64, 0xFFFFFFF0u);
 #define B2_TRAIN_PRETOK(P)                                                                                                  \
-    pretok_kernel<P><<<grid, 256, 0, s>>>(T.ct.p, (long long)n, T.dbits.p, uc, T.pbits.p, T.psum.p, n_words, nullptr,     \
+    pretok_kernel<P><<<grid, 256, 0, s>>>(T.ct.p, (long long)n, T.dbits.p, uc, T.pbits.p, 0, n_words, nullptr,            \
                                           T.slow.p, scap, T.ctr);                                                         \
-    pretok_slow_kernel<P><<<n_sm * 8, 256, 0, s>>>(T.ct.p, (long long)n, T.dbits.p, uc, T.pbits.p, T.psum.p, T.slow.p, scap, T.ctr)
+    pretok_slow_kernel<P><<<n_sm * 8, 256, 0, s>>>(T.ct.p, (long long)n, T.dbits.p, uc, T.pbits.p, T.slow.p, scap, T.ctr)
         if (pattern == PAT_R50K) { B2_TRAIN_PRETOK(PAT_R50K); }
         else if (pattern == PAT_CL100K) { B2_TRAIN_PRETOK(PAT_CL100K); }
         else { B2_TRAIN_PRETOK(PAT_O200K); }
diff --git a/tiktoken_b200/csrc/dev_common.cuh b/tiktoken_b200/csrc/dev_common.cuh
--- a/tiktoken_b200/csrc/dev_common.cuh
+++ b/tiktoken_b200/csrc/dev_common.cuh
@@ -42,6 +42,8 @@
     unsigned int err;
     unsigned int n_owner;
     unsigned int n_unplaced;
+    unsigned int slow_done;
+    unsigned int slow_ticket;
 };
 
 static const uint32_t GROUP_MAX = 1024;
diff --git a/tiktoken_b200/csrc/kernels_encode.cuh b/tiktoken_b200/csrc/kernels_encode.cuh
--- a/tiktoken_b200/csrc/kernels_encode.cuh
+++ b/tiktoken_b200/csrc/kernels_encode.cuh
@@ -48,7 +48,6 @@
 };
 
 static const int ENC_WARPS = 4;
-static const int PROBE_BLOCKS_PER_SM = 12;
 static const int SUB_BYTES = 1024;
 static const int STAGE_TEXT = SUB_BYTES + 32;
 static const int STAGE_PW = 36;
@@ -73,13 +72,13 @@
     a3 = __funnelshift_r(w3, w4, sh) & low_mask_clamped(nb - 96);
 }
 
-__global__ void __launch_bounds__(ENC_WARPS * 32) probe_kernel(TileParams p, DevTables T) {
+__global__ void __launch_bounds__(ENC_WARPS * 32) probe_kernel(TileParams p, DevTables T, long long sub0, long long sub1) {
     __shared__ ProbeSmem smem[ENC_WARPS];
     ProbeSmem &S = smem[threadIdx.x >> 5];
     const int lane = threadIdx.x & 31;
     const long long stride = (long long)gridDim.x * ENC_WARPS;
-    long long sub = (long long)blockIdx.x * ENC_WARPS + (threadIdx.x >> 5);
-    if (sub >= p.n_sub) return;
+    long long sub = sub0 + (long long)blockIdx.x * ENC_WARPS + (threadIdx.x >> 5);
+    if (sub >= sub1) return;
     const uint32_t mb0 = smem_u32(&S.mbar[0]), s_text0 = smem_u32(S.text[0]), s_pw0 = smem_u32(S.p[0]);
     auto mb = [&](int b) -> uint32_t { return mb0 + (uint32_t)b * (uint32_t)sizeof(S.mbar[0]); };
     const uint64_t pol = l2_policy_evict_first();
@@ -94,8 +93,8 @@
     };
     if (lane == 0) stage(sub, 0);
     int cur = 0; uint32_t phase = 0;
-    for (; sub < p.n_sub; sub += stride, cur ^= 1) {
-        if (lane == 0 && sub + stride < p.n_sub) stage(sub + stride, cur ^ 1);
+    for (; sub < sub1; sub += stride, cur ^= 1) {
+        if (lane == 0 && sub + stride < sub1) stage(sub + stride, cur ^ 1);
         mbar_wait(mb(cur), (phase >> cur) & 1u);
         phase ^= 1u << cur;
         const uint8_t *txt = S.text[cur];
diff --git a/tiktoken_b200/csrc/kernels_long.cuh b/tiktoken_b200/csrc/kernels_long.cuh
--- a/tiktoken_b200/csrc/kernels_long.cuh
+++ b/tiktoken_b200/csrc/kernels_long.cuh
@@ -6,12 +6,13 @@
 using namespace b2bpe;
 namespace cg = cooperative_groups;
 
+template <bool FINISH>
 __global__ void __launch_bounds__(256) find_long_kernel(const uint32_t *__restrict__ pbits,
                                                         const uint32_t *__restrict__ psum, long long n_bytes,
-                                                        long long n_words, LongQ q, uint32_t *lidx,
+                                                        long long w0, long long w1, LongQ q, uint32_t *lidx,
                                                         const uint32_t *__restrict__ sbits, Counters *ctr) {
-    long long w = blockIdx.x * (long long)blockDim.x + threadIdx.x;
-    if (w >= n_words) return;
+    long long w = w0 + blockIdx.x * (long long)blockDim.x + threadIdx.x;
+    if (w >= w1) return;
     const uint32_t pw = pbits[w];
     if (pw == 0) return;
     uint32_t cand;
@@ -26,6 +27,15 @@
         const int j = __ffs(mm) - 1; mm &= mm - 1;
         const long long s = w * 32 + j;
         if (s >= n_bytes) break;
+        if (!FINISH) {
+            const uint32_t peers = __activemask();
+            unsigned int i = 0;
+            if ((threadIdx.x & 31) == __ffs(peers) - 1) i = atomicAdd(&ctr->n_long, (unsigned int)__popc(peers));
+            i = __shfl_sync(peers, i, __ffs(peers) - 1) + __popc(peers & ((1u << (threadIdx.x & 31)) - 1u));
+            q.start[i] = (unsigned long long)s;
+            lidx[s >> 4] = i;
+            continue;
+        }
         const uint32_t m = (j == 31) ? 0u : (pw & ~((2u << j) - 1u));
         long long nxt;
         if (m) nxt = w * 32 + (__ffs(m) - 1);
@@ -42,29 +52,24 @@
             nxt = w2 * 32 + (__ffs(x) - 1);
         }
         const long long len = nxt - s;
-        if (len > SHORT_MAX) {
-            const uint32_t peers = __activemask();
-            unsigned int i = 0;
-            if ((threadIdx.x & 31) == __ffs(peers) - 1) i = atomicAdd(&ctr->n_long, (unsigned int)__popc(peers));
-            i = __shfl_sync(peers, i, __ffs(peers) - 1) + __popc(peers & ((1u << (threadIdx.x & 31)) - 1u));
-            unsigned long long off = 0; bool fits = true;
-            if (len > LONG_SCRATCH_MIN) {
-                off = atomicAdd(&ctr->long_bytes, (unsigned long long)len);
-                if (off + (unsigned long long)len > q.scratch_cap) { fits = false; atomicOr(&ctr->err, ERR_LONGCAP); }
-            }
-            q.start[i] = (unsigned long long)s; q.len[i] = (unsigned int)len; q.off[i] = off; q.ntok[i] = 0;
-            lidx[s >> 4] = i;
-            const int c = !fits ? N_CLS : len > CLUSTER_MIN ? CLS_CLUSTER : len > BLOCK_MIN ? CLS_BLOCK : len > GROUP_MAX ? CLS_WARP
-                          : len > 256 ? CLS_G1024 : len > 128 ? 3 : len > 64 ? 2 : len > 32 ? 1 : 0;
-            const uint32_t same = __match_any_sync(peers, c);
-            unsigned int k = 0;
-            if ((threadIdx.x & 31) == __ffs(same) - 1) k = atomicAdd(&ctr->n_cls[c], (unsigned int)__popc(same));
-            k = __shfl_sync(peers, k, __ffs(same) - 1) + __popc(same & ((1u << (threadIdx.x & 31)) - 1u));
-            if (c == N_CLS) continue;
-            unsigned int *lst = c == 0 ? q.cls[0] : c == 1 ? q.cls[1] : c == 2 ? q.cls[2] : c == 3 ? q.cls[3] : c == 4 ? q.cls[4]
-                                : c == 5 ? q.cls[5] : c == 6 ? q.cls[6] : q.cls[7];
-            lst[k] = i;
-        }
+        const uint32_t peers = __activemask();
+        const unsigned int i = lidx[s >> 4];
+        unsigned long long off = 0; bool fits = true;
+        if (len > LONG_SCRATCH_MIN) {
+            off = atomicAdd(&ctr->long_bytes, (unsigned long long)len);
+            if (off + (unsigned long long)len > q.scratch_cap) { fits = false; atomicOr(&ctr->err, ERR_LONGCAP); }
+        }
+        q.len[i] = (unsigned int)len; q.off[i] = off; q.ntok[i] = 0;
+        const int c = !fits ? N_CLS : len > CLUSTER_MIN ? CLS_CLUSTER : len > BLOCK_MIN ? CLS_BLOCK : len > GROUP_MAX ? CLS_WARP
+                      : len > 256 ? CLS_G1024 : len > 128 ? 3 : len > 64 ? 2 : len > 32 ? 1 : 0;
+        const uint32_t same = __match_any_sync(peers, c);
+        unsigned int k = 0;
+        if ((threadIdx.x & 31) == __ffs(same) - 1) k = atomicAdd(&ctr->n_cls[c], (unsigned int)__popc(same));
+        k = __shfl_sync(peers, k, __ffs(same) - 1) + __popc(same & ((1u << (threadIdx.x & 31)) - 1u));
+        if (c == N_CLS) continue;
+        unsigned int *lst = c == 0 ? q.cls[0] : c == 1 ? q.cls[1] : c == 2 ? q.cls[2] : c == 3 ? q.cls[3] : c == 4 ? q.cls[4]
+                            : c == 5 ? q.cls[5] : c == 6 ? q.cls[6] : q.cls[7];
+        lst[k] = i;
     }
 }
 
diff --git a/tiktoken_b200/csrc/kernels_pretok.cuh b/tiktoken_b200/csrc/kernels_pretok.cuh
--- a/tiktoken_b200/csrc/kernels_pretok.cuh
+++ b/tiktoken_b200/csrc/kernels_pretok.cuh
@@ -38,26 +38,23 @@
 template <int PAT, bool CUT = false>
 __global__ void __launch_bounds__(PRETOK_WARPS * 32, PAT == PAT_O200K ? 4 : 5) pretok_kernel(const uint8_t *__restrict__ text, long long n_bytes,
                                                                   const uint32_t *__restrict__ dbits, UcTables uc,
-                                                                  uint32_t *__restrict__ pbits, uint32_t *__restrict__ psum,
-                                                                  long long n_words, const uint32_t *__restrict__ ibits,
+                                                                  uint32_t *__restrict__ pbits, long long w0, long long w1,
+                                                                  const uint32_t *__restrict__ ibits,
                                                                   uint32_t *__restrict__ slow_list, uint32_t slow_cap, Counters *ctr) {
     __shared__ uint32_t s_cnt, s_base;
-    const long long w = blockIdx.x * (long long)blockDim.x + threadIdx.x;
+    const long long w = w0 + blockIdx.x * (long long)blockDim.x + threadIdx.x;
     const int lane = threadIdx.x & 31;
     const TextAccess t{text, n_bytes, dbits, uc.stage1, uc.stage2, uc.ascii, uc.one};
     if (threadIdx.x == 0) s_cnt = 0;
     uint64_t b = 0, slow = 0;
-    if (w < n_words) b = span_fast<PAT, CUT>(t, w, slow);
+    if (w < w1) b = span_fast<PAT, CUT>(t, w, slow);
     uint32_t sm = (uint32_t)(slow >> 8);
-    if (ibits && w < n_words) sm &= ~ibits[w];
-    uint32_t word = 0;
-    if (w < n_words) {
-        word = span_word(t, w, b);
+    if (ibits && w < w1) sm &= ~ibits[w];
+    if (w < w1) {
+        uint32_t word = span_word(t, w, b);
         if (ibits) word &= ~ibits[w];
         pbits[w] = word;
     }
-    const uint32_t nz = __ballot_sync(0xFFFFFFFFu, word != 0);
-    if (lane == 0 && (w >> 5) <= ((n_words - 1) >> 5)) psum[w >> 5] = nz;
     const uint32_t cnt = (uint32_t)__popc(sm);
     const uint32_t inc = warp_incl_scan_u32(cnt, lane);
     const uint32_t wtot = __shfl_sync(0xFFFFFFFFu, inc, 31);
@@ -80,18 +77,26 @@
 template <int PAT>
 __global__ void __launch_bounds__(256) pretok_slow_kernel(const uint8_t *__restrict__ text, long long n_bytes,
                                                          const uint32_t *__restrict__ dbits, UcTables uc,
-                                                         uint32_t *pbits, uint32_t *psum, const uint32_t *__restrict__ slow_list,
-                                                         uint32_t slow_cap, const Counters *ctr) {
+                                                         uint32_t *pbits, const uint32_t *__restrict__ slow_list,
+                                                         uint32_t slow_cap, Counters *ctr) {
     if (ctr->err & ERR_SLOWCAP) return;
-    const uint32_t n = min(ctr->n_slow, slow_cap);
+    const uint32_t lo = ctr->slow_done, n = min(ctr->n_slow, slow_cap);
     const TextAccess t{text, n_bytes, dbits, uc.stage1, uc.stage2, uc.ascii};
-    for (uint32_t i = blockIdx.x * 256u + threadIdx.x; i < n; i += gridDim.x * 256u) {
+    for (uint32_t i = lo + blockIdx.x * 256u + threadIdx.x; i < n; i += gridDim.x * 256u) {
         const uint32_t pos = slow_list[i];
-        if (slow_boundary<PAT>(t, (long long)pos)) {
-            atomicOr(&pbits[pos >> 5], 1u << (pos & 31));
-            atomicOr(&psum[pos >> 10], 1u << ((pos >> 5) & 31));
-        }
+        if (slow_boundary<PAT>(t, (long long)pos)) atomicOr(&pbits[pos >> 5], 1u << (pos & 31));
     }
+    __syncthreads();
+    if (threadIdx.x == 0 && atomicAdd(&ctr->slow_ticket, 1u) == gridDim.x - 1) {
+        ctr->slow_done = n;
+        ctr->slow_ticket = 0;
+    }
+}
+
+__global__ void psum_kernel(const uint32_t *__restrict__ pbits, uint32_t *psum, long long n_words) {
+    const long long w = blockIdx.x * (long long)blockDim.x + threadIdx.x;
+    const uint32_t nz = __ballot_sync(0xFFFFFFFFu, w < n_words && pbits[w] != 0);
+    if ((threadIdx.x & 31) == 0 && (w >> 5) <= ((n_words - 1) >> 5)) psum[w >> 5] = nz;
 }
 
 __global__ void single_piece_bits_kernel(uint32_t *pbits, uint32_t *psum, const uint32_t *__restrict__ dbits, long long n_words) {
```

Result: faster. 170.9, median of 6 (+6.9%).
